# quickwit-oss/tantivy

Measured on AMD Instinct MI355X. Metric: queries_per_sec_2term_AND_bm25_top10, higher is better.
Workload: dtype u32+f32; 1 GPU; and2: 10000 queries/batch, k=10, one 10M-doc Zipf segment per GPU (256 terms, df_r=0.5N/r, WithFreqs); term ranks ~ Zipf(1); distinct_queries=3877, mode=block-max pruned (block_wand_intersection semantics), exchange=single rank: no exchange, segments_per_gpu=1, index_bytes=40381332

## Files before the change

include/tantivy_amd.h:

```cpp
#ifndef TANTIVY_AMD_H
#define TANTIVY_AMD_H

#include <stddef.h>
#include <stdint.h>

#ifdef __cplusplus
extern "C" {
#endif

#define TQ_TERMINATED 0x7FFFFFFFu
#define TQ_MAX_TERMS 16u
#define TQ_MAX_K 1024u

enum tq_status {
  TQ_OK = 0,
  TQ_ERR_INVALID = 1,
  TQ_ERR_HIP = 2,
  TQ_ERR_FORMAT = 3,
  TQ_ERR_UNSUPPORTED = 4,
  TQ_ERR_NO_DEVICE = 5
};

enum tq_record_option { TQ_BASIC = 0, TQ_WITH_FREQS = 1, TQ_WITH_FREQS_AND_POSITIONS = 2 };

// ... 152 lines not shown
typedef struct tq_submit_stats {
  uint64_t batches;
  uint64_t queries;
  uint64_t max_batch;
} tq_submit_stats;
int tq_get_submit_stats(tq_segment *seg, tq_submit_stats *out, int reset);

int tq_merge_topk(const float *scores, const uint32_t *docs, const uint32_t *counts,
                  uint32_t n_segments, uint32_t n_queries, uint32_t stride, uint32_t offset,
                  uint32_t limit, float *out_scores, uint32_t *out_segment_ords,
                  uint32_t *out_docs, uint32_t *out_counts);
int tq_merge_topk_device(tq_ctx *ctx, int device, const float *d_scores, const uint32_t *d_docs,
                         const uint32_t *d_counts, const uint32_t *segment_ords,
                         uint32_t n_segments, uint32_t n_queries, uint32_t stride,
                         uint32_t offset, uint32_t limit, float *d_out_scores,
                         uint32_t *d_out_segment_ords, uint32_t *d_out_docs,
                         uint32_t *d_out_counts, void *hip_stream);
int tq_copy_to_host_async(tq_ctx *ctx, int device, void *dst_pinned_host, const void *src_device, size_t bytes,
                          void *hip_stream);

#define TQ_COMM_ID_BYTES 128
typedef struct tq_comm tq_comm;
int tq_comm_unique_id(uint8_t *id_out );
int tq_comm_init(tq_ctx *ctx, int device, const uint8_t *id, int rank, int world, tq_comm **out);
void tq_comm_free(tq_comm *comm);
int tq_comm_info(const tq_comm *comm, int *rank, int *world, const char **library);
int tq_allgather_topk(tq_comm *comm, const float *d_scores, const uint32_t *d_docs,
                      const uint32_t *d_counts, uint32_t n_rows, uint32_t stride,
                      float *d_all_scores, uint32_t *d_all_docs, uint32_t *d_all_counts,
                      void *hip_stream);

int tq_decode_postings(tq_segment *seg, tq_term_handle term, uint32_t *docs, uint32_t *tfs);
int tq_decode_position_deltas(tq_segment *seg, tq_term_handle term, uint32_t *out, uint64_t cap,
                              uint64_t *n_out);

enum {
  TQ_TABLE_REC = 0,
  TQ_TABLE_COARSE = 1,
  TQ_TABLE_TAIL_DOCS = 2,
  TQ_TABLE_TAIL_TFS = 3,
  TQ_TABLE_POS_BLK = 4,
  TQ_TABLE_POS_TAIL = 5,
  TQ_TABLE_DENSE = 6,
  TQ_TABLE_BITS = 7,
  TQ_TABLE_POS_DIR = 8,
  TQ_TABLE_TF8 = 9,
  TQ_TABLE_RMAX = 10,
  TQ_TABLE_RDIR = 11,
  TQ_TABLE_LNORM = 12,
  TQ_TABLE_FLAT = 13,
  TQ_TABLE_PROBE_DENSE = 14,
  TQ_TABLE_PROBE_TF8 = 15,
  TQ_TABLE_PROBE_POS_DIR = 16,
  TQ_TABLE_DOCMAT = 32,
  TQ_TABLE_DOCCLS = 33,
  TQ_TABLE_LOCAL_CACHE = 34,
  TQ_TABLE_MIN_FIELDNORM_ID = 35
};
typedef struct tq_term_table_info_t {
  uint32_t n_blocks, n_full, n_tail, coarse_shift;
  uint64_t payload_base;
  uint32_t has_freq;
  uint32_t rdir_shift;
  uint32_t rmax_list;
  uint32_t n_pos_blocks, n_pos_tail;
  uint32_t field;
  uint64_t n_positions;
  uint32_t doc_freq;
  uint32_t probe_slot;
} tq_term_table_info_t;
int tq_term_table_read(tq_segment *seg, tq_term_handle term, uint32_t which, void *out, uint64_t cap_bytes,
                       uint64_t *n_bytes);
int tq_term_table_info(tq_segment *seg, tq_term_handle term, tq_term_table_info_t *info);

typedef struct tq_encoder tq_encoder;
int tq_encoder_create(tq_ctx *ctx, int device, tq_encoder **out);
void tq_encoder_free(tq_encoder *enc);
int tq_encode_postings(tq_encoder *enc, uint32_t n_terms, const uint64_t *term_starts,
                       const uint32_t *docs, const uint32_t *tfs, const uint8_t *fieldnorm_ids,
                       uint32_t num_docs, float avg_fieldnorm, uint8_t record_option, uint8_t *out,
                       uint64_t out_cap, uint64_t *out_term_starts, uint64_t *out_len);
int tq_encode_positions(tq_encoder *enc, uint32_t n_terms, const uint64_t *term_starts,
                        const uint32_t *position_deltas, uint8_t *out, uint64_t out_cap,
                        uint64_t *out_term_starts, uint64_t *out_len);
int tq_encode_postings_device(tq_encoder *enc, uint32_t n_terms, const uint64_t *term_starts,
                              const uint64_t *d_term_starts, const uint32_t *d_docs,
                              const uint32_t *d_tfs, const uint8_t *d_fieldnorm_ids,
                              uint32_t num_docs, float avg_fieldnorm, uint8_t record_option,
                              uint8_t *d_out, uint64_t out_cap, uint64_t *d_out_term_starts,
                              uint64_t *out_len, void *hip_stream);
int tq_encode_positions_device(tq_encoder *enc, uint32_t n_terms, const uint64_t *term_starts,
                               const uint64_t *d_term_starts, const uint32_t *d_position_deltas,
                               uint8_t *d_out, uint64_t out_cap, uint64_t *d_out_term_starts,
                               uint64_t *out_len, void *hip_stream);
int tq_encoder_last_kernel_ms(tq_encoder *enc, float *ms);

int tq_segment_set_alive_bitset(tq_segment *seg, const uint8_t *bytes, size_t len);
int tq_count_batch(tq_segment *seg, const tq_query *queries, uint32_t n_queries,
                   uint32_t *out_counts);
int tq_last_batch_match_counts(tq_segment *seg, uint32_t *out, uint32_t n_queries);
int tq_last_batch_slop_overflows(tq_segment *seg, uint32_t *out, uint32_t n_queries);

int tq_docset_batch(tq_segment *seg, const tq_query *queries, uint32_t n_queries,
                    uint32_t *out_docs, uint64_t out_cap, uint64_t *out_starts);
int tq_docset_batch_device(tq_segment *seg, const tq_query *queries, uint32_t n_queries,
                           uint32_t *d_out_docs, uint64_t out_cap, uint64_t *d_out_starts, void *hip_stream);
// ... 105 lines not shown
                           tq_agg_bucket_stats_t *out_entry_stats, uint32_t out_stride);
int tq_agg_terms_sub_batch_device(tq_segment *seg, const tq_query *queries, uint32_t n_queries, const tq_agg_terms_sub_request *req,
                                  tq_agg_terms_t *d_out_terms, uint64_t *d_out_keys, uint32_t *d_out_counts,
                                  tq_agg_bucket_stats_t *d_out_entry_stats, uint32_t out_stride, void *hip_stream);
void tq_agg_terms_sub_lds_capacities(uint32_t out[2]);
int tq_agg_terms_metric_image(const tq_agg_bucket_stats_t *rec, uint32_t value_type, uint32_t metric, uint64_t out[2]);

typedef struct tq_batch_stats {
  uint64_t algorithmic_bytes;
  uint64_t matches;
  float kernel_ms;
  float total_ms;
  uint32_t tiles;
  uint32_t chunks;
  uint32_t batches_averaged;
  float host_plan_ms;
  uint32_t kernel_mask;
  uint64_t unique_bytes;
} tq_batch_stats;
#define TQ_KERNEL_AND_DENSE 0x001u
#define TQ_KERNEL_AND 0x002u
#define TQ_KERNEL_UNION 0x004u
#define TQ_KERNEL_OR_WINDOWS 0x008u
#define TQ_KERNEL_PHRASE 0x010u
#define TQ_KERNEL_PHRASE_SWEEP 0x020u
#define TQ_KERNEL_BOOL 0x040u
#define TQ_KERNEL_USHARE 0x080u
#define TQ_KERNEL_XUNION 0x100u
#define TQ_KERNEL_ASHARE 0x200u
#define TQ_KERNEL_BSHARE 0x400u
#define TQ_KERNEL_COUNT_BITMAPS 0x800u
#define TQ_KERNEL_TREE 0x1000u
#define TQ_KERNEL_DOCSET 0x2000u
#define TQ_KERNEL_DOCSET_SCORE 0x4000u
#define TQ_KERNEL_ALL 0x8000u
#define TQ_KERNEL_DOCSET_TREE 0x10000u
#define TQ_KERNEL_DOCSET_TREE_SCORE 0x20000u
#define TQ_KERNEL_PHRASE_SLOP 0x40000u
#define TQ_KERNEL_SORT 0x80000u
#define TQ_KERNEL_AGG 0x100000u
#define TQ_KERNEL_AGG_SUB 0x200000u
#define TQ_KERNEL_AGG_TERMS 0x400000u
#define TQ_KERNEL_AGG_TERMS_SUB 0x800000u
int tq_last_batch_stats(tq_segment *seg, tq_batch_stats *out);
int tq_last_batch_query_kernels(tq_segment *seg, uint32_t *out, uint32_t n_queries);
typedef struct tq_segment_stats {
  uint64_t index_bytes, positions_bytes, fieldnorm_bytes, alive_bytes;
  uint64_t term_table_bytes, bitmap_bytes , docmat_bytes, posdir_bytes;
  uint64_t scratch_bytes;
  uint64_t dense_budget_bytes;
  uint32_t n_terms, n_dense_lists, n_docmat_columns;
  uint32_t probe_evictions;
  uint64_t device_scratch_bytes;
} tq_segment_stats;
int tq_segment_get_stats(tq_segment *seg, tq_segment_stats *out);
int tq_set_option(tq_segment *seg, const char *name, int64_t value);

#ifdef __cplusplus
}
#endif
#endif
```

tantivy_amd/binding.py:

```python
import ctypes as C
import os

import numpy as np

_HERE = os.path.dirname(os.path.abspath(__file__))
LIB_PATH = os.path.join(_HERE, "lib", "libtantivy_amd.so")
if os.environ.get("TQ_LIB_PATH"):
    LIB_PATH = os.environ["TQ_LIB_PATH"]

TERMINATED = 0x7FFFFFFF
TERM_ABSENT = 0xFFFFFFFF
TERM_ALL = 0xFFFFFFFE
STAR = TERM_ALL
ALL_EMPTY, ALL_PLAIN, ALL_BASED = 0, 1, 2
MODE_AND, MODE_OR, MODE_PHRASE, MODE_BOOL, MODE_TERM = 0, 1, 2, 3, 4
SHOULD, MUST, MUST_NOT = 0, 1, 2
BASIC, WITH_FREQS, WITH_FREQS_AND_POSITIONS = 0, 1, 2


class TantivyAmdError(RuntimeError):
    def __init__(self, code, msg):
        super().__init__("tantivy_amd error %d: %s" % (code, msg))
        self.code = code

# ... 20 lines not shown
    _fields_ = [("algorithmic_bytes", C.c_uint64), ("matches", C.c_uint64),
                ("kernel_ms", C.c_float), ("total_ms", C.c_float), ("tiles", C.c_uint32),
                ("chunks", C.c_uint32), ("batches_averaged", C.c_uint32),
                ("host_plan_ms", C.c_float), ("kernel_mask", C.c_uint32), ("unique_bytes", C.c_uint64)]


KERNEL_AND_DENSE, KERNEL_AND, KERNEL_UNION, KERNEL_OR_WINDOWS, KERNEL_PHRASE = 0x1, 0x2, 0x4, 0x8, 0x10
KERNEL_PHRASE_SWEEP, KERNEL_BOOL, KERNEL_USHARE, KERNEL_XUNION, KERNEL_ASHARE = 0x20, 0x40, 0x80, 0x100, 0x200
KERNEL_BSHARE = 0x400
KERNEL_COUNT_BITMAPS = 0x800
KERNEL_TREE = 0x1000
KERNEL_DOCSET = 0x2000
KERNEL_DOCSET_SCORE = 0x4000
KERNEL_ALL = 0x8000
KERNEL_DOCSET_TREE = 0x10000
KERNEL_DOCSET_TREE_SCORE = 0x20000
KERNEL_PHRASE_SLOP = 0x40000
KERNEL_SORT = 0x80000
KERNEL_AGG = 0x100000
KERNEL_AGG_SUB = 0x200000
KERNEL_AGG_TERMS = 0x400000
KERNEL_AGG_TERMS_SUB = 0x800000
VALUE_U64, VALUE_I64, VALUE_F64 = 0, 1, 2
AGG_MAX_BUCKETS = 65536
SORT_DESC, SORT_ASC = 0, 1
NULLS_LAST, NULLS_FIRST = 0, 1
MAX_K = 1024
MAX_SLOP, SLOP_CARRY_CAP = 255, 32
NESTED_PHRASE = 0x10
KERNEL_NAMES = {0x1: "and_dense", 0x2: "and", 0x4: "union", 0x8: "or_windows", 0x10: "phrase", 0x20: "phrase_sweep",
                0x40: "bool", 0x80: "ushare", 0x100: "xunion", 0x200: "ashare", 0x400: "bshare", 0x800: "count_bitmaps",
                0x1000: "tree", 0x2000: "docset", 0x4000: "docset_score", 0x8000: "all", 0x10000: "docset_tree",
                0x20000: "docset_tree_score", 0x40000: "phrase_slop", 0x80000: "sort", 0x100000: "agg", 0x200000: "agg_sub",
                0x400000: "agg_terms", 0x800000: "agg_terms_sub"}


def kernel_names(mask):
    return [n for b, n in sorted(KERNEL_NAMES.items()) if mask & b]


class TqAllForm(C.Structure):
    _fields_ = [("kind", C.c_uint32), ("base", C.c_float), ("min_should", C.c_uint32), ("keep_mask", C.c_uint32)]


class TqSubmitStats(C.Structure):
    _fields_ = [("batches", C.c_uint64), ("queries", C.c_uint64), ("max_batch", C.c_uint64)]


class TqSegmentStats(C.Structure):
    _fields_ = [(n, C.c_uint64) for n in (
        "index_bytes", "positions_bytes", "fieldnorm_bytes", "alive_bytes", "term_table_bytes",
        "bitmap_bytes", "docmat_bytes", "posdir_bytes", "scratch_bytes", "dense_budget_bytes")] + [
        (n, C.c_uint32) for n in ("n_terms", "n_dense_lists", "n_docmat_columns", "probe_evictions")] + [
        ("device_scratch_bytes", C.c_uint64)]


class TqTermInfo(C.Structure):
    _fields_ = [("postings_off", C.c_uint64), ("positions_off", C.c_uint64), ("postings_len", C.c_uint32),
                ("positions_len", C.c_uint32), ("doc_freq", C.c_uint32), ("pad_", C.c_uint32)]


class TqFieldFiles(C.Structure):
    _fields_ = [("idx", C.c_void_p), ("idx_len", C.c_size_t), ("pos", C.c_void_p), ("pos_len", C.c_size_t),
                ("fieldnorm", C.c_void_p), ("fn_len", C.c_size_t)]


class TqFieldsStats(C.Structure):
    _fields_ = [("n_fields", C.c_uint32), ("n_field_terms", C.c_uint32), ("extra_fieldnorm_bytes", C.c_uint64)]


MAX_FIELDS = 8


class TqhTermInfo(C.Structure):
    _fields_ = [("term_id", C.c_uint32), ("doc_freq", C.c_uint32), ("postings_start", C.c_uint64),
                ("postings_end", C.c_uint64), ("positions_start", C.c_uint64),
                ("positions_end", C.c_uint64)]


class TqhQuery(C.Structure):
    _fields_ = [("mode", C.c_uint8), ("n_terms", C.c_uint32), ("terms", C.POINTER(C.c_uint32)),
                ("phrase_offsets", C.POINTER(C.c_uint32)), ("occurs", C.POINTER(C.c_uint8)),
                ("clause_of", C.POINTER(C.c_uint8)), ("min_should_match", C.c_uint32), ("slop", C.c_uint32),
                ("boosts", C.POINTER(C.c_float)), ("nested_occurs", C.POINTER(C.c_uint8)),
                ("clause_min_should", C.POINTER(C.c_uint8)), ("atom_of", C.POINTER(C.c_uint8)),
                ("set_terms", C.POINTER(C.c_uint32)), ("set_starts", C.POINTER(C.c_uint32))]


TERM_SET_BASE = 0xFFFFFF00


class RawHandle(int):
    """A tq_term_handle as the C ABI returned it (DeviceIndex.term_set_prepare): DeviceIndex.term_handle passes it
    through untouched where a plain int is a term id of the dictionary."""


_lib = None

EXPORTS = [
    "tq_init", "tq_shutdown", "tq_last_error", "tq_segment_upload", "tq_segment_upload_device",
    "tq_segment_free",
    "tq_term_prepare", "tq_term_prepare_batch", "tq_search_batch", "tq_search_batch_device", "tq_search_batch_opts",
    "tq_search_batch_device_opts", "tq_search_batch_device_rows", "tq_merge_topk",
    "tq_merge_topk_device", "tq_copy_to_host_async", "tq_decode_postings", "tq_decode_position_deltas",
    "tq_last_batch_stats", "tq_segment_get_stats", "tq_segment_reserve_columns", "tq_set_option", "tq_segment_set_alive_bitset", "tq_count_batch",
    "tq_last_batch_match_counts", "tq_last_batch_slop_overflows", "tq_last_batch_query_kernels", "tq_encoder_create", "tq_encoder_free", "tq_encode_postings",
    "tq_encode_positions", "tq_encode_postings_device", "tq_encode_positions_device",
    "tq_encoder_last_kernel_ms", "tq_comm_unique_id", "tq_comm_init", "tq_comm_free",
    "tq_comm_info", "tq_allgather_topk",
    "tqh_last_error", "tqh_searcher_new", "tqh_searcher_free", "tqh_searcher_add_segment",
    "tqh_prepare_batch", "tqh_prepare_batch_next", "tqh_commit_next", "tqh_search_prepared", "tqh_collect_segment_prepared",
    "tqh_collect_segment_prepared_device", "tqh_search_prepared_device", "tqh_exchange_ms", "tqh_searcher_add_remote_stats",
    "tqh_bm25_for_terms", "tqh_segment_raw", "tqh_term_handle", "tqh_term_dictionary_values",
    "tqh_term_info_store_open", "tqh_term_info_store_free", "tqh_term_info_store_num_terms",
    "tqh_term_info_store_get", "tqh_term_info_store_write", "tqh_searcher_add_segment_with_store",
    "tqh_count_prepared", "tqh_searcher_add_segment_device_with_store",
    "tq_docset_batch", "tq_docset_batch_device", "tqh_docset_prepared",
    "tq_docset_scored_batch", "tq_docset_scored_batch_device", "tqh_docset_scored_prepared",
    "tq_all_query_form",
    "tq_term_set_prepare", "tq_term_set_info", "tq_term_set_release",
    "tq_segment_upload_fields", "tq_segment_get_fields_stats", "tq_term_prepare_field", "tq_term_prepare_batch_fields",
    "tq_term_field", "tqh_searcher_add_segment_fields", "tqh_searcher_add_remote_stats_fields",
    "tq_term_table_read", "tq_term_table_info",
    "tq_column_parse", "tq_column_upload", "tq_column_info", "tq_column_release", "tq_column_decode", "tq_range_prepare",
    "tq_search_sorted_batch", "tq_search_sorted_batch_device",
    "tq_agg_histogram_plan", "tq_agg_batch", "tq_agg_batch_device",
    "tq_agg_sub_batch", "tq_agg_sub_batch_device", "tq_agg_sub_lds_capacities",
    "tq_agg_terms_plan", "tq_agg_terms_batch", "tq_agg_terms_batch_device", "tq_agg_terms_lds_capacities",
    "tq_agg_terms_max_size",
    "tq_agg_terms_sub_batch", "tq_agg_terms_sub_batch_device", "tq_agg_terms_sub_lds_capacities", "tq_agg_terms_metric_image",
]

TERM_TABLES = {
    "rec": (0, np.uint32), "coarse": (1, np.uint32), "tail_docs": (2, np.uint32), "tail_tfs": (3, np.uint32),
    "pos_blk": (4, np.uint64), "pos_tail": (5, np.uint32), "dense": (6, np.uint32), "bits": (7, np.uint32),
    "pos_dir": (8, np.uint32), "tf8": (9, np.uint8), "rmax": (10, np.uint8), "rdir": (11, np.uint32),
    "lnorm": (12, np.uint8), "flat": (13, np.uint8), "probe_dense": (14, np.uint32), "probe_tf8": (15, np.uint8),
    "probe_pos_dir": (16, np.uint32),
    "docmat": (32, np.uint64), "doccls": (33, np.uint64), "local_cache": (34, np.float32), "min_fieldnorm_id": (35, np.uint32),
}


class TqTermTableInfo(C.Structure):
    _fields_ = [("n_blocks", C.c_uint32), ("n_full", C.c_uint32), ("n_tail", C.c_uint32), ("coarse_shift", C.c_uint32),
                ("payload_base", C.c_uint64), ("has_freq", C.c_uint32), ("rdir_shift", C.c_uint32),
                ("rmax_list", C.c_uint32), ("n_pos_blocks", C.c_uint32), ("n_pos_tail", C.c_uint32), ("field", C.c_uint32),
                ("n_positions", C.c_uint64), ("doc_freq", C.c_uint32), ("probe_slot", C.c_uint32)]


class TqColumnInfo(C.Structure):
    _fields_ = [("min_value", C.c_uint64), ("max_value", C.c_uint64), ("gcd", C.c_uint64), ("resident_bytes", C.c_uint64),
                ("num_rows", C.c_uint32), ("num_bits", C.c_uint32), ("codec", C.c_uint32), ("cardinality", C.c_uint32)]


MAX_COLUMNS = 16
CARD_FULL, CARD_OPTIONAL, CARD_MULTIVALUED = 0, 1, 2
CODEC_BITPACKED, CODEC_LINEAR, CODEC_BLOCKWISE_LINEAR = 0, 1, 2
BOUND_KINDS = {"in": 1, "ex": 2}


class TqAggRequest(C.Structure):
    _fields_ = [("column", C.c_uint32), ("value_type", C.c_uint8), ("histogram", C.c_uint8), ("has_hard_bounds", C.c_uint8),
                ("reserved", C.c_uint8), ("interval", C.c_double), ("offset", C.c_double), ("hard_min", C.c_double),
                ("hard_max", C.c_double)]


class TqAggHistPlan(C.Structure):
    _fields_ = [("base_pos", C.c_int64), ("n_buckets", C.c_uint32), ("reserved", C.c_uint32), ("bounds_min", C.c_double),
                ("bounds_max", C.c_double)]


AGG_STATS_DTYPE = np.dtype([(n, np.uint64) for n in ("matches", "count", "min_value", "max_value", "sum_lo", "sum_hi",
                                                     "in_bounds", "out_of_range")])


class TqAggMetricRequest(C.Structure):
    _fields_ = [("column", C.c_uint32), ("value_type", C.c_uint8), ("reserved", C.c_uint8 * 3)]


AGG_BUCKET_STATS_DTYPE = np.dtype([(n, np.uint64) for n in ("count", "min_value", "max_value", "sum_lo", "sum_hi")])


def _agg_request(column, value_type, histogram):
    req = TqAggRequest(column=int(column), value_type=int(value_type))
    if histogram is not None:
        req.histogram = 1
        req.interval = float(histogram["interval"])
        req.offset = float(histogram.get("offset", 0.0))
        hb = histogram.get("hard_bounds")
        if hb is not None:
            req.has_hard_bounds, req.hard_min, req.hard_max = 1, float(hb[0]), float(hb[1])
# ... 1040 lines not shown
        _check(lib().tq_term_table_info(self.segment_raw(segment_ord), int(handle), C.byref(info)))
        return {n: int(getattr(info, n)) for n, _ in TqTermTableInfo._fields_}

    def decode_position_deltas(self, term_id, cap, segment_ord=0):
        h = self.term_handle(term_id, segment_ord)
        out = np.zeros(max(1, cap), np.uint32)
        n = C.c_uint64()
        _check(lib().tq_decode_position_deltas(self.segment_raw(segment_ord), h, _u32(out), cap,
                                               C.byref(n)))
        return out[: min(cap, n.value)], n.value

    def set_alive_bitset(self, alive_bytes, segment_ord=0):
        if alive_bytes is None:
            _check(lib().tq_segment_set_alive_bitset(self.segment_raw(segment_ord), None, 0))
            return
        a = np.ascontiguousarray(np.frombuffer(bytes(alive_bytes), dtype=np.uint8))
        _check(lib().tq_segment_set_alive_bitset(self.segment_raw(segment_ord), a.ctypes.data,
                                                 a.size))

    def last_batch_match_counts(self, n, segment_ord=0):
        out = np.zeros(max(1, n), np.uint32)
        _check(lib().tq_last_batch_match_counts(self.segment_raw(segment_ord), _u32(out), n))
        return out[:n]

    def last_batch_slop_overflows(self, n, segment_ord=0):
        out = np.zeros(max(1, n), np.uint32)
        _check(lib().tq_last_batch_slop_overflows(self.segment_raw(segment_ord), _u32(out), n))
        return out[:n]

    def last_batch_query_kernels(self, n, segment_ord=0):
        out = np.zeros(max(1, n), np.uint32)
        _check(lib().tq_last_batch_query_kernels(self.segment_raw(segment_ord), _u32(out), n))
        return out[:n]

    def set_option(self, name, value, segment_ord=None):
        ords = range(self.n_segments) if segment_ord is None else [segment_ord]
        for o in ords:
            _check(lib().tq_set_option(self.segment_raw(o), name.encode(), int(value)))

    def last_batch_stats(self, segment_ord=0):
        st = TqBatchStats()
        _check(lib().tq_last_batch_stats(self.segment_raw(segment_ord), C.byref(st)))
        return {"algorithmic_bytes": st.algorithmic_bytes, "matches": st.matches,
                "kernel_ms": st.kernel_ms, "total_ms": st.total_ms, "tiles": st.tiles,
                "chunks": st.chunks, "batches_averaged": st.batches_averaged,
                "host_plan_ms": st.host_plan_ms, "kernel_mask": int(st.kernel_mask),
                "kernels": kernel_names(int(st.kernel_mask)), "unique_bytes": int(st.unique_bytes)}

    def segment_stats(self, segment_ord=0):
        st = TqSegmentStats()
        _check(lib().tq_segment_get_stats(self.segment_raw(segment_ord), C.byref(st)))
        out = {n: int(getattr(st, n)) for n, _ in TqSegmentStats._fields_}
        out["derived_bytes"] = (out["term_table_bytes"] + out["bitmap_bytes"] + out["docmat_bytes"]
                                + out["posdir_bytes"])
        out["tantivy_bytes"] = (out["index_bytes"] + out["positions_bytes"] + out["fieldnorm_bytes"]
                                + out["alive_bytes"])
        return out

    def _raw_flat_queries(self, queries, segment_ord):
        n = len(queries)
        qs = (TqQuery * max(1, n))()
        keep = []
        for i, q in enumerate(queries):
            extra = q[-1] if isinstance(q[-1], dict) else None
            if extra is not None:
                q = q[:-1]
            mode, terms = q[0], q[1]
            hs = (C.c_uint32 * max(1, len(terms)))(*[self.term_handle(t, segment_ord) for t in terms])
            keep.append(hs)
            qs[i].n_terms = len(terms)
            qs[i].terms = C.cast(hs, C.POINTER(C.c_uint32))
            qs[i].mode = mode
            qs[i].k = 1
            if mode == MODE_BOOL:
                oc = (C.c_uint8 * len(terms))(*[int(o) for o in q[2]])
                keep.append(oc)
                qs[i].occurs = C.cast(oc, C.POINTER(C.c_uint8))
                if len(q) > 3 and q[3] is not None:
                    co = (C.c_uint8 * len(terms))(*[int(o) for o in q[3]])
                    keep.append(co)
                    qs[i].clause_of = C.cast(co, C.POINTER(C.c_uint8))
                if len(q) > 4:
                    qs[i].min_should_match = int(q[4])
                if extra and extra.get("nested_occurs") is not None:
                    na = (C.c_uint8 * len(terms))(*[int(o) for o in extra["nested_occurs"]])
                    keep.append(na)
                    qs[i].nested_occurs = C.cast(na, C.POINTER(C.c_uint8))
                if extra and extra.get("atom_of") is not None:
                    aa = (C.c_uint8 * len(terms))(*[int(o) for o in extra["atom_of"]])
                    keep.append(aa)
                    qs[i].atom_of = C.cast(aa, C.POINTER(C.c_uint8))
                if extra and extra.get("phrase_offsets") is not None:
                    pa = (C.c_uint32 * len(terms))(*[int(o) for o in extra["phrase_offsets"]])
                    keep.append(pa)
                    qs[i].phrase_offsets = C.cast(pa, C.POINTER(C.c_uint32))
                if extra and extra.get("clause_min_should") is not None:
                    ma = (C.c_uint8 * 16)(*[int(extra["clause_min_should"].get(c, 0)) for c in range(16)])
                    keep.append(ma)
                    qs[i].clause_min_should = C.cast(ma, C.POINTER(C.c_uint8))
            elif mode == MODE_PHRASE:
                oa = (C.c_uint32 * len(terms))(*(q[2] if len(q) > 2 and q[2] is not None else range(len(terms))))
                keep.append(oa)
                qs[i].phrase_offsets = C.cast(oa, C.POINTER(C.c_uint32))
                if len(q) > 3:
                    qs[i].slop = int(q[3])
        return qs, keep

# ... 390 lines not shown
```

tantivy_amd/csrc/tq_api.cpp:

```cpp
#include "tq_internal.hpp"
#include "../host/bm25.hpp"

namespace tqi {

thread_local std::string g_last_error;

int fail(int code, const char *fmt, ...) {
  char buf[512];
  va_list ap;
  va_start(ap, fmt);
  vsnprintf(buf, sizeof buf, fmt, ap);
  va_end(ap);
  g_last_error = buf;
  return code;
}
}

int tq_internal_fail(int code, const char *where, const char *what) {
  return fail(code, "%s: %s", where, what);
}
bool tq_internal_ctx_has_device(const tq_ctx *ctx, int device) {
  return std::find(ctx->devices.begin(), ctx->devices.end(), device) != ctx->devices.end();
}

// ... 465 lines not shown
      }
      s->batches_reported = s->batches_timed;
      if (n) {
        s->stats.kernel_ms = (float)(k_sum / n);
        s->stats.total_ms = (float)(t_sum / n);
      }
      s->stats.batches_averaged = n;
    }
    s->stats.host_plan_ms = s->host_ms_n ? (float)(s->host_ms_sum / s->host_ms_n) : 0.0f;
    s->host_ms_sum = 0;
    s->host_ms_n = 0;
    s->stats_pending = false;
  }
  *out = s->stats;
  return TQ_OK;
}

int tq_segment_reserve_columns(tq_segment *s, const uint64_t *postings_offs, uint32_t n) {
  if (!s || (!postings_offs && n)) return fail(TQ_ERR_INVALID, "tq_segment_reserve_columns: null argument");
  TQ_SEGMENT_LOCK(s);
  if (!s->terms.empty())
    return fail(TQ_ERR_INVALID, "tq_segment_reserve_columns: call it before the first tq_term_prepare");
  s->reserved_cols.clear();
  for (uint32_t i = 0; i < n && i < TQD_MAT_SLOTS; ++i) s->reserved_cols[postings_offs[i]] = true;
  s->cols_reserved = true;
  return TQ_OK;
}

int tq_segment_get_stats(tq_segment *s, tq_segment_stats *out) {
  if (!s || !out) return fail(TQ_ERR_INVALID, "tq_segment_get_stats: null argument");
  TQ_SEGMENT_LOCK(s);
  tq_segment_stats r{};
  r.index_bytes = s->idx_len;
  r.positions_bytes = s->pos_len;
  r.fieldnorm_bytes = s->d_fn ? s->max_doc : 0;
  r.alive_bytes = s->bytes_alive;
  r.term_table_bytes = s->bytes_term_tables + s->d_terms_cap * sizeof(TqdTerm);
  r.bitmap_bytes = s->bytes_bitmaps;
  r.docmat_bytes = s->bytes_docmat;
  r.posdir_bytes = s->bytes_posdir;
  r.scratch_bytes = s->d_stage.cap + s->d_stage_alt.cap + s->d_misc.cap + s->d_thr.cap + s->d_qmatches.cap + s->d_share_words.cap +
                    s->d_ashare_words.cap + s->d_bshare_words.cap + s->d_count_queries.cap + s->d_count_out.cap +
                    s->d_count_bits.cap + s->d_count_wgs.cap + s->d_set_work.cap + s->docset_scratch_bytes();
  {
    std::lock_guard<std::mutex> lk(s->dscratch->m);
    r.device_scratch_bytes = s->dscratch->partials.cap + s->dscratch->share_stage.cap + s->dscratch->ashare_stage.cap +
                             s->dscratch->bshare_stage.cap;
  }
  r.n_terms = (uint32_t)s->terms.size();
  r.n_dense_lists = s->n_dense_lists;
  r.n_docmat_columns = s->n_mat_slots;
  r.probe_evictions = (uint32_t)std::min<uint64_t>(s->probe_evictions, 0xFFFFFFFFull);
  r.dense_budget_bytes = s->dense_budget();
  *out = r;
  return TQ_OK;
}

int tq_set_option(tq_segment *s, const char *name, int64_t value) {
  if (!s || !name) return fail(TQ_ERR_INVALID, "tq_set_option: null argument");
  TQ_SEGMENT_LOCK(s);
  if (!strcmp(name, "exhaustive"))
    __atomic_store_n(&s->opt.exhaustive, value != 0 ? 1 : 0, __ATOMIC_RELAXED);
  else if (!strcmp(name, "timing"))
    s->opt.timing = value != 0;
  else if (!strcmp(name, "use_dpp"))
    s->opt.use_dpp = value != 0;
  else if (!strcmp(name, "use_dense"))
    s->opt.use_dense = value != 0;
  else if (!strcmp(name, "or_windows"))
    s->opt.or_windows = value < 0 ? -1 : (value != 0);
  else if (!strcmp(name, "dense_ratio") && value >= 1)
    s->opt.dense_ratio = (int)value;
  else if (!strcmp(name, "rdir_budget_x") && value >= 0 && value <= 0x7FFFFFFF)
    s->opt.rdir_budget_x = (int)value;
  else if (!strcmp(name, "probe_budget_x") && value >= 0 && value <= 0x7FFFFFFF)
    s->opt.probe_budget_x = (int)value, s->probe_full = false;
  else if (!strcmp(name, "dense_budget_x") && value >= 0)
    s->opt.dense_budget_x = (int)value;
  else if (!strcmp(name, "bound_slack_ppm") && value >= 0 && value <= 1000000000)
    __atomic_store_n(&s->opt.bound_slack_ppm, (int)value, __ATOMIC_RELAXED);
  else if (!strcmp(name, "dense"))
    s->opt.dense = value != 0;
  else if (!strcmp(name, "docmat"))
    s->opt.docmat = value != 0;
  else if (!strcmp(name, "docsig"))
    s->opt.docsig = value != 0;
  else if (!strcmp(name, "device_prepare"))
    s->opt.device_prepare = value != 0;
  else if (!strcmp(name, "xunion_ratio") && value >= 0 && value <= 0x7FFFFFFF)
    s->opt.xunion_ratio = (int)value;
  else if (!strcmp(name, "count_bitmap_ratio") && value >= 0 && value <= 0x7FFFFFFF)
    s->opt.count_bitmap_ratio = (int)value;
  else if (!strcmp(name, "docset_temp_lists") && value >= 0 && value <= 0x7FFFFFFF)
    s->opt.docset_temp_lists = (int)value;
  else if (!strcmp(name, "docset_trees") && (value == 0 || value == 1))
    s->opt.docset_trees = (int)value;
  else if (!strcmp(name, "docset_score_trees") && (value == 0 || value == 1))
    s->opt.docset_score_trees = (int)value;
  else if (!strcmp(name, "sort_slices") && value >= 0 && value <= 256)
    s->opt.sort_slices = (int)value;
  else if (!strcmp(name, "agg_slices") && value >= 0 && value <= 256)
    s->opt.agg_slices = (int)value;
  else if (!strcmp(name, "agg_lds_buckets") && value >= 0 && value <= (int64_t)tqk_agg_lds_buckets())
    s->opt.agg_lds_buckets = (int)value;
  else if (!strcmp(name, "ashare_inline_warm") && value >= 0 && value <= 2)
    s->opt.ashare_inline_warm = (int)value;
  else if (!strcmp(name, "ashare_min_batch") && value >= 0 && value <= 0x7FFFFFFF)
    s->opt.ashare_min_batch = (int)value;
  else if (!strcmp(name, "xunion_min_queries") && value >= 1 && value <= 0x7FFFFFFF)
    s->opt.xunion_min_queries = (int)value;
  else if (!strcmp(name, "record_query_kernels"))
    s->opt.record_query_kernels = value != 0;
  else if (!strcmp(name, "debug") && value >= -1 && value <= 0x7FFFFFFF)
    s->opt.debug = (int)value;
  else if (!strcmp(name, "submit_window_us") && value >= 0 && value <= 1000000)
    s->opt.submit_window_us = (int)value;
  else
    return fail(TQ_ERR_INVALID, "unknown option '%s'", name);
  return TQ_OK;
}

int tq_decode_postings(tq_segment *s, tq_term_handle term, uint32_t *docs, uint32_t *tfs) {
  if (!s || !docs || !tfs) return fail(TQ_ERR_INVALID, "tq_decode_postings: null argument");
  TQ_SEGMENT_LOCK(s);
  if (term >= s->terms.size()) return fail(TQ_ERR_INVALID, "unknown term handle %u", term);
  if (s->terms[term].set_kind != TermHost::kNoSet) return fail(TQ_ERR_INVALID, "tq_decode_postings: handle %u is a term set: it has no postings", term);
  HIP_TRY(hipSetDevice(s->device));
// ... 26 lines not shown
  if (n == 0 || !out) return TQ_OK;
  HIP_TRY(hipSetDevice(s->device));
  int rc = sync_terms(s, s->stream);
  if (rc != TQ_OK) return rc;
  rc = s->d_misc.ensure(n * sizeof(uint32_t));
  if (rc != TQ_OK) return rc;
  hipError_t e = tqk_launch_decode_positions(s->dseg, s->d_terms, term, (uint32_t *)s->d_misc.p, n,
                                             s->stream);
  if (e != hipSuccess) return fail(TQ_ERR_HIP, "decode launch: %s", hipGetErrorString(e));
  HIP_TRY(hipMemcpyAsync(out, s->d_misc.p, n * sizeof(uint32_t), hipMemcpyDeviceToHost, s->stream));
  HIP_TRY(hipStreamSynchronize(s->stream));
  return TQ_OK;
}

namespace {
struct TableSpan {
  const void *p = nullptr;
  size_t bytes = 0;
  bool host = false;
};
bool table_span(tq_segment *s, uint32_t term, uint32_t which, TableSpan &sp) {
  if (which >= TQ_TABLE_DOCMAT) {
    const size_t per_doc = (size_t)s->max_doc * sizeof(uint64_t);
    switch (which) {
      case TQ_TABLE_DOCMAT: sp = {s->d_docmat, s->d_docmat ? per_doc : 0, false}; return true;
      case TQ_TABLE_DOCCLS: sp = {s->d_doccls, s->d_doccls ? per_doc : 0, false}; return true;
      case TQ_TABLE_LOCAL_CACHE: sp = {s->d_local_cache, s->d_local_cache ? 256 * sizeof(float) : 0, false}; return true;
      case TQ_TABLE_MIN_FIELDNORM_ID: sp = {&s->dseg.min_fieldnorm_id, sizeof(uint32_t), true}; return true;
      default: return false;
    }
  }
  const TermHost &t = s->terms[term];
  const TqdTerm &d = s->h_dterms[term];
  const size_t n_words = bitmap_words(s);
  const size_t n_dir = ((size_t)t.doc_freq + 3) / 4 + 1;
  const bool list = t.set_kind == TermHost::kNoSet;
  uint32_t n_buckets = 0;
  if (list && t.n_blocks) (void)coarse_shift(s->max_doc, t.n_blocks, &n_buckets);
  auto span = [&](const void *p, size_t bytes) { sp = {p, p ? bytes : 0, false}; };
  switch (which) {
    case TQ_TABLE_REC: span(list ? d.rec : nullptr, 16 * ((size_t)t.n_blocks + 1)); return true;
    case TQ_TABLE_COARSE: span(list ? d.coarse : nullptr, 4 * ((size_t)n_buckets + 1)); return true;
    case TQ_TABLE_TAIL_DOCS: span(list && t.n_tail ? d.tail_docs : nullptr, 4 * (size_t)t.n_tail); return true;
    case TQ_TABLE_TAIL_TFS: span(list && t.n_tail ? d.tail_tfs : nullptr, 4 * (size_t)t.n_tail); return true;
    case TQ_TABLE_POS_BLK: span(list && d.n_pos_blocks ? d.pos_blk : nullptr, 8 * (size_t)d.n_pos_blocks); return true;
    case TQ_TABLE_POS_TAIL: span(list && d.n_pos_tail ? d.pos_tail : nullptr, 4 * (size_t)d.n_pos_tail); return true;
    case TQ_TABLE_DENSE: span(t.dense_blob, n_words * sizeof(uint2)); return true;
    case TQ_TABLE_BITS: span(list ? d.bits : nullptr, ((n_words + 255) & ~(size_t)255) * sizeof(uint32_t)); return true;
    case TQ_TABLE_POS_DIR: span(list ? t.posdir_blob : nullptr, n_dir * sizeof(uint32_t)); return true;
    case TQ_TABLE_TF8: span(list ? t.tf8_blob : nullptr, t.doc_freq); return true;
    case TQ_TABLE_RMAX: span(list ? t.rmax_blob : nullptr, tqd_rm_level_off(s->max_doc, TQD_RM_LEVELS)); return true;
    case TQ_TABLE_RDIR: span(list ? t.rdir_blob : nullptr, t.rdir_shift ? rdir_bytes(s, t.doc_freq, t.rdir_shift) : 0); return true;
    case TQ_TABLE_LNORM: span(list ? t.lnorm_blob : nullptr, (size_t)t.n_blocks * 128u); return true;
    case TQ_TABLE_FLAT:
      span(list ? t.flat_blob : nullptr, (((size_t)t.doc_freq * sizeof(uint32_t) + 15) & ~(size_t)15) + t.doc_freq);
      return true;
    case TQ_TABLE_PROBE_DENSE: span(t.probe_dense_blob, n_words * sizeof(uint2)); return true;
    case TQ_TABLE_PROBE_TF8: span(t.probe_tf8_blob, t.doc_freq); return true;
    case TQ_TABLE_PROBE_POS_DIR: span(t.probe_posdir_blob, n_dir * sizeof(uint32_t)); return true;
    default: return false;
  }
}
int table_handle_ok(tq_segment *s, tq_term_handle term, const char *who) {
  if (term >= s->terms.size()) return fail(TQ_ERR_INVALID, "%s: unknown term handle %u", who, term);
  if (s->terms[term].set_kind == TermHost::kSetReleased) return fail(TQ_ERR_INVALID, "%s: handle %u is a released term set", who, term);
  return TQ_OK;
}
int table_quiesce(tq_segment *s) {
  HIP_TRY(hipSetDevice(s->device));
  const int rc = wait_segment_idle(s);
  if (rc != TQ_OK) return rc;
  HIP_TRY(hipStreamSynchronize(s->stream));
  prep_apply_lmax(s, true);
  return TQ_OK;
}
}

int tq_term_table_read(tq_segment *s, tq_term_handle term, uint32_t which, void *out, uint64_t cap_bytes, uint64_t *n_bytes) {
  if (!s || !n_bytes) return fail(TQ_ERR_INVALID, "tq_term_table_read: null argument");
  *n_bytes = 0;
  TQ_SEGMENT_LOCK(s);
  if (which < TQ_TABLE_DOCMAT) {
    const int hrc = table_handle_ok(s, term, "tq_term_table_read");
    if (hrc != TQ_OK) return hrc;
  }
  int rc = table_quiesce(s);
  if (rc != TQ_OK) return rc;
  TableSpan sp;
  if (!table_span(s, term, which, sp)) return fail(TQ_ERR_INVALID, "tq_term_table_read: unknown table %u", which);
  *n_bytes = sp.bytes;
  if (!sp.bytes || !out || !cap_bytes) return TQ_OK;
  if (cap_bytes < sp.bytes)
    return fail(TQ_ERR_INVALID, "tq_term_table_read: table %u holds %zu bytes, room for %llu", which, sp.bytes, (unsigned long long)cap_bytes);
  if (sp.host) {
    memcpy(out, sp.p, sp.bytes);
    return TQ_OK;
  }
  HIP_TRY(hipMemcpyAsync(out, sp.p, sp.bytes, hipMemcpyDeviceToHost, s->stream));
  HIP_TRY(hipStreamSynchronize(s->stream));
  return TQ_OK;
}

int tq_term_table_info(tq_segment *s, tq_term_handle term, tq_term_table_info_t *info) {
  if (!s || !info) return fail(TQ_ERR_INVALID, "tq_term_table_info: null argument");
  TQ_SEGMENT_LOCK(s);
  int rc = table_handle_ok(s, term, "tq_term_table_info");
// ... 113 lines not shown
```

tantivy_amd/csrc/tq_ashare.hip:

```cpp
#include "tq_common.hpp"

#ifndef TQ_BS_SGPR
#define TQ_BS_SGPR 96
#endif
#ifndef TQ_BS_WAVES
#define TQ_BS_WAVES 5
#endif
#ifndef TQ_AS_WAVES
#define TQ_AS_WAVES 5
#endif
#ifndef TQ_AS_TIMERS
#define TQ_AS_TIMERS 0
#endif
#ifndef TQ_AS_PREFETCH
#define TQ_AS_PREFETCH 1
#endif

namespace {

constexpr uint32_t AS_GROUP = TQD_AS_GROUP;
constexpr uint32_t AS_COUNTER_BITS = 0x7FE0u | 0xF00000u | 0x40000000u;

template <bool BOOLQ>
struct AShareLds {
  float cache[256];
  uint32_t q_doc[127], q_tf[127], q_tag[127];
  TqdALeadLds lead[AS_GROUP];
  uint32_t lthr[AS_GROUP];
  uint32_t lk[AS_GROUP];
  uint32_t cnt[AS_GROUP];
  uint32_t flen[AS_GROUP];
  float bw[BOOLQ ? AS_GROUP * TQD_AS_MAX_TERMS : 1];
  uint32_t pay[(TQ_AS_PREFETCH && !BOOLQ) ? 260 : 1];
};

template <int R>
__device__ __forceinline__ uint64_t as_kth_largest_key(const uint64_t (&v)[R], uint32_t k) {
  uint64_t ans = 0;
  for (int bit = 63; bit >= 0; --bit) {
    const uint64_t trial = ans | (1ull << bit);
    uint32_t c = 0;
#pragma unroll
    for (int r = 0; r < R; ++r) c += (uint32_t)__popcll(__ballot(v[r] >= trial));
    if (c >= k) ans = trial;
  }
  return ans;
}

__device__ __forceinline__ uint32_t as_exact_tf(const uint8_t *idx, const TqdTerm *terms, uint32_t handle,
                                                uint32_t pi) {
  const TqdTermHead *h = terms + handle;
  TermRef tr{};
  tr.rec = h->rec;
  tr.tail_tfs = h->tail_tfs;
  tr.payload_base = h->payload_base;
  tr.has_freq = h->has_freq & 1u;
  const uint4 r = tr.rec[pi >> 7];
  return block_tf_at(idx, tr, make_uint2(r.y, r.z), pi & 127u);
}

template <int KPL, bool BOOLQ, bool RD = false>
__global__ __launch_bounds__(64) __attribute__((amdgpu_num_sgpr(TQ_BS_SGPR), amdgpu_waves_per_eu(BOOLQ ? TQ_BS_WAVES : TQ_AS_WAVES, 8))) void
ashare_kernel(TqkAShareParams p) {
  constexpr bool USE_DPP = true;
  constexpr bool PF = TQ_AS_PREFETCH && !BOOLQ;
  constexpr int R = KPL + 1;
  constexpr uint32_t CAPL = (uint32_t)R * 64u;
  __shared__ AShareLds<BOOLQ> L;
  const int lane = (int)__lane_id();
  const TqdSegment seg = p.seg;
  const uint8_t *idx = seg.idx;
  uint64_t *const my_stage = p.stage + (size_t)blockIdx.x * (size_t)(AS_GROUP * CAPL);
  const uint8_t *const tbase = p.table_base;
  const uint32_t bmode = BOOLQ ? 0u : p.bound_mode;
  uint32_t cache_loaded = 0xFFFFFFFFu;
  uint32_t qn = 0;
  uint32_t n_scored = 0;
  uint32_t n_leads = 0;
  const uint32_t tphase = TQ_AS_TIMERS ? (p.debug >> 16) & 15u : 0u;
  uint64_t tacc = 0, tlast = 0;
  auto tb = [&](uint32_t ph) __attribute__((always_inline)) {
    if (TQ_AS_TIMERS && tphase == ph) tlast = __builtin_readcyclecounter();
  };
  auto te = [&](uint32_t ph) __attribute__((always_inline)) {
    if (TQ_AS_TIMERS && tphase == ph) tacc += __builtin_readcyclecounter() - tlast;
  };
// ... 231 lines not shown
    wave_mem_fence();
    const uint32_t cn = (uint32_t)lane < AS_GROUP ? L.cnt[lane] & 0xFFFFu : 0u;
    uint64_t full = __ballot(cn > CAPL - 64u);
    while (full) {
      const uint32_t gs = (uint32_t)__builtin_ctzll(full);
      full &= full - 1ull;
      const uint32_t ns = (uint32_t)__builtin_amdgcn_readlane((int)cn, (int)gs);
      const uint32_t ks = uni(L.lk[gs]) & 0xFFu;
      if (p.debug & 4096u) ++n_scored;
      const uint64_t kth = compact_slot(gs, ns, ks);
      const uint32_t t = (uint32_t)(kth >> 32);
      if ((uint32_t)lane == gs) {
        L.cnt[gs] = (L.cnt[gs] & 0xFFFF0000u) | ks;
        if (t > L.lthr[gs]) L.lthr[gs] = t;
        atomicMax(p.thr_val + L.lead[gs].query, t);
      }
    }
    wave_mem_fence();
    te(7u);
    tb(6u);
  };

  const uint32_t n_launch = p.n_tasks - p.task_begin;
  const uint32_t nq = p.n_queues ? p.n_queues : 1u;
  const uint32_t xcc = (uint32_t)__builtin_amdgcn_s_getreg((3 << 11) | 20) & 7u;
  const uint32_t home = xcc % nq;
  uint32_t q_tried = 0;
  for (;;) {
    tb(2u);
    uint32_t task = 0xFFFFFFFFu;
    while (q_tried < nq) {
      uint32_t qx = home + q_tried;
      if (qx >= nq) qx -= nq;
      const uint32_t q0 = (uint32_t)((uint64_t)n_launch * qx / nq), q1 = (uint32_t)((uint64_t)n_launch * (qx + 1u) / nq);
      uint32_t t = 0;
      if (lane == 0) t = atomicAdd(p.task_counter + qx, 1u);
      t = uni(t) + q0;
      if (t < q1) {
        task = t + p.task_begin;
        break;
      }
      ++q_tried;
    }
    if (task == 0xFFFFFFFFu) break;
    const uint4 trec = sload(p.tasks + task);
    const uint32_t j0 = trec.y, nb_task = trec.z & 0xFFFFu, ci = trec.z >> 24, lead0 = trec.w;
    n_leads = (trec.z >> 16) & 0xFFu;
    const TermRef lead = load_term(p.terms, trec.x);
    uint32_t lnorm = 0;
    if constexpr (!BOOLQ) lnorm = sload(&p.leads[lead0].any2_lo);
    auto norm_pair = [&](uint32_t j) __attribute__((always_inline)) -> uint32_t {
      return reinterpret_cast<const uint16_t *>(tbase + ((uint64_t)lnorm << 3))[(size_t)j * 64u + (uint32_t)lane];
    };
    if (ci != cache_loaded) {
      const float *cg = p.caches + (size_t)ci * 256u;
      wave_mem_fence();
      for (int i = lane; i < 256; i += WAVE) L.cache[i] = cg[i];
      wave_mem_fence();
      cache_loaded = ci;
    }
    wave_mem_fence();
    float my_w = 0.0f, my_rest = 0.0f;
    uint32_t my_mlo = 0, my_mhi = 0;
    uint32_t my_xlo = 0, my_xhi = 0, my_a1lo = 0, my_a1hi = 0, my_a2lo = 0, my_a2hi = 0;
    uint32_t my_blo = 0, my_bhi = 0;
    bool twin = false;
    const bool is_lead = (uint32_t)lane < n_leads;
    if (is_lead) {
      const TqdALead mine = p.leads[lead0 + lane];
      L.lead[lane] = TqdALeadLds{mine.query, mine.info, mine.w, mine.rest, mine.dense_off, mine.tf8_off};
      my_w = mine.w;
      my_rest = mine.rest;
      my_mlo = mine.mask_lo;
      my_mhi = mine.mask_hi;
      if constexpr (BOOLQ) {
        my_xlo = mine.excl_lo;
        my_xhi = mine.excl_hi;
        my_a1lo = mine.any1_lo;
        my_a1hi = mine.any1_hi;
        my_a2lo = mine.any2_lo;
        my_a2hi = mine.any2_hi;
        my_blo = mine.dense_off;
        my_bhi = mine.tf8_off;
        const TqdQuery *Q = p.queries + mine.query;
        const uint32_t li = (mine.info >> 16) & 15u, nt = mine.info & 31u;
#pragma unroll
        for (uint32_t m = 0; m < TQD_AS_MAX_TERMS; ++m) L.bw[(uint32_t)lane * TQD_AS_MAX_TERMS + m] = (m > li && m < nt) ? Q->weight[m] : 0.0f;
      }
      if constexpr (!BOOLQ) {
        my_xlo = (bmode && (mine.info & 31u) == 2u) ? mine.excl_lo : 0u;
        const bool rdir = bmode && (mine.info & TQD_AL_RDIR) != 0u;
        my_xhi = rdir ? mine.dense_off | ((mine.info >> 16) & 31u) : 0u;
        if (my_xlo || rdir) {
          const float r1 = mine.rest * p.bound_slack * (1.00002f / 255.0f) * (float)(mine.any1_hi & 0xFFu);
          my_rest = r1 < mine.rest ? r1 : mine.rest;
        }
      }
      twin = lane != 0 && (mine.info & 0x200u) != 0u;
      L.lk[lane] = mine.k | (mine.thr_row << 8);
      L.lthr[lane] = __hip_atomic_load(p.thr_val + mine.query, __ATOMIC_RELAXED, __HIP_MEMORY_SCOPE_AGENT);
    }
    if ((uint32_t)lane < AS_GROUP) L.cnt[lane] = 0u;
    const bool is_head = is_lead && !twin;
    const uint32_t heads = (uint32_t)__ballot(is_head);
    if (is_head) {
      const uint32_t above = (uint32_t)lane >= 31u ? 0u : heads & ~((2u << lane) - 1u);
// ... 60 lines not shown
          blk_last = rec_mine.x;
          const uint32_t wide = blk_last >= blk_first ? (blk_last - blk_first) >> TQD_RM_SHIFT : 0xFFFFFFFFu;
          const uint32_t lvl = wide ? (33u - (uint32_t)__builtin_clz(wide)) >> 1 : 0u;
          if (lvl < TQD_RM_LEVELS) rm_pack = tqd_rm_level_off(seg.max_doc, lvl) | ((TQD_RM_SHIFT + 2u * lvl) << 24);
        }
      }
      uint32_t pass_mask = 0;
      float need_blk = 3.0e38f;
      for (uint32_t lm = live_heads; lm; lm &= lm - 1u) {
        const uint32_t g = (uint32_t)__builtin_ctz(lm);
        const float w = __uint_as_float((uint32_t)__builtin_amdgcn_readlane((int)__float_as_uint(my_w), (int)g));
        float rest = __uint_as_float((uint32_t)__builtin_amdgcn_readlane((int)__float_as_uint(my_rest), (int)g));
        const uint32_t thr = (uint32_t)__builtin_amdgcn_readlane((int)fam_thr, (int)g);
        if constexpr (!BOOLQ) {
          const uint32_t rmo = (uint32_t)__builtin_amdgcn_readlane((int)my_xlo, (int)g);
          if ((bmode & 1u) && rmo) {
            const uint8_t *rt = tbase + ((uint64_t)rmo << 3) + (rm_pack & 0xFFFFFFu);
            const uint32_t sh = rm_pack >> 24;
            const uint32_t qa = sh ? (uint32_t)rt[blk_first >> sh] : 255u, qb = sh ? (uint32_t)rt[blk_last >> sh] : 255u;
            if (p.debug & 0x800000u) n_scored += 2u * (uint32_t)__popcll(__ballot(sh != 0u));
            const float w1 = uni_f(L.lead[g].rest);
            const float r1 = w1 * p.bound_slack * (1.00002f / 255.0f) * (float)(qa > qb ? qa : qb);
            rest = r1 < rest ? r1 : rest;
          }
        }
        bool empty = false;
        if constexpr (!BOOLQ) {
          const uint32_t rdo = (uint32_t)__builtin_amdgcn_readlane((int)my_xhi, (int)g);
          if ((bmode & 1u) && rdo) {
            const uint32_t S = rdo & 31u;
            const uint32_t *dr = reinterpret_cast<const uint32_t *>(tbase + ((uint64_t)(rdo & ~31u) << 3));
            if (blk_last >= blk_first) empty = dr[blk_first >> S] == dr[(blk_last >> S) + 1u];
          }
        }
        const float ub = w * tfn_max * p.bound_slack;
        if (in_tile && !empty && sortable((ub + rest) * 1.000004f + (w + rest) * 4.0e-6f) >= thr) {
          pass_mask |= 1u << g;
          if constexpr (!BOOLQ) {
            const float thr_f = __uint_as_float((uint32_t)__builtin_amdgcn_readlane((int)__float_as_uint(fam_thr_f), (int)g));
            const float num = thr_f - rest * 1.00001f;
            const float nd = (thr_f > 0.0f && num > 0.0f) ? num * __builtin_amdgcn_rcpf(w) * 0.99999f : -1.0f;
            need_blk = nd < need_blk ? nd : need_blk;
          }
        }
      }
      uint64_t todo = __ballot(pass_mask != 0u);
      uint32_t since_refresh = 0;
      te(3u);
      uint32_t npair_next = 0;
      auto prefetch = [&](uint64_t rest) __attribute__((always_inline)) {
        if (!PF || !rest) return;
        const uint32_t nb2 = (uint32_t)__builtin_ctzll(rest);
        if (lnorm) npair_next = norm_pair(i_base + nb2);
        const uint32_t meta = (uint32_t)__builtin_amdgcn_readlane((int)rec_mine.y, (int)nb2);
        const uint32_t off = (uint32_t)__builtin_amdgcn_readlane((int)rec_mine.z, (int)nb2);
        if (meta == META_TAIL) return;
        const uint32_t nbytes = 16u * ((meta & 31u) + (lead.has_freq ? (meta >> 8) & 0xFFu : 0u));
        const uint32_t o = 16u * (uint32_t)lane;
        if (o < nbytes)
          __builtin_amdgcn_global_load_lds((const __attribute__((address_space(1))) void *)(idx + lead.payload_base + off + o),
                                           (__attribute__((address_space(3))) void *)L.pay, 16, 0, 0);
      };
      if constexpr (PF) {
        wave_mem_fence();
        prefetch(todo);
      }
      while (todo) {
        const uint32_t b = (uint32_t)__builtin_ctzll(todo);
        todo &= todo - 1ull;
        if (++since_refresh == 8u) {
          since_refresh = 0;
          tb(9u);
          refresh_thr();
          update_families();
          te(9u);
          if (!live) break;
        }
        tb(4u);
        uint32_t lm = (uint32_t)__builtin_amdgcn_readlane((int)pass_mask, (int)b) & live_heads;
        const uint32_t prev_l = (uint32_t)__builtin_amdgcn_readlane((int)prev_mine, (int)b);
        const uint2 mo_l = make_uint2((uint32_t)__builtin_amdgcn_readlane((int)rec_mine.y, (int)b),
                                      (uint32_t)__builtin_amdgcn_readlane((int)rec_mine.z, (int)b));
        if (!lm) {
          if constexpr (PF) {
            asm volatile("s_waitcnt vmcnt(0)" ::: "memory");
            wave_mem_fence();
            prefetch(todo);
          }
          te(4u);
          continue;
        }
        if (p.debug & 256u) ++n_scored;
        if (p.debug & 0x100000u)
          n_scored += 16u + (mo_l.x == META_TAIL ? 8u * lead.n_tail : 16u * ((mo_l.x & 31u) + (lead.has_freq ? (mo_l.x >> 8) & 0xFFu : 0u)));
        uint32_t c0, c1, t0, t1;
        uint32_t npair = 0;
        if constexpr (PF) {
        npair = npair_next;
        if (mo_l.x == META_TAIL) {
          asm volatile("s_waitcnt vmcnt(0)" ::: "memory");
          decode_docs<USE_DPP>(idx, lead, mo_l, prev_l, lane, c0, c1);
          decode_tfs(idx, lead, mo_l, lane, t0, t1);
        } else {
          const uint32_t doc_bits = mo_l.x & 31u;
          const uint32_t strict = (mo_l.x >> 6) & 1u;
          const uint32_t tf_bits = lead.has_freq ? (mo_l.x >> 8) & 0xFFu : 0u;
          asm volatile("s_waitcnt vmcnt(0)" ::: "memory");
          wave_mem_fence();
          if (lead.has_freq) {
            unpack2_lds(L.pay + 4u * doc_bits, tf_bits, lane, t0, t1);
            t0 += strict;
            t1 += strict;
          } else {
            t0 = 1u;
            t1 = 1u;
          }
          uint32_t x0, x1;
          unpack2_lds(L.pay, doc_bits, lane, x0, x1);
          finish_docs<USE_DPP>(x0, x1, strict, prev_l, lane, c0, c1);
        }
        wave_mem_fence();
        prefetch(todo);
        } else {
        if (lnorm) npair = norm_pair(i_base + b);
        decode_docs<USE_DPP>(idx, lead, mo_l, prev_l, lane, c0, c1);
        decode_tfs(idx, lead, mo_l, lane, t0, t1);
        }
        if (TQ_AS_TIMERS && tphase == 4u && c0 == 0xFFFFFFFEu) ++n_scored;
        te(4u);
        tb(5u);
        const bool v0 = c0 != TQD_TERMINATED, v1 = c1 != TQD_TERMINATED;
        float block_need = 3.0e38f;
        for (uint32_t x = lm; x; x &= x - 1u) {
          const float nd = __uint_as_float((uint32_t)__builtin_amdgcn_readlane((int)__float_as_uint(fam_need), (int)__builtin_ctz(x)));
          block_need = nd < block_need ? nd : block_need;
        }
        if constexpr (!BOOLQ) {
          if (bmode & 2u) {
            const float nb = __uint_as_float((uint32_t)__builtin_amdgcn_readlane((int)__float_as_uint(need_blk), (int)b));
            block_need = nb > block_need ? nb : block_need;
          }
        }
        if (!lnorm) {
          npair = (v0 ? fieldnorm_id(seg, c0) : 0u) | ((v1 ? fieldnorm_id(seg, c1) : 0u) << 8);
          if (p.debug & 0x40000000u) n_scored += (uint32_t)(__popcll(__ballot(v0)) + __popcll(__ballot(v1)));
        }
        const uint32_t nid0 = npair & 0xFFu, nid1 = npair >> 8;
        const float f0 = (float)t0, f1 = (float)t1;
        const float tfn0 = f0 * __builtin_amdgcn_rcpf(f0 + L.cache[nid0]);
        const float tfn1 = f1 * __builtin_amdgcn_rcpf(f1 + L.cache[nid1]);
        const bool g0 = v0 && tfn0 >= block_need, g1 = v1 && tfn1 >= block_need;
        const uint64_t mw0 = g0 ? seg.docmat[c0] : 0ull;
        const uint64_t mw1 = g1 ? seg.docmat[c1] : 0ull;
        const uint64_t valid0 = __ballot(g0), valid1 = __ballot(g1);
        if (p.debug & 0x200000u) n_scored += (uint32_t)(__popcll(__ballot(v0)) + __popcll(__ballot(v1)));
        if (p.debug & 0x400000u) n_scored += (uint32_t)(__popcll(valid0) + __popcll(valid1));
        if (TQ_AS_TIMERS && tphase == 5u && (uint32_t)mw0 == 0xFFFFFFFEu) ++n_scored;
        te(5u);
        tb(6u);
        uint32_t pm_lo = 0, pm_hi = 0;
        uint64_t mem0 = valid0, mem1 = valid1;
        uint32_t pb0 = 0xFFu, pb1 = 0xFFu;
        if (p.debug & 2048u) lm = 0;
        for (; lm; lm &= lm - 1u) {
          const uint32_t g = (uint32_t)__builtin_ctz(lm);
          if (p.debug & 32u) ++n_scored;
          const uint32_t mlo = (uint32_t)__builtin_amdgcn_readlane((int)my_mlo, (int)g);
          const uint32_t mhi = (uint32_t)__builtin_amdgcn_readlane((int)my_mhi, (int)g);
          const float need = __uint_as_float((uint32_t)__builtin_amdgcn_readlane((int)__float_as_uint(fam_need), (int)g));
          if constexpr (BOOLQ) {
            const uint32_t xlo = (uint32_t)__builtin_amdgcn_readlane((int)my_xlo, (int)g);
            const uint32_t xhi = (uint32_t)__builtin_amdgcn_readlane((int)my_xhi, (int)g);
            const uint32_t a1lo = (uint32_t)__builtin_amdgcn_readlane((int)my_a1lo, (int)g);
            const uint32_t a1hi = (uint32_t)__builtin_amdgcn_readlane((int)my_a1hi, (int)g);
            const uint32_t a2lo = (uint32_t)__builtin_amdgcn_readlane((int)my_a2lo, (int)g);
            const uint32_t a2hi = (uint32_t)__builtin_amdgcn_readlane((int)my_a2hi, (int)g);
            const uint32_t l0 = (uint32_t)mw0, h0 = (uint32_t)(mw0 >> 32), l1 = (uint32_t)mw1, h1 = (uint32_t)(mw1 >> 32);
            bool b0 = !((l0 & xlo) | (h0 & xhi));
            bool b1 = !((l1 & xlo) | (h1 & xhi));
            if (a1lo | a1hi) {
              b0 = b0 && ((l0 & a1lo) | (h0 & a1hi));
              b1 = b1 && ((l1 & a1lo) | (h1 & a1hi));
            }
            if (a2lo | a2hi) {
              b0 = b0 && ((l0 & a2lo) | (h0 & a2hi));
              b1 = b1 && ((l1 & a2lo) | (h1 & a2hi));
            }
            b0 = b0 && tfn0 >= need;
            b1 = b1 && tfn1 >= need;
            if (!((__ballot(b0) & valid0) | (__ballot(b1) & valid1))) continue;
            const uint32_t blo = (uint32_t)__builtin_amdgcn_readlane((int)my_blo, (int)g);
            const uint32_t bhi = (uint32_t)__builtin_amdgcn_readlane((int)my_bhi, (int)g);
            pb0 = pb1 = (uni(L.lead[g].info) >> 20) & 0xFFu;
            if (blo | bhi) {
              const float wl = __uint_as_float((uint32_t)__builtin_amdgcn_readlane((int)__float_as_uint(my_w), (int)g));
              const float thr_f = __uint_as_float((uint32_t)__builtin_amdgcn_readlane((int)__float_as_uint(fam_thr_f), (int)g));
              const float4 wa = *reinterpret_cast<const float4 *>(&L.bw[g * TQD_AS_MAX_TERMS]);
              const float4 wb = *reinterpret_cast<const float4 *>(&L.bw[g * TQD_AS_MAX_TERMS + 4u]);
              const float wv[8] = {wa.x, wa.y, wa.z, wa.w, wb.x, wb.y, wb.z, wb.w};
              float ps0 = __uint_as_float(mlo), ps1 = ps0;
#pragma unroll
              for (uint32_t m = 0; m < TQD_AS_MAX_TERMS; ++m) {
                const uint32_t bp = ((m < 4u ? blo : bhi) >> (8u * (m & 3u))) & 0xFFu;
                if (!bp) continue;
                const uint32_t sh = bp & 31u;
                const uint32_t p0 = ((bp & 32u ? h0 : l0) >> sh) & 1u, p1 = ((bp & 32u ? h1 : l1) >> sh) & 1u;
                ps0 += p0 ? wv[m] : 0.0f;
                ps1 += p1 ? wv[m] : 0.0f;
                pb0 &= ~((p0 ^ 1u) << m);
// ... 174 lines not shown
```

tantivy_amd/csrc/tq_internal.hpp:

```cpp
#pragma once
#include <hip/hip_runtime.h>

#include <algorithm>
#include <array>
#include <atomic>
#include <chrono>
#include <condition_variable>
#include <deque>
#include <map>
#include <mutex>
#include <new>
#include <cstdlib>
#include <cmath>
#include <cstdarg>
#include <cstdio>
#include <cstring>
#include <string>
#include <unordered_map>
#include <unordered_set>
#include <thread>
#include <vector>

#include "../../include/tantivy_amd.h"
#include "tq_device.h"
// ... 28 lines not shown
    cap = 0;
    void *np = nullptr;
    HIP_TRY(hipMalloc(&np, ncap));
    p = np;
    cap = ncap;
    return TQ_OK;
  }
  void release() {
    if (p) (void)hipFree(p);
    p = nullptr;
    cap = 0;
  }
};
struct PinnedBuf {
  void *p = nullptr;
  size_t cap = 0;
  int ensure(size_t n) {
    if (n <= cap) return TQ_OK;
    const size_t ncap = std::max(n, cap * 2);
    if (p) (void)hipHostFree(p);
    p = nullptr;
    cap = 0;
    void *np = nullptr;
    HIP_TRY(hipHostMalloc(&np, ncap, hipHostMallocDefault));
    p = np;
    cap = ncap;
    return TQ_OK;
  }
  void release() {
    if (p) (void)hipHostFree(p);
    p = nullptr;
    cap = 0;
  }
};

struct TermHost {
  void *blob = nullptr;
  const TqdTerm *d_self = nullptr;
  void *dense_blob = nullptr;
  void *posdir_blob = nullptr;
  void *tf8_blob = nullptr;
  void *pos_blob = nullptr;
  void *probe_dense_blob = nullptr, *probe_tf8_blob = nullptr;
  void *probe_posdir_blob = nullptr;
  int32_t probe_slot = -1;
  void *rdir_blob = nullptr;
  void *rdir_ent = nullptr;
  uint32_t rdir_shift = 0;
  uint8_t *probe_own_dir = nullptr;
  void *rmax_blob = nullptr;
  uint32_t rmax_list = 255;
  void *flat_blob = nullptr;
  void *lnorm_blob = nullptr;
  uint32_t doc_freq = 0, n_blocks = 0, n_full = 0, n_tail = 0;
  uint32_t last_doc = 0;
  bool wants_col = true;
  uint64_t postings_len = 0, positions_len = 0;
  uint64_t n_positions = 0;
  enum : uint8_t { kNoSet = 0, kSet = 1, kSetReleased = 2 };
  uint8_t set_kind = kNoSet;
  uint8_t field = 0;
};

inline uint32_t rd32(const uint8_t *p) {
  return (uint32_t)p[0] | ((uint32_t)p[1] << 8) | ((uint32_t)p[2] << 16) | ((uint32_t)p[3] << 24);
}
inline bool read_vint(const uint8_t *d, size_t len, size_t &at, uint64_t &out) {
  uint64_t r = 0;
  unsigned shift = 0;
  while (at < len) {
    uint8_t b = d[at++];
    r |= (uint64_t)(b & 127u) << shift;
    if (b & 128u) {
      out = r;
      return true;
    }
    shift += 7;
    if (shift > 63) return false;
  }
  return false;
}
inline bool read_vint32_block(const uint8_t *d, size_t len, size_t &at, uint32_t &out) {
  uint32_t r = 0, shift = 0;
  while (at < len) {
    uint8_t b = d[at++];
    r += (uint32_t)(b & 127u) << shift;
    if (b & 128u) {
      out = r;
      return true;
    }
    shift += 7;
  }
  return false;
}

struct Options {
  int exhaustive = 0;
  int timing = 0;
  int use_dpp = 1;
  int dense = 1;
  int dense_ratio = TQD_DENSE_RATIO;
  int dense_budget_x = 8;
  int use_dense = 1;
  int docmat = 1;
  int docsig = 1;
  int device_prepare = 0;
  int or_windows = -1;
  int bound_slack_ppm = 0;
  int xunion_ratio = 64;
  int xunion_min_queries = 64;
  int rdir_budget_x = 4;
  int probe_budget_x = 16;
  int count_bitmap_ratio = 128;
  int docset_temp_lists = 0;
  int docset_trees = 0;
  int docset_score_trees = 0;
  int sort_slices = 0;
  int agg_slices = 0;
  int agg_lds_buckets = -1;
  int ashare_inline_warm = 1;
  int ashare_min_batch = 16;
  int submit_window_us = 100;
  int record_query_kernels = 0;
  int debug = -1;
};


inline uint32_t tune_u32(const char *name, uint32_t dflt) {
  const char *v = getenv(name);
  return v && *v ? (uint32_t)strtoul(v, nullptr, 10) : dflt;
}

}
using namespace tqi;

struct DeviceScratch {
  std::mutex m;
  DevBuf partials, share_stage, ashare_stage, bshare_stage;
  hipEvent_t ev_last = nullptr;
  hipStream_t last_stream = nullptr;
  bool in_flight = false;
};
struct tq_ctx {
  std::vector<int> devices;
  std::mutex m;
  std::map<int, DeviceScratch *> scratch;
  DeviceScratch *scratch_for(int device) {
    std::lock_guard<std::mutex> lk(m);
    DeviceScratch *&p = scratch[device];
    if (!p) p = new DeviceScratch();
    return p;
  }
  ~tq_ctx() {
    for (auto &kv : scratch) {
      (void)hipSetDevice(kv.first);
      if (kv.second->ev_last) (void)hipEventDestroy(kv.second->ev_last);
      kv.second->partials.release();
      kv.second->share_stage.release();
      kv.second->ashare_stage.release();
      kv.second->bshare_stage.release();
      delete kv.second;
    }
  }
// ... 34 lines not shown
  bool d_terms_dirty = false;
  size_t d_terms_dirty_from = ~(size_t)0;
  size_t d_terms_synced = 0;
  size_t dense_bytes_total = 0;
  uint8_t *dense_arena = nullptr;
  size_t dense_arena_cap = 0, dense_arena_used = 0;
  std::vector<void *> dense_extra;
  bool dense_arena_vmm = false;
  void *dense_arena_va = nullptr;
  size_t dense_arena_mapped = 0, dense_arena_first = 0;
  std::vector<std::pair<hipMemGenericAllocationHandle_t, size_t>> dense_arena_chunks;
  size_t bytes_term_tables = 0, bytes_bitmaps = 0, bytes_docmat = 0, bytes_posdir = 0, bytes_alive = 0;
  uint32_t n_dense_lists = 0;
  uint32_t n_set_slots = 0;
  std::vector<uint32_t> set_free_slots;
  std::vector<void *> set_free_tables;
  DevBuf d_set_work;
  struct ColumnHost {
    bool live = false;
    tq_column_info_t info{};
    TqkColumn dev{};
    void *d_payload = nullptr;
    void *d_blocks = nullptr;
    void *d_present = nullptr;
    uint64_t payload_len = 0;
  };
  ColumnHost columns[TQ_MAX_COLUMNS];
  uint32_t alive_docs = 0;
  std::unordered_map<uint64_t, uint32_t> term_by_off;
  std::unordered_map<uint64_t, bool> reserved_cols;
  bool cols_reserved = false;
  DevBuf d_stage, d_misc, d_thr, d_qmatches;
  DevBuf d_share_words;
  DevBuf d_count_queries, d_count_out, d_count_bits, d_count_wgs;
  DevBuf d_docset_queries, d_docset_counts, d_docset_offs, d_docset_partials, d_docset_starts, d_docset_docs;
  DevBuf d_docset_squeries, d_docset_caches, d_docset_scores;
  DevBuf d_docset_trees;
  DevBuf d_sort_ks, d_sort_partials, d_sort_slice_counts, d_sort_rows;
  PinnedBuf h_sort_ks;
  DevBuf d_agg_rows;
  DevBuf d_agg_term_rows;
  PinnedBuf h_docset;
  size_t docset_scratch_bytes() const {
    return d_docset_queries.cap + d_docset_counts.cap + d_docset_offs.cap + d_docset_partials.cap + d_docset_starts.cap +
           d_docset_docs.cap + d_docset_squeries.cap + d_docset_caches.cap + d_docset_scores.cap +
           d_docset_trees.cap + d_sort_ks.cap + d_sort_partials.cap + d_sort_slice_counts.cap + d_sort_rows.cap + d_agg_rows.cap + d_agg_term_rows.cap;
  }
  DevBuf d_ashare_words, d_bshare_words;
  DeviceScratch *dscratch = nullptr;
  size_t share_span_terms = 0;
  uint64_t share_table_lo = 0;
  bool share_span_ok = true;
  bool lnorm_off = false;
  uint32_t last_batch_queries = 0;
  DevBuf d_slop_over;
  bool last_batch_slop = false;
  uint32_t slop_over_words = 0;
  std::vector<uint32_t> slop_over_host;
  std::vector<uint32_t> last_query_kernel;
  PinnedBuf h_stage, h_out;
  static constexpr int kTimingRing = 16;
  hipEvent_t ev_stage_done = nullptr, ev_fork = nullptr, ev_join = nullptr;
  hipEvent_t ev_batch_done = nullptr;
  hipStream_t last_stream = nullptr;
  bool batch_in_flight = false;
  hipStream_t side_stream = nullptr;
  hipStream_t copy_stream = nullptr;
  DevBuf d_stage_alt;
  hipEvent_t ev_copy_done[2] = {nullptr, nullptr}, ev_buf_free[2] = {nullptr, nullptr};
  bool buf_used[2] = {false, false};
  uint64_t batches_enqueued = 0;
  hipEvent_t ev_t0[kTimingRing] = {}, ev_t1[kTimingRing] = {}, ev_k0[kTimingRing] = {},
             ev_k1[kTimingRing] = {};
  uint64_t batches_timed = 0, batches_reported = 0;
  bool stage_in_flight = false;
  double host_ms_sum = 0;
  uint32_t host_ms_n = 0;
  unsigned long long *d_match_counter = nullptr;
  Options opt;
  size_t dense_budget() const { return (size_t)opt.dense_budget_x * (idx_len + pos_len + max_doc); }
  size_t probe_budget() const { return (size_t)opt.probe_budget_x * (idx_len + pos_len + max_doc); }
  size_t rdir_budget() const { return (size_t)opt.rdir_budget_x * (idx_len + pos_len + max_doc); }
  size_t rdir_bytes_total = 0;
  PinnedBuf h_prep_stage[2];
  hipEvent_t ev_prep[2] = {nullptr, nullptr}, ev_prep_order = nullptr;
  bool prep_used[2] = {false, false};
  uint32_t prep_calls = 0;
  int prep_pending = -1;
  std::vector<uint32_t> prep_lmax_handles[2];
  const uint32_t *prep_lmax_host[2] = {nullptr, nullptr};
  size_t probe_bytes_total = 0;
  bool probe_full = false;
  struct ProbeSlot {
    uint8_t *base = nullptr;
    uint32_t owner = 0xFFFFFFFFu;
    uint64_t last_batch = 0;
  };
  std::vector<ProbeSlot> probe_slots;
  size_t probe_slot_bytes = 0, probe_bm_bytes = 0, probe_tf_cap = 0, probe_dir_cap = 0, probe_rm_bytes = 0;
  uint64_t probe_batch = 1;
  uint64_t probe_evictions = 0;
  uint64_t probe_replaced_batch = 0;
  uint32_t probe_replaced_n = 0;
  uint64_t probe_no_room_batch = 0;
  bool probe_waited = false;
  bool device_prepare() const { return h_idx.empty() || opt.device_prepare != 0; }
// ... 369 lines not shown
inline bool dense_fits(const tq_segment *s) { return s->dense_bytes_total + dense_table_bytes(s) <= s->dense_budget(); }
struct WalkSource {
  const uint8_t *idx;
  size_t idx_len;
  const uint8_t *pos;
  size_t pos_len;
  uint8_t record_option;
  uint32_t max_doc;
};
inline WalkSource walk_source(const tq_segment *s) {
  return {s->h_idx.data(), s->h_idx.size(), s->h_pos.data(), s->h_pos.size(), s->record_option, s->max_doc};
}
inline size_t align16(size_t x) { return (x + 15) & ~(size_t)15; }
struct TermBlobLayout {
  size_t o_rec = 0, o_coarse = 0, o_tdocs = 0, o_ttfs = 0, o_pboff = 0, o_ptail = 0, o_self = 0, total = 0;
};
TermBlobLayout term_blob_layout(uint32_t n_blocks, uint32_t n_buckets, uint32_t n_tail, uint32_t n_pos_blocks, uint32_t n_pos_tail);
uint32_t coarse_shift(uint32_t max_doc, uint32_t n_blocks, uint32_t *n_buckets);
struct WalkedTerm {
  std::vector<uint8_t> hb;
  TermBlobLayout lay;
  TqdTerm dt{};
  TermHost th;
  uint64_t postings_off = 0;
};
int host_walk_term(const WalkSource &src, uint64_t postings_off, uint32_t postings_len, uint64_t positions_off,
                   uint32_t positions_len, uint32_t doc_freq, WalkedTerm &w);
void place_walked_term(WalkedTerm &w, uint8_t *blob);
const char *tqp_message(uint32_t st);
int term_alloc(tq_segment *s, size_t bytes, uint8_t **out);
void term_release(tq_segment *s, uint8_t *blob, size_t bytes);
int dense_alloc(tq_segment *s, size_t bytes, void **out);
void dense_release(tq_segment *s, void *ptr);
void dense_arena_free(tq_segment *s);
int rdir_alloc(tq_segment *s, size_t bytes, void **out);
struct DecodedList {
  uint32_t *dd = nullptr, *dt = nullptr, *scan_scratch = nullptr, *rm_acc = nullptr;
};
int decode_list(tq_segment *s, const TermHost &t, size_t scan_words, bool want_rm, DecodedList &dl);
hipError_t enqueue_bitmap(tq_segment *s, const DecodedList &dl, uint32_t doc_freq, void *blob);
hipError_t enqueue_rmax(tq_segment *s, const DecodedList &dl, uint32_t doc_freq, uint8_t *out);
hipError_t finish_tables(tq_segment *s, const DecodedList &dl, uint32_t *bad, uint32_t *lmax);
inline uint32_t rmax_list_of(uint32_t lmax) { return lmax ? std::min<uint32_t>(lmax, 255u) : 255u; }
inline uint32_t sig_bit(uint32_t handle) { return (handle * 0x9E3779B1u) >> (32 - 4); }
uint32_t rdir_plan(tq_segment *s, uint32_t doc_freq);
size_t rdir_dir_words(const tq_segment *s, uint32_t S);
size_t rdir_bytes(const tq_segment *s, uint32_t doc_freq, uint32_t S);
int attach_rdir(tq_segment *s, uint32_t handle, uint32_t S, void **tab);
int ensure_docmat(tq_segment *s);
int add_to_doc_signatures(tq_segment *s, uint32_t handle);
int build_dense_device(tq_segment *s, uint32_t handle);
int build_flat(tq_segment *s, uint32_t handle, hipStream_t st, bool *ok);
void build_lnorm(tq_segment *s, uint32_t handle, hipStream_t st);
void prep_apply_lmax(tq_segment *s, bool wait);
int build_probe_tables(tq_segment *s, uint32_t handle, bool *ok, bool must = false);
int build_probe_posdir(tq_segment *s, uint32_t handle, bool *ok);
void probe_begin_batch(tq_segment *s);
void probe_touch(tq_segment *s, uint32_t handle);
inline bool query_has_all(const tq_query &q) {
  if (!q.terms || q.n_terms > TQ_MAX_TERMS) return false;
  for (uint32_t i = 0; i < q.n_terms; ++i)
    if (q.terms[i] == TQ_TERM_ALL) return true;
  return false;
}
struct AllForm {
  uint32_t kind = TQ_ALL_EMPTY;
  float base = 0.0f;
  uint32_t min_should = 0, keep_mask = 0;
  bool boost_mixed = false;
};
int all_query_form(const tq_query &q, AllForm &f, const char **why);
struct AllView {
  tq_query q;
  tq_term_handle terms[TQ_MAX_TERMS];
  float weights[TQ_MAX_TERMS];
  uint8_t occurs[TQ_MAX_TERMS], clause_of[TQ_MAX_TERMS];
  uint32_t pos[TQ_MAX_TERMS];
};
void all_strip_view(const tq_query &q, const AllForm &f, AllView &v);
inline bool is_term_set(const tq_segment *s, uint32_t h) { return h < s->terms.size() && s->terms[h].set_kind == TermHost::kSet; }
int set_table_acquire(tq_segment *s, void **tab);
void set_table_release(tq_segment *s, void *tab);
uint32_t set_slot_commit(tq_segment *s, void *tab, uint32_t n_docs);
void free_columns(tq_segment *s);
inline const void *expression_bitmap(const tq_segment *s, const TermHost &th) {
  return th.dense_blob && (s->opt.use_dense || th.set_kind == TermHost::kSet) ? th.dense_blob : nullptr;
}
static_assert(TQK_MAX_FIELDS == TQ_MAX_FIELDS, "the multi-field launch parameters hold one fieldnorm pointer per field");
inline uint32_t term_field_of(const tq_segment *s, uint32_t h) { return h < s->terms.size() ? s->terms[h].field : 0u; }
inline bool query_names_field(const tq_segment *s, const tq_query &q) {
  if (!q.terms || q.n_terms > TQ_MAX_TERMS) return false;
  for (uint32_t i = 0; i < q.n_terms; ++i)
    if (term_field_of(s, q.terms[i])) return true;
  return false;
}
struct FieldScope {
  tq_segment *s;
  uint8_t was;
  FieldScope(tq_segment *seg, uint8_t field) : s(seg), was(seg->prep_field) { s->prep_field = field; }
  ~FieldScope() { s->prep_field = was; }
  FieldScope(const FieldScope &) = delete;
  FieldScope &operator=(const FieldScope &) = delete;
};
int check_field_query(const tq_segment *s, const tq_query &q, uint32_t qi, const char *fn);
inline bool query_names_set(const tq_segment *s, const tq_query &q) {
  if (!q.terms || q.n_terms > TQ_MAX_TERMS) return false;
// ... 163 lines not shown
```

tantivy_amd/csrc/tq_launch.h:

```cpp
#pragma once
#include <hip/hip_runtime.h>
#include <stdint.h>

#include "tq_device.h"

struct TqkSinks {
  uint64_t *partials;
  unsigned long long *match_counter;
  uint32_t *query_matches;
  const uint32_t *out_index;
};

struct TqkScanParams {
  TqdSegment seg;
  const TqdTerm *terms;
  const TqdQuery *queries;
  const uint32_t *tile_starts;
  const uint4 *chunk_recs;
  const float *caches;
  const TqkSinks *sinks;
  uint32_t *thr_slots;
  uint32_t n_queries;
  uint32_t total_tiles;
  uint32_t n_chunks;
// ... 465 lines not shown
  uint32_t access;
  uint32_t clause_end;
  uint32_t n_must_lists;
  uint32_t all_base_bits;
  uint32_t handle[TQD_MAX_TERMS];
  float weight[TQD_MAX_TERMS];
  uint32_t shift[TQD_MAX_TERMS];
  const void *tab[TQD_MAX_TERMS];
  const void *aux[TQD_MAX_TERMS];
};
struct TqkScoreParams {
  TqdSegment seg;
  const TqdTerm *terms;
  const TqkScoreQuery *queries;
  const float *caches;
  const uint32_t *tile_counts;
  const uint64_t *tile_offs;
  const uint32_t *out_docs;
  float *out_scores;
  uint64_t out_cap;
  uint32_t n_queries, n_tiles;
  uint32_t any_blocks;
};
hipError_t tqk_launch_docset_score(const TqkScoreParams &p, hipStream_t st);
struct TqkScoreFieldsParams {
  TqkScoreParams base;
  const uint8_t *fn[TQK_MAX_FIELDS];
};
hipError_t tqk_launch_docset_score_fields(const TqkScoreFieldsParams &p, hipStream_t st);
struct TqkDocsetTreeScoreParams {
  TqdSegment seg;
  const TqdTerm *terms;
  const TqdTreeQuery *queries;
  const uint32_t *query_of;
  const float *caches;
  const uint8_t *table_base;
  const uint32_t *tile_counts;
  const uint64_t *tile_offs;
  const uint32_t *out_docs;
  float *out_scores;
  uint64_t out_cap;
  uint32_t n_queries, n_tiles;
  uint32_t any_phrase;
};
hipError_t tqk_launch_docset_tree_score(const TqkDocsetTreeScoreParams &p, hipStream_t st);
hipError_t tqk_launch_ashare(const TqkAShareParams &p, int kpl, hipStream_t st);
uint32_t tqk_ashare_waves_per_cu();
uint32_t tqk_bshare_waves_per_cu();
hipError_t tqk_launch_xunion(const TqkDenseParams &p, int kpl, hipStream_t st);
hipError_t tqk_launch_flat_list(const TqdSegment &seg, const TqdTerm *terms, uint32_t handle,
                                uint32_t n_blocks, uint32_t *docs, uint8_t *tf8, hipStream_t st);
hipError_t tqk_launch_lead_norms(const TqdSegment &seg, const TqdTerm *terms, uint32_t handle, uint32_t n_blocks,
                                 uint8_t *out, hipStream_t st);
hipError_t tqk_launch_decode_list(const TqdSegment &seg, const TqdTerm *terms, uint32_t handle,
                                  uint32_t n_blocks, uint32_t *docs, uint32_t *tfs, bool use_dpp,
                                  hipStream_t st);
hipError_t tqk_launch_decode_positions(const TqdSegment &seg, const TqdTerm *terms,
                                       uint32_t handle, uint32_t *out, uint64_t n, hipStream_t st);
hipError_t tqk_launch_merge_segments(const TqkSegMergeParams &p, hipStream_t st);
hipError_t tqk_launch_docmat_init(uint64_t *mat, const uint8_t *fieldnorm, uint32_t const_id,
                                  uint32_t max_doc, hipStream_t st);
hipError_t tqk_launch_docmat_set(uint64_t *mat, const uint32_t *docs, uint32_t n, uint32_t slot,
                                 uint32_t max_doc, hipStream_t st);
hipError_t tqk_launch_tf8_pack(const uint32_t *tfs, uint32_t n, uint8_t *out, hipStream_t st);


struct tq_ctx;
int tq_internal_fail(int code, const char *where, const char *what);
bool tq_internal_ctx_has_device(const tq_ctx *ctx, int device);
```

tantivy_amd/csrc/tq_misc.hip:

```cpp
#include "tq_common.hpp"

namespace {

template <int KPL, bool PRE>
__global__ __launch_bounds__(64) void merge_kernel(TqkMergeParams p) {
  const int lane = (int)__lane_id();
  const uint32_t q = PRE ? blockIdx.x % p.n_queries : blockIdx.x;
  if (q >= p.n_queries) return;
  const TqdQuery *Q = uni_ptr(p.queries + q);
  const uint32_t k = uni(Q->k);
  uint32_t part_start = uni(Q->part_start), n_parts = uni(Q->n_parts);
  const uint32_t per = tqk_merge_slice_lists(n_parts, p.pre_slices);
  uint32_t stride = 1u;
  if constexpr (PRE) {
    if (per == 1u) return;
    const uint32_t sl = blockIdx.x / p.n_queries;
    if (sl * per >= n_parts) return;
    part_start += sl * per;
    n_parts = n_parts - sl * per < per ? n_parts - sl * per : per;
    if (n_parts == 1u) return;
  } else {
    stride = per;
    n_parts = (n_parts + per - 1u) / per;
  }
// ... 180 lines not shown
          }
        }
      }
    }
  }
  if (!ent || !cache) return;
  for (int o = 32; o; o >>= 1) {
    const uint32_t other = (uint32_t)__shfl_xor((int)lmax, o, WAVE);
    lmax = other > lmax ? other : lmax;
  }
  if (lane == 0 && lmax) atomicMax(lmax_out + blockIdx.x, lmax);
}
__global__ void rdir_fill_kernel(const uint32_t *docs, const uint32_t *tfs, uint32_t n, uint32_t max_doc, uint32_t *dir,
                                 uint32_t S) {
  const uint32_t i = blockIdx.x * blockDim.x + threadIdx.x;
  if (i >= n) return;
  uint32_t *ent = dir + (((max_doc >> S) + 2u + 3u) & ~3u);
  const uint32_t doc = docs[i];
  if (doc >= max_doc) return;
  ent[i] = rdir_entry(doc, tfs[i], S);
  const uint32_t r_to = doc >> S;
  for (uint32_t r = i ? (docs[i - 1u] >> S) + 1u : 0u; r <= r_to; ++r) dir[r] = i;
  if (i + 1u == n)
    for (uint32_t r = r_to + 1u; r <= (max_doc >> S) + 1u; ++r) dir[r] = n;
}

__global__ void doccls_set_kernel(uint64_t *cls, const uint32_t *docs, const uint32_t *tfs, uint32_t n, uint32_t slot,
                                  uint32_t max_doc) {
  const uint32_t i = blockIdx.x * blockDim.x + threadIdx.x;
  if (i < n && docs[i] < max_doc) {
    const uint32_t tf = tfs[i];
    const uint64_t c = tf >= 3u ? 3ull : (tf ? (uint64_t)tf : 3ull);
    atomicOr((unsigned long long *)(cls + docs[i]), (unsigned long long)(c << (2u * slot)));
  }
}

__global__ void tf8_pack_kernel(const uint32_t *tfs, uint32_t n, uint8_t *out) {
  const uint32_t i = blockIdx.x * blockDim.x + threadIdx.x;
  if (i < n) out[i] = (uint8_t)(tfs[i] < 255u ? tfs[i] : 255u);
}

__global__ __launch_bounds__(256) void lead_norms_kernel(TqdSegment seg, const TqdTerm *terms, uint32_t handle, uint8_t *out) {
  const int lane = (int)__lane_id();
  const uint32_t wave = uni(threadIdx.x >> 6);
  const TermRef t = load_term(terms, handle);
  const uint32_t j = blockIdx.x * 4u + wave;
  if (j >= t.n_blocks) return;
  uint32_t d0, d1;
  decode_docs<true>(uni_ptr(seg.idx), t, uni_mo(t, j), block_prev_last(t, j), lane, d0, d1);
  const uint32_t n0 = d0 < seg.max_doc ? (uint32_t)seg.fieldnorm[d0] : 0u, n1 = d1 < seg.max_doc ? (uint32_t)seg.fieldnorm[d1] : 0u;
  reinterpret_cast<uint16_t *>(out)[j * 64u + (uint32_t)lane] = (uint16_t)(n0 | (n1 << 8));
}

}

hipError_t tqk_launch_tf8_pack(const uint32_t *tfs, uint32_t n, uint8_t *out, hipStream_t st) {
  if (n == 0) return hipSuccess;
  hipLaunchKernelGGL(tf8_pack_kernel, dim3((n + 255) / 256), dim3(256), 0, st, tfs, n, out);
  return hipGetLastError();
}
hipError_t tqk_launch_lead_norms(const TqdSegment &seg, const TqdTerm *terms, uint32_t handle, uint32_t n_blocks,
                                 uint8_t *out, hipStream_t st) {
  if (n_blocks == 0 || !seg.fieldnorm) return hipSuccess;
  hipLaunchKernelGGL(lead_norms_kernel, dim3((n_blocks + 3) / 4), dim3(256), 0, st, seg, terms, handle, out);
  return hipGetLastError();
}
hipError_t tqk_launch_docmat_init(uint64_t *mat, const uint8_t *fieldnorm, uint32_t const_id,
                                  uint32_t max_doc, hipStream_t st) {
  if (max_doc == 0) return hipSuccess;
  hipLaunchKernelGGL(docmat_init_kernel, dim3((max_doc + 255) / 256), dim3(256), 0, st, mat,
                     fieldnorm, const_id, max_doc);
  return hipGetLastError();
}
hipError_t tqk_launch_docmat_set(uint64_t *mat, const uint32_t *docs, uint32_t n, uint32_t slot,
                                 uint32_t max_doc, hipStream_t st) {
  if (n == 0) return hipSuccess;
  hipLaunchKernelGGL(docmat_set_kernel, dim3((n + 255) / 256), dim3(256), 0, st, mat, docs, n, slot,
                     max_doc);
  return hipGetLastError();
}
hipError_t tqk_launch_docsig_batch(const TqdSegment &seg, const TqdTerm *const *selfs, const uint32_t *bits, uint32_t n,
                                   uint64_t *mat, uint32_t *const *tabs, const uint32_t *shifts, const uint32_t *dfs,
                                   const float *cache, uint32_t *lmax_out, bool use_dpp, hipStream_t st) {
  if (n == 0) return hipSuccess;
  if (use_dpp)
    hipLaunchKernelGGL((docsig_batch_kernel<true>), dim3(n), dim3(256), 0, st, seg, selfs, bits, mat, tabs, shifts, dfs, cache, lmax_out);
  else
    hipLaunchKernelGGL((docsig_batch_kernel<false>), dim3(n), dim3(256), 0, st, seg, selfs, bits, mat, tabs, shifts, dfs, cache, lmax_out);
  return hipGetLastError();
}
hipError_t tqk_launch_rdir_fill(const uint32_t *docs, const uint32_t *tfs, uint32_t n, uint32_t max_doc, uint32_t *dir,
                                uint32_t S, hipStream_t st) {
  if (n == 0) return hipSuccess;
  hipLaunchKernelGGL(rdir_fill_kernel, dim3((n + 255) / 256), dim3(256), 0, st, docs, tfs, n, max_doc, dir, S);
  return hipGetLastError();
}
hipError_t tqk_launch_doccls_set(uint64_t *cls, const uint32_t *docs, const uint32_t *tfs, uint32_t n, uint32_t slot,
                                 uint32_t max_doc, hipStream_t st) {
  if (n == 0) return hipSuccess;
  hipLaunchKernelGGL(doccls_set_kernel, dim3((n + 255) / 256), dim3(256), 0, st, cls, docs, tfs, n, slot, max_doc);
  return hipGetLastError();
}
hipError_t tqk_launch_zero(const TqkZeroParams &p, hipStream_t st) {
  if (p.n == 0) return hipSuccess;
  uint32_t max_words = 0;
  for (uint32_t i = 0; i < p.n; ++i) max_words = max_words > p.words[i] ? max_words : p.words[i];
  if (max_words == 0) return hipSuccess;
  const uint32_t bx = (max_words / 4u + 2047u) / 2048u;
  hipLaunchKernelGGL(zero_regions_kernel, dim3(bx ? (bx > 256u ? 256u : bx) : 1u, p.n), dim3(256), 0, st, p);
  return hipGetLastError();
}
template <bool PRE>
static void launch_merge_t(const TqkMergeParams &p, int kpl, dim3 grid, dim3 block, hipStream_t st) {
  switch (kpl) {
    case 1: merge_kernel<1, PRE><<<grid, block, 0, st>>>(p); break;
    case 2: merge_kernel<2, PRE><<<grid, block, 0, st>>>(p); break;
    case 4: merge_kernel<4, PRE><<<grid, block, 0, st>>>(p); break;
// ... 39 lines not shown
```

tantivy_amd/csrc/tq_plan_share.cpp:

```cpp
#include "tq_internal.hpp"

namespace tqi {

int build_share_plan(tq_segment *s, Group &g, PlanScratch &ps) {
  static const uint32_t kTaskCost = std::max<uint32_t>(64u, tune_u32("TQ_US_TASK_COST", 2048));
  static const uint32_t kTaskBlocksMax = std::max<uint32_t>(1u, tune_u32("TQ_US_TASK_BLOCKS", 64));
  static const uint32_t kGroupMax = std::min<uint32_t>(TQD_US_GROUP, std::max<uint32_t>(1u, tune_u32("TQ_US_GROUP", TQD_US_GROUP)));
  const size_t nq = g.queries.size();
  g.kpl = kpl_for(g.max_k);
  static const bool ptrace = getenv("TQ_PLAN_TRACE") != nullptr;
  auto pt_last = std::chrono::steady_clock::now();
  auto pt = [&](const char *what) {
    if (!ptrace) return;
    const auto now = std::chrono::steady_clock::now();
    fprintf(stderr, "[tq share plan] %-12s %7.2f ms\n", what, std::chrono::duration<double, std::milli>(now - pt_last).count());
    pt_last = now;
  };
  std::vector<ShareKey> &keys = ps.share_keys;
  {
    std::vector<uint32_t> &rank = ps.term_rank, &distinct = ps.term_distinct;
    if (rank.size() < s->terms.size()) rank.resize(s->terms.size(), 0u);
    distinct.clear();
    size_t n_pairs = 0;
    for (size_t q = 0; q < nq; ++q) {
// ... 297 lines not shown
      if (owner[q] != q) continue;
      const TqdQuery &dq = g.queries[q];
      const uint64_t sig = sigs[q];
      auto bit_of = [&](uint32_t handle) -> uint32_t {
        const uint32_t col = column_of(handle);
        const uint32_t sig1 = !col ? (s->h_dterms[handle].has_freq >> 16) & 0xFFu : 0u;
        return col ? col : (sig1 ? TQD_SIG_SHIFT + (sig1 - 1u) : 0u);
      };
      if (!boolean) {
        TqdALead ld{};
        ld.query = (uint32_t)q;
        ld.w = dq.weight[0];
        float rest = 0.0f;
        uint64_t mask = 0;
        for (uint32_t m = 1; m < dq.n_terms; ++m) {
          rest += dq.weight[m];
          const uint32_t bitpos = bit_of(dq.term[m]);
          if (bitpos) mask |= 1ull << bitpos;
        }
        ld.rest = rest;
        ld.mask_lo = (uint32_t)mask;
        ld.mask_hi = (uint32_t)(mask >> 32);
        ld.info = dq.n_terms | (column_of(dq.term[1]) ? 0x100u : 0u);
        {
          static const bool kUseCls = tune_u32("TQ_AS_CLS", 1) != 0;
          const uint32_t hf = s->h_dterms[dq.term[1]].has_freq;
          if (kUseCls && s->d_doccls && ((hf >> 24) & 1u)) ld.info |= ((hf >> 8) & 0x3Fu) << 10;
        }
        {
          const TermHost &t1 = s->terms[dq.term[1]];
          const bool own = t1.dense_blob && t1.tf8_blob;
          static const bool kUseRdir = tune_u32("TQ_AS_RDIR", 1) != 0;
          if (!own && dq.n_terms == 2u && t1.rdir_blob && s->rdir_span_ok && (kUseRdir || !(t1.probe_dense_blob && t1.probe_tf8_blob))) {
            ld.info |= TQD_AL_RDIR | (t1.rdir_shift << 16);
            ld.dense_off = off_of(t1.rdir_blob);
            ld.tf8_off = off_of(t1.rdir_ent);
          } else {
            ld.dense_off = off_of(own ? t1.dense_blob : t1.probe_dense_blob);
            ld.tf8_off = off_of(own ? t1.tf8_blob : t1.probe_tf8_blob);
          }
        }
        {
          const TermHost &t1 = s->terms[dq.term[1]];
          const float w1 = dq.weight[1];
          float others = 0.0f;
          for (uint32_t m = 2; m < dq.n_terms; ++m) others += dq.weight[m];
          const bool rdir = (ld.info & TQD_AL_RDIR) != 0u;
          ld.excl_lo = kUseRanges && !rdir && t1.rmax_blob ? off_of(t1.rmax_blob) : 0u;
          memcpy(&ld.excl_hi, &w1, sizeof(float));
          memcpy(&ld.any1_lo, &others, sizeof(float));
          ld.any1_hi = (ld.excl_lo || (kUseRanges && rdir)) ? t1.rmax_list : 255u;
        }
        ld.any2_lo = off_of(s->terms[dq.term[0]].lnorm_blob);
        ld.k = dq.k;
        ld.thr_row = dq.thr_index;
        unsorted[lead0[q]] = ld;
        keys[lead0[q]] = ALeadKey{((uint64_t)dq.term[0] << 8) | (uint64_t)(dq.cache_idx & 0xFFu), mask, sig, lead0[q], 0u};
        continue;
      }
      const uint32_t n_lead = std::max<uint32_t>(1u, dq.n_lead);
      for (uint32_t m = 0; m < dq.n_terms; ++m)
      {
        const TermHost &th = s->terms[dq.term[m]];
        const bool own = th.dense_blob && th.tf8_blob;
        if (!own && !(th.probe_dense_blob && th.probe_tf8_blob) && th.rdir_blob && s->rdir_span_ok)
        {
          A.alists[q * TQD_AS_MAX_TERMS + m] = make_uint2(off_of(th.rdir_blob) | th.rdir_shift, off_of(th.rdir_ent));
          any_rdir.store(true, std::memory_order_relaxed);
        } else
          A.alists[q * TQD_AS_MAX_TERMS + m] = make_uint2(off_of(own ? th.dense_blob : th.probe_dense_blob), off_of(own ? th.tf8_blob : th.probe_tf8_blob));
      }
      for (uint32_t li = 0; li < n_lead; ++li) {
        TqdALead ld{};
        ld.query = (uint32_t)q;
        ld.w = dq.weight[li];
        float rest = 0.0f;
        for (uint32_t m = dq.n_terms; m-- > li + 1u;) rest += dq.weight[m];
        uint64_t excl = 0, any[TQ_MAX_TERMS + 1] = {0};
        uint32_t n_any = 0;
        if (li < dq.n_opt_lead) {
          uint64_t m1 = 0;
          for (uint32_t m = dq.n_opt_lead; m < dq.n_lead; ++m) {
            const uint32_t b = bit_of(dq.term[m]);
            m1 = b && m1 != ~0ull ? m1 | (1ull << b) : ~0ull;
          }
          if (m1 != ~0ull && m1) any[n_any++] = m1;
        }
        uint64_t cm = 0;
        for (uint32_t m = 0; m < dq.n_terms; ++m) {
          if (m == li) continue;
          const uint32_t role = (dq.roles >> (2u * m)) & 3u;
          const uint32_t col = column_of(dq.term[m]);
          if (role == TQD_ROLE_MUST_NOT) {
            if (col) excl |= 1ull << col;
          } else if (m < dq.n_lead) {
            if (m < li && col) excl |= 1ull << col;
          } else if (role == TQD_ROLE_MUST) {
            const uint32_t b = bit_of(dq.term[m]);
            cm = b && cm != ~0ull ? cm | (1ull << b) : ~0ull;
            if ((dq.clause_end >> m) & 1u) {
              if (cm != ~0ull && cm) any[n_any++] = cm;
              cm = 0;
            }
          }
        }
        uint64_t bytes = 0;
// ... 295 lines not shown
```

tantivy_amd/csrc/tq_search.cpp:

```cpp
#include "tq_internal.hpp"

namespace tqi {
namespace {

using Clock = std::chrono::steady_clock;

struct Knobs {
  bool use_bshare = tune_u32("TQ_BSHARE", 1) != 0, bs_rdir = tune_u32("TQ_BS_RDIR", 1) != 0;
  bool use_ashare = tune_u32("TQ_ASHARE", 1) != 0;
  uint32_t ashare_min = std::max<uint32_t>(1u, tune_u32("TQ_AS_MIN_LEADS", 1));
  bool use_ushare = tune_u32("TQ_USHARE", 1) != 0;
  uint32_t debug = tune_u32("TQ_DEBUG", 0);
};
const Knobs &knobs() {
  static const Knobs k;
  return k;
}

struct Batch {
  tq_segment *s;
  const tq_query *queries;
  uint32_t n_queries, out_stride;
  float *out_scores;
  uint32_t *out_docs, *out_counts;
  void *hip_stream;
  CallOpts co;
  uint32_t *out_segment_ords;
  uint32_t segment_ord;
  bool replan = false;
  hipStream_t st = nullptr;
  bool exhaustive = false, or_windows = false;
  Clock::time_point t0, t_route, t_routed, t_laid, t_waited, t_filled;
  size_t terms_from = 0, terms_to = 0;
  std::vector<const float *> caches;
  uint32_t n_union_queries = 0, n_bool_queries = 0, n_sparse2 = 0;
  uint32_t n_all_queries = 0;
  const uint8_t *set_q = nullptr;
  const uint32_t *slop_q = nullptr;
  bool and_probe = false, ashare_on = false, ashare_and = false;
  uint32_t and_tile_cap = TQD_AND_TILE, dense_min_queries = 1;
  uint64_t unique_bytes = 0, dense_ratio = 0;
  PlanScratch *ps = nullptr;
  Group *groups = nullptr;
  RouteTotals t;
  int cus = 256;
  size_t part_off_bytes[kNGroups] = {}, partial_bytes = 0;
  struct Copy { size_t off; const void *src; size_t bytes; };
  std::vector<Copy> copies;
  size_t stage = 0, o_caches = 0, o_terms = 0;
  int bx = 0;
  const uint8_t *ds = nullptr;
  DeviceScratch *sc = nullptr;
  int slot = 0;
  uint32_t grid[kNGroups] = {};
};

}

void update_table_span(tq_segment *s) {
  if (s->share_span_terms == s->terms.size()) return;
  uint64_t lo = ~0ull, hi = 0;
  for (const TermHost &th : s->terms)
    for (const void *ptr : {th.dense_blob, th.tf8_blob, th.probe_dense_blob, th.probe_tf8_blob, th.rmax_blob, th.posdir_blob, th.probe_posdir_blob, th.lnorm_blob})
      if (ptr) {
        lo = std::min<uint64_t>(lo, (uint64_t)ptr);
        hi = std::max<uint64_t>(hi, (uint64_t)ptr);
      }
  if (lo == ~0ull) lo = hi = 8;
  {
    uint64_t lo2 = lo, hi2 = hi;
    for (const auto &ch : s->rdir_chunks) {
      lo2 = std::min<uint64_t>(lo2, (uint64_t)ch.first);
      hi2 = std::max<uint64_t>(hi2, (uint64_t)ch.first + ch.second);
    }
    s->rdir_span_ok = !s->rdir_chunks.empty() && hi2 - (lo2 - 8) < (8ull << 32);
    if (s->rdir_span_ok) {
      lo = lo2;
      hi = hi2;
    }
  }
  s->share_table_lo = (lo - 8) & ~255ull;
  s->share_span_ok = hi - s->share_table_lo < (8ull << 32);
  s->share_span_terms = s->terms.size();
}

namespace {

int sync_term_records(Batch &b) {
  HIP_TRY(hipSetDevice(b.s->device));
  b.st = b.hip_stream ? (hipStream_t)b.hip_stream : b.s->stream;
  prep_apply_lmax(b.s, false);
  if (b.s->prep_pending >= 0) {
    if (b.st != b.s->stream) HIP_TRY(hipStreamWaitEvent(b.st, b.s->ev_prep[b.s->prep_pending], 0));
    b.s->prep_pending = -1;
  }
  if (b.s->d_terms_dirty) {
    const size_t n_terms_now = b.s->h_dterms.size();
    if (b.s->d_terms && n_terms_now <= b.s->d_terms_cap && b.s->d_terms_dirty_from >= b.s->d_terms_synced) {
      b.terms_from = std::min(b.s->d_terms_dirty_from, n_terms_now);
      b.terms_to = n_terms_now;
    } else {
      const int rc = sync_terms(b.s, b.st);
      if (rc != TQ_OK) return rc;
    }
  }
  update_table_span(b.s);
  return TQ_OK;
}

void look_at_queries(Batch &b) {
  if (!b.s->plan) b.s->plan = new PlanScratch();
  b.ps = b.s->plan;
  b.ps->q_cache.resize(b.n_queries);
  const size_t n_terms_known = b.s->terms.size();
  const float *last_tc = nullptr;
  uint32_t last_idx = 0;
// ... 148 lines not shown
  b.ashare_on = knobs().use_ashare && !b.exhaustive && b.s->d_docmat && b.s->opt.use_dense && b.s->share_span_ok;
  b.ashare_and = b.ashare_on && !b.co.no_ashare;
  uint64_t and_lead_blocks = 0;
  if (ps.term_stamp.size() < 2 * b.s->terms.size()) ps.term_stamp.resize(2 * b.s->terms.size(), 0u);
  if (++ps.batch_stamp == 0u) {
    std::fill(ps.term_stamp.begin(), ps.term_stamp.end(), 0u);
    ps.batch_stamp = 1u;
  }
  ps.and_lead_count.assign(b.ashare_on ? b.s->terms.size() : 0, 0u);
  ps.q_leader.resize(b.ashare_on ? b.n_queries : 0);
  for (uint32_t qi = 0; qi < b.n_queries; ++qi) {
    const tq_query &q = b.queries[qi];
    if (!q.terms || q.n_terms > TQ_MAX_TERMS) continue;
    uint32_t lead_blocks = 0xFFFFFFFFu;
    for (uint32_t i = 0; i < q.n_terms; ++i) {
      const uint32_t h = q.terms[i];
      if (h >= b.s->terms.size()) continue;
      lead_blocks = std::min(lead_blocks, b.s->terms[h].n_blocks);
      if (ps.term_stamp[2 * h] != ps.batch_stamp) {
        ps.term_stamp[2 * h] = ps.batch_stamp;
        b.unique_bytes += b.s->terms[h].postings_len;
      }
      if (q.mode == TQ_MODE_PHRASE && ps.term_stamp[2 * h + 1] != ps.batch_stamp) {
        ps.term_stamp[2 * h + 1] = ps.batch_stamp;
        b.unique_bytes += b.s->terms[h].positions_len;
      }
    }
    if (q.mode == TQ_MODE_AND && q.n_terms >= 2 && lead_blocks != 0xFFFFFFFFu) and_lead_blocks += lead_blocks;
    if (b.ashare_on) {
      const uint32_t lh = ashare_leader(b, q, ps.q_cache[qi]);
      ps.q_leader[qi] = lh;
      if (lh != 0xFFFFFFFFu) ++ps.and_lead_count[lh];
    }
  }
  if (b.ashare_on) {
    static const uint32_t kMinBatchEnv = tune_u32("TQ_AS_MIN_BATCH", 0xFFFFFFFFu);
    const uint32_t min_batch = kMinBatchEnv != 0xFFFFFFFFu ? kMinBatchEnv : (uint32_t)b.s->opt.ashare_min_batch;
    uint32_t n_el = 0;
    for (uint32_t qi = 0; qi < b.n_queries && n_el < min_batch; ++qi) {
      const uint32_t lh = ps.q_leader[qi];
      if (lh != 0xFFFFFFFFu && ps.and_lead_count[lh] >= knobs().ashare_min) ++n_el;
    }
    b.ashare_and = n_el >= min_batch;
  }
  static const uint32_t kSmallBatchTiles = std::max<uint32_t>(1u, tune_u32("TQ_AND_SMALL_TILES", 2048));
  static const uint32_t kMinTileBlocks = std::min<uint32_t>(TQD_AND_TILE, std::max<uint32_t>(1u, tune_u32("TQ_AND_MIN_TILE", 4)));
  static const uint64_t kSmallBatchBlocks = tune_u32("TQ_AND_SMALL_BLOCKS", 8192);
  b.and_tile_cap = and_lead_blocks < kSmallBatchBlocks
                       ? (uint32_t)std::min<uint64_t>(TQD_AND_TILE, std::max<uint64_t>(kMinTileBlocks, and_lead_blocks / kSmallBatchTiles))
                       : TQD_AND_TILE;
}

void build_leader_norms(Batch &b) {
  if (!b.ashare_and || !b.s->dseg.fieldnorm) return;
  const PlanScratch &ps = *b.ps;
  for (size_t h = 0; h < ps.and_lead_count.size(); ++h)
    if (ps.and_lead_count[h] >= knobs().ashare_min && !b.s->terms[h].lnorm_blob) build_lnorm(b.s, (uint32_t)h, b.st);
  update_table_span(b.s);
}

struct Route {
  TqdQuery dq{};
  int group = kGUnion;
  uint32_t n_tiles = 0, tile_cost = 1;
  uint64_t qbytes = 0;
};

int check_query(const Batch &b, uint32_t qi) {
  const tq_query &q = b.queries[qi];
  if (q.n_terms == 0 || q.n_terms > TQ_MAX_TERMS)
    return fail(TQ_ERR_INVALID, "query %u: n_terms %u not in 1..%u", qi, q.n_terms, TQ_MAX_TERMS);
  if (q.k == 0 || q.k > TQ_MAX_K || q.k > b.out_stride)
    return fail(TQ_ERR_INVALID, "query %u: k %u not in 1..min(%u, out_stride %u)", qi, q.k,
                TQ_MAX_K, b.out_stride);
  if (!q.terms || !q.weights || !q.tf_cache)
    return fail(TQ_ERR_INVALID, "query %u: null terms/weights/tf_cache", qi);
  if (q.mode > TQ_MODE_BOOL) return fail(TQ_ERR_INVALID, "query %u: bad mode", qi);
  if (q.mode == TQ_MODE_BOOL && !q.occurs)
    return fail(TQ_ERR_INVALID, "query %u: TQ_MODE_BOOL needs occurs", qi);
  if (q.mode == TQ_MODE_PHRASE && (q.n_terms < 2 || !q.phrase_offsets))
    return fail(TQ_ERR_INVALID, "query %u: a phrase needs >= 2 terms and offsets", qi);
  if (q.mode == TQ_MODE_PHRASE && q.n_terms > 8)
    return fail(TQ_ERR_UNSUPPORTED, "query %u: device phrases take at most 8 terms", qi);
  for (uint32_t i = 0; i < (q.mode == TQ_MODE_PHRASE ? 1u : q.n_terms); ++i)
    if (!std::isfinite(q.weights[i]))
      return fail(TQ_ERR_INVALID, "query %u: weight %u is not finite", qi, i);
  for (uint32_t i = 0; i < q.n_terms; ++i)
    if (q.terms[i] != TQ_TERM_ABSENT && q.terms[i] != TQ_TERM_ALL && q.terms[i] >= b.s->terms.size())
      return fail(TQ_ERR_INVALID, "query %u: unknown term handle %u", qi, q.terms[i]);
  return TQ_OK;
}

int sort_by_doc_freq(const Batch &b, uint32_t qi, Route &r) {
  const tq_query &q = b.queries[qi];
  const bool phrase = q.mode == TQ_MODE_PHRASE;
  uint32_t order[TQ_MAX_TERMS];
  for (uint32_t i = 0; i < q.n_terms; ++i) order[i] = i;
  small_stable_sort(order, order + q.n_terms, [&](uint32_t x, uint32_t y) {
    return b.s->terms[q.terms[x]].doc_freq < b.s->terms[q.terms[y]].doc_freq;
  });
  uint32_t max_off = 0;
  if (phrase)
    for (uint32_t i = 0; i < q.n_terms; ++i) max_off = std::max(max_off, q.phrase_offsets[i]);
  for (uint32_t i = 0; i < q.n_terms; ++i) {
    const uint32_t src = order[i];
    r.dq.term[i] = q.terms[src];
    r.dq.weight[i] = phrase ? q.weights[0] : q.weights[src];
    r.qbytes += b.s->terms[q.terms[src]].postings_len;
    if (phrase) {
      r.dq.phrase_off[i] = max_off - q.phrase_offsets[src];
      if (b.s->terms[q.terms[src]].positions_len == 0)
// ... 569 lines not shown
  uint8_t *hs = (uint8_t *)b.s->h_stage.p;
  for (const Batch::Copy &c : b.copies) {
    const uint32_t parts = c.bytes >= (1u << 20) ? std::min<uint32_t>(plan_threads(), 4u) : 1u;
    parallel_slabs(parts, [&](uint32_t pi) {
      const size_t x = (c.bytes * pi / parts) & ~(size_t)63, y = pi + 1 == parts ? c.bytes : (c.bytes * (pi + 1) / parts) & ~(size_t)63;
      memcpy(hs + c.off + x, (const uint8_t *)c.src + x, y - x);
    });
  }
  {
    const Group &g = b.groups[kGAShare];
    TqdAQuery *aq = (TqdAQuery *)(hs + g.o_queries);
    TqdQuery *xq = (TqdQuery *)(hs + g.o_xqueries);
    uint32_t n_ext = 0;
    for (size_t q = 0; q < g.queries.size(); ++q) {
      const TqdQuery &dq = g.queries[q];
      TqdAQuery r{};
      r.part_start = dq.part_start;
      r.chunk_first = dq.chunk_first;
      r.k = dq.k;
      r.term1 = dq.term[1];
      r.n_terms = dq.n_terms;
      r.ext = 0xFFFFFFFFu;
      if (dq.n_terms > 2u) {
        if (n_ext == b.t.n_ashare_ext) return fail(TQ_ERR_INVALID, "shared intersections: more queries of three and more lists than were routed");
        r.ext = n_ext;
        xq[n_ext++] = dq;
      }
      aq[q] = r;
    }
  }
  for (int gi = 0; gi < kNGroups; ++gi) {
    const Group &g = b.groups[gi];
    if (g.queries.empty()) continue;
    TqkSinks sk{};
    sk.partials = (uint64_t *)((uint8_t *)b.sc->partials.p + b.part_off_bytes[gi]);
    sk.match_counter = b.s->d_match_counter;
    sk.query_matches = (uint32_t *)b.s->d_qmatches.p;
    sk.out_index = (const uint32_t *)(b.ds + g.o_outidx);
    memcpy(hs + g.o_sinks, &sk, sizeof sk);
  }
  b.t_filled = Clock::now();
  return TQ_OK;
}

int order_batch(Batch &b) {
  b.slot = (int)(b.s->batches_timed % tq_segment::kTimingRing);
  const int rc = order_after_last_batch(b.s, b.st);
  if (rc != TQ_OK) return rc;
  if (b.sc->in_flight && b.sc->last_stream != b.st) HIP_TRY(hipStreamWaitEvent(b.st, b.sc->ev_last, 0));
  if (b.s->opt.timing) HIP_TRY(hipEventRecord(b.s->ev_t0[b.slot], b.st));
  return TQ_OK;
}

int enqueue_copy(Batch &b) {
  if (b.s->buf_used[b.bx]) HIP_TRY(hipStreamWaitEvent(b.s->copy_stream, b.s->ev_buf_free[b.bx], 0));
  HIP_TRY(hipMemcpyAsync((void *)b.ds, b.s->h_stage.p, b.stage, hipMemcpyHostToDevice, b.s->copy_stream));
  HIP_TRY(hipEventRecord(b.s->ev_stage_done, b.s->copy_stream));
  HIP_TRY(hipEventRecord(b.s->ev_copy_done[b.bx], b.s->copy_stream));
  HIP_TRY(hipStreamWaitEvent(b.st, b.s->ev_copy_done[b.bx], 0));
  b.s->stage_in_flight = true;
  if (b.terms_to > b.terms_from) {
    HIP_TRY(hipMemcpyAsync(b.s->d_terms + b.terms_from, b.ds + b.o_terms, (b.terms_to - b.terms_from) * sizeof(TqdTerm),
                           hipMemcpyDeviceToDevice, b.st));
    b.s->d_terms_dirty = false;
    b.s->d_terms_dirty_from = ~(size_t)0;
    b.s->d_terms_synced = b.terms_to;
  }
  return TQ_OK;
}

DevBuf &list_words(tq_segment *s, int gi) {
  return gi == kGAShare ? s->d_ashare_words : gi == kGBShare ? s->d_bshare_words : s->d_share_words;
}
DevBuf &list_stage(DeviceScratch &sc, int gi) {
  return gi == kGAShare ? sc.ashare_stage : gi == kGBShare ? sc.bshare_stage : sc.share_stage;
}

int zero_batch_buffers(Batch &b) {
  TqkZeroParams zp{};
  auto zero_later = [&](void *ptr, size_t bytes) -> int {
    if (!bytes) return TQ_OK;
    if (zp.n == (uint32_t)TQK_ZERO_MAX || (bytes & 3u) || ((uintptr_t)ptr & 3u) || bytes > 0xFFFFFFFFull * 4u) {
      HIP_TRY(hipMemsetAsync(ptr, 0, bytes, b.st));
      return TQ_OK;
    }
    zp.ptr[zp.n] = (uint32_t *)ptr;
    zp.words[zp.n++] = (uint32_t)(bytes >> 2);
    return TQ_OK;
  };
  int rc = zero_later(b.s->d_match_counter, sizeof(unsigned long long));
  if (rc == TQ_OK) rc = zero_later(b.s->d_qmatches.p, (size_t)b.n_queries * sizeof(uint32_t));
  if (rc != TQ_OK) return rc;
  b.s->last_batch_queries = b.n_queries;
  b.s->last_batch_slop = !b.groups[kGSlop].queries.empty();
  b.s->slop_over_words = b.n_queries;
  if (b.s->last_batch_slop) {
    rc = b.s->d_slop_over.ensure((size_t)b.n_queries * sizeof(uint32_t));
    if (rc == TQ_OK) rc = zero_later(b.s->d_slop_over.p, (size_t)b.n_queries * sizeof(uint32_t));
    if (rc != TQ_OK) return rc;
  }
  if (b.t.n_thr_rows) {
    const size_t thr_bytes = (size_t)b.t.n_thr_rows * TQD_THR_SLOTS * sizeof(uint32_t);
    rc = b.s->d_thr.ensure(thr_bytes);
    if (rc == TQ_OK) rc = zero_later(b.s->d_thr.p, thr_bytes);
    if (rc != TQ_OK) return rc;
  }
// ... 409 lines not shown
    if (all_based) {
      for (uint32_t i = 0; i < q.n_terms; ++i) {
        const bool must_not = q.mode == TQ_MODE_BOOL && q.occurs && q.occurs[i] == TQ_MUST_NOT;
        if (is_term_set(s, q.terms[i]) && !must_not)
          return fail(TQ_ERR_UNSUPPORTED, "tq_search_batch: query %u: a term set as a Should clause beside a match-all clause stays on the CPU (its counts and doc sets are taken)", qi);
        if (names_field && term_field_of(s, q.terms[i]) && !must_not)
          return fail(TQ_ERR_UNSUPPORTED, "tq_search_batch: query %u: a Should term of field %u (the scoring terms of a query whose match-all clauses make every doc a candidate are its Should terms) stays on the CPU (its counts and doc sets are taken)", qi, term_field_of(s, q.terms[i]));
      }
      continue;
    }
    if (!(names_set && query_names_set(s, q)) && !(names_field && query_names_field(s, q))) continue;
    if (st.set_q.empty()) st.set_q.assign(n_queries, 0);
    st.set_q[qi] = 1;
    ++st.n_set;
    if (q.mode == TQ_MODE_BOOL) continue;
    if (st.eff.empty()) st.eff.assign(queries, queries + n_queries);
    st.set_occurs.emplace_back();
    st.set_occurs.back().fill(q.mode == TQ_MODE_AND ? (uint8_t)TQ_MUST : (uint8_t)TQ_SHOULD);
    tq_query &v = st.eff[qi];
    v.mode = TQ_MODE_BOOL;
    v.occurs = st.set_occurs.back().data();
    v.clause_of = v.nested_occurs = v.clause_min_should = v.atom_of = nullptr;
    v.min_should_match = 0;
  }
  return TQ_OK;
}

size_t host_rows_layout(uint32_t n_queries, uint32_t out_stride, size_t &o_docs, size_t &o_counts) {
  const size_t n = (size_t)n_queries * out_stride;
  o_docs = (n * sizeof(float) + 255) & ~(size_t)255;
  o_counts = (o_docs + n * sizeof(uint32_t) + 255) & ~(size_t)255;
  return o_counts + (size_t)n_queries * sizeof(uint32_t);
}

}

int search_batch_impl(tq_segment *s, const tq_query *queries, uint32_t n_queries,
                      uint32_t out_stride, float *d_out_scores, uint32_t *d_out_docs,
                      uint32_t *d_out_counts, void *hip_stream, const CallOpts &co, uint32_t *d_out_segment_ords,
                      uint32_t segment_ord) {
  if (!s || (!queries && n_queries) || !d_out_scores || !d_out_docs || !d_out_counts)
    return fail(TQ_ERR_INVALID, "tq_search_batch: null argument");
  if (n_queries == 0) return TQ_OK;
  AllStrip strip;
  int rc = strip_all_clauses(s, queries, n_queries, strip);
  if (rc != TQ_OK) return rc;
  if (!strip.eff.empty()) queries = strip.eff.data();
  Batch b{s, queries, n_queries, out_stride, d_out_scores, d_out_docs, d_out_counts, hip_stream, co, d_out_segment_ords, segment_ord};
  b.n_all_queries = strip.n_all_based;
  b.set_q = strip.n_set ? strip.set_q.data() : nullptr;
  b.slop_q = strip.slop_q.empty() ? nullptr : strip.slop_q.data();
  rc = plan_batch(b);
  while (rc != TQ_OK && b.replan) {
    b = Batch{s, queries, n_queries, out_stride, d_out_scores, d_out_docs, d_out_counts, hip_stream, b.co, d_out_segment_ords, segment_ord};
    b.n_all_queries = strip.n_all_based;
    b.set_q = strip.n_set ? strip.set_q.data() : nullptr;
    b.slop_q = strip.slop_q.empty() ? nullptr : strip.slop_q.data();
    rc = plan_batch(b);
  }
  if (rc != TQ_OK) return rc;
  b.sc = s->dscratch;
  std::unique_lock<std::mutex> scratch_lock(b.sc->m);
  if ((rc = lay_out_stage(b)) != TQ_OK || (rc = fill_stage(b)) != TQ_OK || (rc = order_batch(b)) != TQ_OK) return rc;
  DrainOnError drain_on_error{s, b.st};
  if ((rc = enqueue_copy(b)) != TQ_OK || (rc = zero_batch_buffers(b)) != TQ_OK || (rc = launch_groups(b)) != TQ_OK ||
      (rc = launch_merges(b)) != TQ_OK || (rc = finish_batch(b)) != TQ_OK)
    return rc;
  drain_on_error.armed = false;
  s->host_ms_sum += std::chrono::duration<double, std::milli>((Clock::now() - b.t0) - (b.t_waited - b.t_laid)).count();
  ++s->host_ms_n;
  return TQ_OK;
}

int resolve_opts(const tq_segment *s, const tq_search_opts *o, CallOpts &co) {
  co.exhaustive = __atomic_load_n(&s->opt.exhaustive, __ATOMIC_RELAXED) != 0;
  uint32_t ppm = (uint32_t)__atomic_load_n(&s->opt.bound_slack_ppm, __ATOMIC_RELAXED);
  if (o) {
    if (o->exhaustive == 0 || o->exhaustive == 1)
      co.exhaustive = o->exhaustive != 0;
    else if (o->exhaustive != -1)
      return fail(TQ_ERR_INVALID, "tq_search_opts.exhaustive must be -1, 0 or 1");
    if (o->bound_slack_ppm != TQ_OPT_DEFAULT) ppm = o->bound_slack_ppm;
    if (ppm > 1000000000u) return fail(TQ_ERR_INVALID, "bound_slack_ppm above 1e9");
  }
  co.bound_slack = 1.0f + (float)ppm * 1e-6f;
  return TQ_OK;
}

int search_batch_host(tq_segment *s, const tq_query *queries, uint32_t n_queries,
                      uint32_t out_stride, float *out_scores, uint32_t *out_docs,
                      uint32_t *out_counts, const CallOpts &co) {
  if (!s || !out_scores || !out_docs || !out_counts)
    return fail(TQ_ERR_INVALID, "tq_search_batch: null argument");
  if (n_queries == 0) return TQ_OK;
  HIP_TRY(hipSetDevice(s->device));
  const size_t n = (size_t)n_queries * out_stride;
  size_t o_docs, o_counts;
  const size_t o_over = (host_rows_layout(n_queries, out_stride, o_docs, o_counts) + 255) & ~(size_t)255;
  int rc = s->h_out.ensure(o_over + (size_t)n_queries * sizeof(uint32_t));
  if (rc != TQ_OK) return rc;
  uint8_t *h = (uint8_t *)s->h_out.p;
  CallOpts co_over = co;
  co_over.h_slop_over = (uint32_t *)(h + o_over);
  rc = search_batch_impl(s, queries, n_queries, out_stride, (float *)h, (uint32_t *)(h + o_docs),
                         (uint32_t *)(h + o_counts), nullptr, co_over);
  if (rc != TQ_OK) return rc;
  HIP_TRY(hipStreamSynchronize(s->stream));
  memcpy(out_scores, h, n * sizeof(float));
  memcpy(out_docs, h + o_docs, n * sizeof(uint32_t));
  memcpy(out_counts, h + o_counts, (size_t)n_queries * sizeof(uint32_t));
  if (co.defer_slop_verdict) {
    if (s->last_batch_slop) s->slop_over_host.assign((const uint32_t *)(h + o_over), (const uint32_t *)(h + o_over) + n_queries);
    return TQ_OK;
  }
  return s->last_batch_slop ? slop_overflow_verdict("tq_search_batch", (const uint32_t *)(h + o_over), n_queries) : TQ_OK;
}
// ... 104 lines not shown
```

tantivy_amd/csrc/tq_term_tables.cpp:

```cpp
#include "tq_internal.hpp"

namespace tqi {

size_t rdir_dir_words(const tq_segment *s, uint32_t S) { return (((size_t)(s->max_doc >> S) + 2u) + 3u) & ~(size_t)3u; }
size_t rdir_bytes(const tq_segment *s, uint32_t doc_freq, uint32_t S) {
  return (rdir_dir_words(s, S) + (size_t)doc_freq) * sizeof(uint32_t);
}
uint32_t rdir_plan(tq_segment *s, uint32_t doc_freq) {
  static const uint32_t kRatio = tune_u32("TQ_RDIR_RATIO", 0);
  static const uint32_t kMinDf = std::max<uint32_t>(1u, tune_u32("TQ_RDIR_MIN_DF", 256));
  if (!s->opt.dense || s->opt.rdir_budget_x <= 0 || s->max_doc < 4096u || doc_freq < kMinDf) return 0u;
  if (kRatio && (uint64_t)doc_freq * kRatio >= s->max_doc) return 0u;
  static const uint32_t kPerRange = std::max<uint32_t>(1u, tune_u32("TQ_RDIR_PER_RANGE", 1));
  uint32_t S = 2;
  while (S < 16u && (s->max_doc >> S) + 1u > doc_freq / kPerRange) ++S;
  if (s->rdir_bytes_total + rdir_bytes(s, doc_freq, S) > s->rdir_budget()) return 0u;
  return S;
}
int attach_rdir(tq_segment *s, uint32_t handle, uint32_t S, void **tab) {
  TermHost &t = s->terms[handle];
  const int rc = rdir_alloc(s, rdir_bytes(s, t.doc_freq, S), tab);
  if (rc != TQ_OK) return rc;
  t.rdir_blob = *tab;
  t.rdir_ent = (uint32_t *)*tab + rdir_dir_words(s, S);
// ... 103 lines not shown
}

int build_flat(tq_segment *s, uint32_t handle, hipStream_t st, bool *ok) {
  TermHost &t = s->terms[handle];
  *ok = t.flat_blob != nullptr;
  if (*ok || t.doc_freq == 0) return TQ_OK;
  const size_t doc_bytes = ((size_t)t.doc_freq * sizeof(uint32_t) + 15) & ~(size_t)15;
  const size_t bytes = doc_bytes + (((size_t)t.doc_freq + 15) & ~(size_t)15);
  if (s->dense_bytes_total + bytes > s->dense_budget()) return TQ_OK;
  void *blob = nullptr;
  {
    const int arc = dense_alloc(s, bytes + PAD, &blob);
    if (arc != TQ_OK) return arc;
  }
  const hipError_t e = tqk_launch_flat_list(s->dseg, t.d_self, 0u, t.n_blocks, (uint32_t *)blob,
                                            (uint8_t *)blob + doc_bytes, st);
  if (e != hipSuccess) {
    dense_release(s, blob);
    return fail(TQ_ERR_HIP, "flat list: %s", hipGetErrorString(e));
  }
  t.flat_blob = blob;
  s->dense_bytes_total += bytes;
  s->bytes_bitmaps += bytes;
  *ok = true;
  return TQ_OK;
}

void build_lnorm(tq_segment *s, uint32_t handle, hipStream_t st) {
  TermHost &t = s->terms[handle];
  if (t.lnorm_blob || s->lnorm_off || !t.n_blocks || !t.d_self || !s->dseg.fieldnorm || t.field) return;
  const size_t bytes = (size_t)t.n_blocks * 128u;
  if (s->dense_bytes_total + bytes > s->dense_budget()) return;
  void *blob = nullptr;
  if (dense_alloc(s, bytes + PAD, &blob) != TQ_OK) {
    (void)hipGetLastError();
    return;
  }
  if ((uint64_t)blob < s->share_table_lo + 8u || (uint64_t)blob + bytes - s->share_table_lo >= (8ull << 32)) {
    dense_release(s, blob);
    s->lnorm_off = true;
    return;
  }
  if (tqk_launch_lead_norms(s->dseg, t.d_self, 0u, t.n_blocks, (uint8_t *)blob, st) != hipSuccess) {
    (void)hipGetLastError();
    dense_release(s, blob);
    return;
  }
  t.lnorm_blob = blob;
  s->dense_bytes_total += bytes;
  s->bytes_bitmaps += bytes;
  s->share_span_terms = ~(size_t)0;
}

int ensure_docmat(tq_segment *s) {
  if (s->d_docmat) return TQ_OK;
  const size_t mat_bytes = (size_t)s->max_doc * sizeof(uint64_t);
  if (s->dense_bytes_total + mat_bytes > s->dense_budget()) return TQ_OK;
  HIP_TRY(hipMalloc((void **)&s->d_docmat, mat_bytes + PAD));
  HIP_TRY(hipMemsetAsync((uint8_t *)s->d_docmat + mat_bytes, 0, PAD, s->stream));
  const hipError_t e = tqk_launch_docmat_init(s->d_docmat, s->d_fn, s->dseg.const_fieldnorm_id, s->max_doc, s->stream);
  if (e != hipSuccess) return fail(TQ_ERR_HIP, "docmat init: %s", hipGetErrorString(e));
  s->dense_bytes_total += mat_bytes;
  s->bytes_docmat = mat_bytes;
  s->dseg.docmat = s->d_docmat;
  return TQ_OK;
}

int add_to_doc_signatures(tq_segment *s, uint32_t handle) {
  TermHost &t = s->terms[handle];
  if (t.doc_freq == 0) return TQ_OK;
  const bool has_col = ((s->h_dterms[handle].has_freq >> 8) & 0xFFu) != 0u;
  bool want_sig = s->opt.docsig && s->opt.docmat && s->opt.dense && s->max_doc >= 4096u && !has_col;
  const uint32_t rd_shift = !(t.dense_blob && t.tf8_blob) && !t.rdir_blob ? rdir_plan(s, t.doc_freq) : 0u;
  if (want_sig) {
    const int rc = ensure_docmat(s);
    if (rc != TQ_OK) return rc;
    want_sig = s->d_docmat != nullptr;
  }
  if (!want_sig && !rd_shift) return TQ_OK;
  DecodedList dl;
  int rc = decode_list(s, t, 0, false, dl);
  if (rc != TQ_OK) return rc;
  hipError_t e = hipSuccess;
  if (want_sig) {
    const uint32_t bit = sig_bit(handle);
    e = tqk_launch_docmat_set(s->d_docmat, dl.dd, t.doc_freq, (TQD_SIG_SHIFT - 8u) + bit, s->max_doc, s->stream);
    if (e != hipSuccess) return fail(TQ_ERR_HIP, "docmat signature: %s", hipGetErrorString(e));
    s->h_dterms[handle].has_freq |= (bit + 1u) << 16;
    mark_term_dirty(s, handle);
  }
  if (rd_shift) {
    void *tab = nullptr;
    rc = attach_rdir(s, handle, rd_shift, &tab);
    if (rc != TQ_OK) return rc;
    e = tqk_launch_rdir_fill(dl.dd, dl.dt, t.doc_freq, s->max_doc, (uint32_t *)tab, rd_shift, s->stream);
    if (e != hipSuccess) {
      t.rdir_blob = t.rdir_ent = nullptr, t.rdir_shift = 0;
      return fail(TQ_ERR_HIP, "range directory: %s", hipGetErrorString(e));
    }
    if (s->d_local_cache && !t.field) {
      uint32_t *acc = dl.dt + t.doc_freq + 8u, lmax = 0;
      e = hipMemsetAsync(acc, 0, sizeof(uint32_t), s->stream);
      if (e == hipSuccess) e = tqp_launch_list_max(dl.dd, dl.dt, t.doc_freq, s->d_fn, s->dseg.const_fieldnorm_id, s->d_local_cache, acc, s->stream);
      if (e == hipSuccess) e = hipMemcpyAsync(&lmax, acc, 4, hipMemcpyDeviceToHost, s->stream);
      if (e == hipSuccess) e = hipStreamSynchronize(s->stream);
      if (e != hipSuccess) return fail(TQ_ERR_HIP, "list maximum: %s", hipGetErrorString(e));
      if (lmax) t.rmax_list = std::min<uint32_t>(lmax, 255u);
    }
  }
  return TQ_OK;
}

int build_dense_device(tq_segment *s, uint32_t handle) {
  TermHost &t = s->terms[handle];
  const size_t n_words = bitmap_words(s);
  DecodedList dl;
  int rc = decode_list(s, t, tqp_scan_scratch_words((uint32_t)std::max<size_t>(n_words, (size_t)t.doc_freq / 4 + 2)), true, dl);
  if (rc != TQ_OK) return rc;
  uint32_t *const dd = dl.dd, *const dt = dl.dt;
  rc = build_tf8(s, handle, dt);
  if (rc != TQ_OK) return rc;
  if (t.tf8_blob) {
    rc = build_rmax(s, handle, dl);
    if (rc != TQ_OK) return rc;
  }
  void *blob = nullptr;
  {
    const int arc = dense_alloc(s, n_words * sizeof(uint2), &blob);
    if (arc != TQ_OK) return arc;
  }
  s->bytes_bitmaps += n_words * sizeof(uint2);
  ++s->n_dense_lists;
  uint32_t h_bad = 0;
  hipError_t e = enqueue_bitmap(s, dl, t.doc_freq, blob);
  if (e == hipSuccess) e = finish_tables(s, dl, &h_bad, nullptr);
  if (e != hipSuccess || h_bad) {
    dense_release(s, blob);
    return e != hipSuccess ? fail(TQ_ERR_HIP, "dense tables: %s", hipGetErrorString(e))
                           : fail(TQ_ERR_FORMAT, "posting list not strictly increasing below max_doc");
  }
  t.dense_blob = blob;
  s->h_dterms[handle].dense = (const uint2 *)blob;
  mark_term_dirty(s, handle);
  if (s->n_mat_slots < TQD_MAT_SLOTS && s->opt.docmat && t.wants_col) {
    {
      const int mrc = ensure_docmat(s);
      if (mrc != TQ_OK) return mrc;
    }
    if (s->d_docmat) {
      const uint32_t slot = s->n_mat_slots++;
      e = tqk_launch_docmat_set(s->d_docmat, dd, t.doc_freq, slot, s->max_doc, s->stream);
      if (e != hipSuccess) return fail(TQ_ERR_HIP, "docmat set: %s", hipGetErrorString(e));
      static const bool kDocCls = tune_u32("TQ_DOCCLS", 1) != 0;
      if (kDocCls && slot < TQD_CLS_SLOTS && t.tf8_blob) {
        const size_t cls_bytes = (size_t)s->max_doc * sizeof(uint64_t);
        if (!s->d_doccls && s->dense_bytes_total + cls_bytes <= s->dense_budget()) {
          HIP_TRY(hipMalloc((void **)&s->d_doccls, cls_bytes + PAD));
          HIP_TRY(hipMemsetAsync(s->d_doccls, 0, cls_bytes + PAD, s->stream));
          s->dense_bytes_total += cls_bytes;
          s->bytes_docmat += cls_bytes;
          s->dseg.doccls = s->d_doccls;
        }
        if (s->d_doccls) {
          e = tqk_launch_doccls_set(s->d_doccls, dd, dt, t.doc_freq, slot, s->max_doc, s->stream);
          if (e != hipSuccess) return fail(TQ_ERR_HIP, "doccls set: %s", hipGetErrorString(e));
          s->h_dterms[handle].has_freq |= 1u << 24;
        }
      }
      s->h_dterms[handle].has_freq |= (slot + 1u) << 8;
    }
  }
  if (t.positions_len > 0) {
    const size_t n_dir = ((size_t)t.doc_freq + 3) / 4 + 1;
    const size_t dir_bytes = (n_dir * sizeof(uint32_t) + PAD + 15) & ~(size_t)15;
    const size_t n_bits = (n_words + 255) & ~(size_t)255;
    void *db = nullptr;
    {
      const int arc = dense_alloc(s, dir_bytes + n_bits * sizeof(uint32_t) + PAD, &db);
      if (arc != TQ_OK) return arc;
    }
    e = tqp_launch_posdir(dt, t.doc_freq, (uint32_t *)db, (uint32_t)n_dir, dl.scan_scratch, s->stream);
    if (e == hipSuccess)
      e = tqp_launch_bits((const uint2 *)blob, (uint32_t)n_words, (uint32_t *)((uint8_t *)db + dir_bytes), (uint32_t)n_bits, s->stream);
    uint32_t total = 0;
    if (e == hipSuccess)
      e = hipMemcpyAsync(&total, (uint32_t *)db + (n_dir - 1), 4, hipMemcpyDeviceToHost, s->stream);
    if (e == hipSuccess) e = hipStreamSynchronize(s->stream);
    if (e != hipSuccess || total != (uint32_t)t.n_positions) {
      dense_release(s, db);
      return e != hipSuccess ? fail(TQ_ERR_HIP, "position directory: %s", hipGetErrorString(e))
                             : fail(TQ_ERR_FORMAT, "term freqs sum to %u positions, the stream holds %llu",
                                    total, (unsigned long long)t.n_positions);
    }
    t.posdir_blob = db;
    s->h_dterms[handle].pos_dir = (const uint32_t *)db;
    s->h_dterms[handle].bits = (const uint32_t *)((uint8_t *)db + dir_bytes);
    s->dense_bytes_total += n_dir * sizeof(uint32_t) + n_bits * sizeof(uint32_t);
    s->bytes_posdir += n_dir * sizeof(uint32_t) + n_bits * sizeof(uint32_t);
  }
  HIP_TRY(hipStreamSynchronize(s->stream));
  return TQ_OK;
}

// ... 2 lines not shown
```

tantivy_amd/csrc/tq_terms.cpp:

```cpp
#include "tq_internal.hpp"

namespace tqi {

uint32_t add_term(tq_segment *s, const TqdTerm &dt, const TermHost &th, uint64_t postings_off) {
  const uint32_t handle = (uint32_t)s->terms.size();
  s->terms.push_back(th);
  s->terms.back().wants_col = !s->cols_reserved || s->reserved_cols.count(postings_off) != 0;
  s->h_dterms.push_back(dt);
  if (s->prep_field) {
    s->terms.back().field = s->prep_field;
    s->terms.back().wants_col = !s->cols_reserved;
    s->h_dterms.back().has_freq |= (uint32_t)s->prep_field << 26;
    ++s->n_field_terms;
  }
  mark_term_dirty(s, handle);
  s->term_by_off.emplace(postings_off, handle);
  return handle;
}

int register_term(tq_segment *s, const TqdTerm &dt, const TermHost &th, uint64_t postings_off, tq_term_handle *out) {
  const uint32_t handle = add_term(s, dt, th, postings_off);
  *out = handle;
  if (dense_candidate(s, th.doc_freq) && dense_fits(s)) {
    s->dense_bytes_total += dense_table_bytes(s);
// ... 355 lines not shown
    const uint32_t handle = add_term(s, w.dt, w.th, w.postings_off);
    b.out[b.walked_of[k]] = handle;
    if (!w.th.doc_freq) continue;
    const bool sig = sigs && s->d_docmat;
    const uint32_t S = rdir_plan(s, w.th.doc_freq);
    void *tab = nullptr;
    if (S && attach_rdir(s, handle, S, &tab) != TQ_OK) {
      (void)hipGetLastError();
      tab = nullptr;
    }
    if (tab) b.any_tab = true;
    if (!sig && !tab) continue;
    const uint32_t bit = sig_bit(handle);
    h_selfs[b.n_sig++] = w.th.d_self;
    b.tabs.push_back((uint32_t *)tab);
    b.bits.push_back(sig ? bit : 0xFFFFFFFFu);
    b.shifts.push_back(tab ? S : 0u);
    b.dfs.push_back(w.th.doc_freq);
    s->prep_lmax_handles[b.bx].push_back(handle);
    if (sig) s->h_dterms[handle].has_freq |= (bit + 1u) << 16;
  }
  if (b.n_sig) {
    const size_t n_sig = b.n_sig;
    uint8_t *at = (uint8_t *)(h_selfs + n_sig);
    memcpy(at, b.tabs.data(), n_sig * sizeof(uint32_t *));
    at += n_sig * sizeof(uint32_t *);
    for (const std::vector<uint32_t> *arr : {&b.bits, &b.shifts, &b.dfs}) {
      memcpy(at, arr->data(), n_sig * sizeof(uint32_t));
      at += n_sig * sizeof(uint32_t);
    }
    memset(at, 0, n_sig * sizeof(uint32_t));
  }
  b.t4 = Clock::now();
  return TQ_OK;
}

int enqueue_upload(PrepareBatch &b) {
  tq_segment *s = b.s;
  const uint32_t bx = b.bx, n_sig = b.n_sig;
  hipStream_t cs = s->copy_stream ? s->copy_stream : s->stream;
  hipError_t e = hipSuccess;
  if (cs != s->stream) {
    if (!s->ev_prep_order) e = hipEventCreateWithFlags(&s->ev_prep_order, hipEventDisableTiming);
    if (e == hipSuccess) e = hipEventRecord(s->ev_prep_order, s->stream);
    if (e == hipSuccess) e = hipStreamWaitEvent(cs, s->ev_prep_order, 0);
  }
  if (e == hipSuccess) e = hipMemcpyAsync(b.region, b.hs, b.stage_bytes + b.ptr_bytes, hipMemcpyHostToDevice, cs);
  bool lmax_pending = false;
  if (e == hipSuccess && n_sig) {
    const TqdTerm **d_selfs = (const TqdTerm **)(b.region + b.stage_bytes);
    uint32_t *const *d_tabs = (uint32_t *const *)(d_selfs + n_sig);
    const uint32_t *d_bits = (const uint32_t *)(d_tabs + n_sig);
    uint32_t *d_lmax = (uint32_t *)(d_bits + 3 * n_sig);
    e = tqk_launch_docsig_batch(s->dseg, d_selfs, d_bits, n_sig, s->d_docmat, b.any_tab ? d_tabs : nullptr, d_bits + n_sig,
                                d_bits + 2 * n_sig, s->d_local_cache, d_lmax, s->opt.use_dpp != 0, cs);
    if (e == hipSuccess && b.any_tab && s->d_local_cache) {
      uint32_t *h_lmax = (uint32_t *)(b.hs + b.stage_bytes + b.ptr_bytes);
      e = hipMemcpyAsync(h_lmax, d_lmax, (size_t)n_sig * sizeof(uint32_t), hipMemcpyDeviceToHost, cs);
      s->prep_lmax_host[bx] = h_lmax;
      lmax_pending = true;
    }
  }
  if (!lmax_pending) s->prep_lmax_handles[bx].clear();
  if (e == hipSuccess) e = hipEventRecord(s->ev_prep[bx], cs);
  if (e == hipSuccess && cs != s->stream) e = hipStreamWaitEvent(s->stream, s->ev_prep[bx], 0);
  if (e != hipSuccess) return fail(TQ_ERR_HIP, "term upload: %s", hipGetErrorString(e));
  s->prep_used[bx] = true;
  s->prep_pending = (int)bx;
  return TQ_OK;
}

void resolve_repeats(PrepareBatch &b) {
  for (uint32_t i : b.fresh)
    if (b.out[i] == TQ_TERM_ABSENT) {
      auto it = b.s->term_by_off.find(b.infos[i].postings_off);
      if (it != b.s->term_by_off.end()) b.out[i] = it->second;
    }
}
}

int tqi::term_prepare_batch_shifted(tq_segment *s, const tq_term_info *infos, uint32_t n, tq_term_handle *out, uint8_t field) {
  PrepareBatch b{s, infos, n, out};
  {
    TQ_SEGMENT_LOCK(s);
    resolve_known(b);
  }
  if (b.fresh.empty()) return TQ_OK;
  static const bool trace = getenv("TQ_TRACE") != nullptr;
  b.trace = trace;
  b.t0 = b.t1 = b.t2 = b.t3 = b.t4 = Clock::now();
  if (!s->device_prepare()) prewalk(b);
  b.t1 = Clock::now();
  TQ_SEGMENT_LOCK(s);
  FieldScope field_scope(s, field);
  b.t2 = b.t3 = b.t4 = Clock::now();
  HIP_TRY(hipSetDevice(s->device));
  if (s->device_prepare()) {
    for (uint32_t i : b.fresh) {
      const int rc = prepare_one(b, i);
      if (rc != TQ_OK) return rc;
    }
    return TQ_OK;
  }
  int rc = classify_and_walk(b);
  if (rc == TQ_OK && !b.walked.empty()) {
    rc = stage_blobs(b);
// ... 14 lines not shown
```

tantivy_amd/host/searcher.cpp:

```cpp
#include "searcher.hpp"

#include "term_info_store.hpp"

#include <algorithm>
#include <cmath>
#include <cstring>

namespace tantivy_amd {

namespace {
[[noreturn]] void throw_tq(int code) {
  const std::string msg = tq_last_error();
  switch (code) {
    case TQ_ERR_INVALID: throw TantivyError(TantivyError::InvalidArgument, msg);
    case TQ_ERR_FORMAT: throw TantivyError(TantivyError::DataCorruption, msg);
    case TQ_ERR_UNSUPPORTED: throw TantivyError(TantivyError::Unsupported, msg);
    default: throw TantivyError(TantivyError::SystemError, msg);
  }
}
}

SegmentReader::SegmentReader(tq_ctx *ctx, int device, uint32_t segment_ord, uint32_t max_doc,
                             uint8_t record_option, const uint8_t *idx, size_t idx_len,
                             const uint8_t *pos, size_t pos_len, const uint8_t *fieldnorm,
// ... 487 lines not shown
              w.nested_occurs.push_back((uint8_t)TQ_MUST);
              w.atom_of.push_back(member);
            }
          }
        } else if (c.second.kind == Query::Term) {
          add(c.second.term, bc, Occur::Must);
        } else if (c.second.kind == Query::Phrase) {
          add_phrase(c.second, bc, Occur::Must);
        } else {
          for (auto &sub : c.second.clauses) {
            if (sub.second.kind == Query::Term)
              add(sub.second.term, bc * sub.second.boost, sub.first);
            else if (sub.second.kind == Query::Phrase)
              add_phrase(sub.second, bc * sub.second.boost, sub.first);
            else if (is_member_union(sub.second))
              for (auto &leaf : sub.second.clauses) add(leaf.second.term, bc * sub.second.boost * leaf.second.boost, sub.first, TQ_NESTED_ANY);
            else
              for (auto &leaf : sub.second.clauses) add(leaf.second.term, bc * sub.second.boost * leaf.second.boost, sub.first);
            ++member;
          }
          if (tree && c.second.minimum_number_should_match) {
            if (clause >= TQ_MAX_TERMS || c.second.minimum_number_should_match > 255)
              throw TantivyError(TantivyError::Unsupported, "nested minimum_number_should_match out of range");
            if (w.clause_min_should.empty()) w.clause_min_should.assign(TQ_MAX_TERMS, 0);
            w.clause_min_should[clause] = (uint8_t)c.second.minimum_number_should_match;
          }
        }
        ++clause;
      }
      if (w.terms.size() > TQ_MAX_TERMS)
        throw TantivyError(TantivyError::Unsupported, "more than 16 terms stay on the CPU");
      if (any_phrase) w.phrase_offsets.resize(w.terms.size(), 0u);
      w.min_should_match = (uint32_t)std::min<size_t>(msm, 0xFFFFu);
      return w;
    }
  }
  throw TantivyError(TantivyError::InvalidArgument, "unknown query kind");
}

namespace {
struct SegmentBatch {
  std::vector<tq_query> qs;
  std::vector<tq_term_handle> handles;
  SegmentBatch() = default;
  SegmentBatch(const std::shared_ptr<SegmentReader> &seg_p, const std::vector<Weight> &weights, uint32_t k) { fill(seg_p, weights, k); }
  void fill(const std::shared_ptr<SegmentReader> &seg_p, const std::vector<Weight> &weights, uint32_t k) {
    SegmentReader &seg = *seg_p;
    const size_t n = weights.size();
    qs.resize(n);
    size_t total_terms = 0;
    for (auto &w : weights) total_terms += w.terms.size();
    handles.clear();
    handles.reserve(total_terms);
    if (n > 1) {
      std::vector<uint32_t> fresh;
      for (auto &w : weights)
        for (uint32_t t : w.terms)
          if (t < kTermSetBase && !seg.handle_known(t)) fresh.push_back(t);
      if (!fresh.empty()) seg.prepare_terms(fresh.data(), fresh.size());
    }
    for (size_t i = 0; i < n; ++i) {
      const Weight &w = weights[i];
      const size_t at = handles.size();
      for (uint32_t t : w.terms) handles.push_back(resolve_handle(seg_p, w, t));
      tq_query &q = qs[i];
      q.n_terms = (uint32_t)w.terms.size();
      q.terms = handles.data() + at;
      q.weights = w.weights.data();
      q.tf_cache = w.bm25->tf_cache();
      q.mode = w.mode;
      q.phrase_offsets = w.phrase_offsets.empty() ? nullptr : w.phrase_offsets.data();
      q.k = k;
      q.occurs = w.occurs.empty() ? nullptr : w.occurs.data();
      q.clause_of = w.clause_of.empty() ? nullptr : w.clause_of.data();
      q.min_should_match = w.min_should_match;
      q.slop = w.slop;
      q.nested_occurs = w.nested_occurs.empty() ? nullptr : w.nested_occurs.data();
      q.clause_min_should = w.clause_min_should.empty() ? nullptr : w.clause_min_should.data();
      q.atom_of = w.atom_of.empty() ? nullptr : w.atom_of.data();
    }
  }
};
}

struct Searcher::DeviceBatch {
  std::mutex m;
  SegmentBatch b;
};

Searcher::Searcher(std::vector<std::shared_ptr<SegmentReader>> segments)
    : segments_(std::move(segments)), device_batch_(new DeviceBatch()) {
  for (auto &s : segments_) n_fields_ = std::max(n_fields_, s->num_fields());
}
Searcher::~Searcher() { delete[] fast_weights_.load(std::memory_order_relaxed); }

uint32_t Searcher::bound_slack_ppm(const SegmentReader &seg) const {
  const double global = (double)total_num_tokens() / (double)total_num_docs();
  const double local = seg.max_doc() ? (double)seg.total_num_tokens() / (double)seg.max_doc() : global;
  double ppm = 0.0;
  if (global > 0.0 && local > 0.0 && global != local) {
    const double d = std::abs(global - local) / std::min(global, local);
    ppm = std::ceil(((1.0 + d) * (1.0 + d) - 1.0) * 1e6) + 2.0;
  }
  return (uint32_t)std::min(ppm, 1e9);
}

void Searcher::collect_segment_batch(size_t segment_ord, const std::vector<Weight> &weights,
                                     uint32_t k, std::vector<float> &scores,
                                     std::vector<uint32_t> &docs, std::vector<uint32_t> &counts) {
  SegmentReader &seg = *segments_[segment_ord];
  const size_t n = weights.size();
  SegmentBatch b(segments_[segment_ord], weights, k);
  scores.assign(n * k, 0.0f);
  docs.assign(n * k, TERMINATED);
  counts.assign(n, 0);
  const tq_search_opts opts{-1, bound_slack_ppm(seg)};
  const int rc = tq_search_batch_opts(seg.raw(), b.qs.data(), (uint32_t)n, k, scores.data(),
                                      docs.data(), counts.data(), &opts);
  if (rc != TQ_OK) throw_tq(rc);
}

std::vector<uint64_t> Searcher::count_batch(const std::vector<Weight> &weights) {
  std::vector<uint64_t> total(weights.size(), 0);
  std::vector<uint32_t> per(weights.size());
  for (auto &seg : segments_) {
    SegmentBatch b(seg, weights, 1);
    const int rc = tq_count_batch(seg->raw(), b.qs.data(), (uint32_t)weights.size(), per.data());
    if (rc != TQ_OK) throw_tq(rc);
    for (size_t i = 0; i < per.size(); ++i) total[i] += per[i];
  }
  return total;
}

// ... 143 lines not shown
```

tantivy_amd/host/searcher.hpp:

```cpp
#pragma once
#include <atomic>
#include <memory>
#include <mutex>
#include <stdexcept>
#include <string>
#include <unordered_map>
#include <utility>
#include <vector>

#include "../../include/tantivy_amd.h"
#include "bm25.hpp"

namespace tantivy_amd {

struct TantivyError : std::runtime_error {
  enum Kind { InvalidArgument, SchemaError, SystemError, DataCorruption, Unsupported } kind;
  TantivyError(Kind k, const std::string &msg) : std::runtime_error(msg), kind(k) {}
};

struct TermInfo {
  uint32_t doc_freq = 0;
  uint64_t postings_start = 0, postings_end = 0;
  uint64_t positions_start = 0, positions_end = 0;
};

struct DocAddress {
  uint32_t segment_ord = 0;
  DocId doc_id = 0;
  bool operator==(const DocAddress &o) const {
    return segment_ord == o.segment_ord && doc_id == o.doc_id;
  }
};

class SegmentReader {
 public:
  SegmentReader(tq_ctx *ctx, int device, uint32_t segment_ord, uint32_t max_doc, uint8_t record_option,
                const tq_field_files *fields, uint32_t n_fields);
  SegmentReader(tq_ctx *ctx, int device, uint32_t segment_ord, uint32_t max_doc,
                uint8_t record_option, const uint8_t *idx, size_t idx_len, const uint8_t *pos,
                size_t pos_len, const uint8_t *fieldnorm, size_t fn_len);
  struct DeviceResident {};
  SegmentReader(DeviceResident, tq_ctx *ctx, int device, uint32_t segment_ord, uint32_t max_doc,
                uint8_t record_option, const uint8_t *d_idx, size_t idx_len, const uint8_t *d_pos,
                size_t pos_len, const uint8_t *d_fieldnorm, size_t fn_len, uint64_t total_num_tokens);
  ~SegmentReader();
  SegmentReader(const SegmentReader &) = delete;
  SegmentReader &operator=(const SegmentReader &) = delete;

  void add_term(uint32_t term_id, const TermInfo &info, uint32_t field = 0);
  uint32_t term_field(uint32_t term_id) const;
  uint32_t num_fields() const { return n_fields_; }
  void set_term_info_store(std::shared_ptr<const class TermInfoStore> store);
  const TermInfo *get_term_info(uint32_t term_id) const;
  tq_term_handle term_handle(uint32_t term_id);
  void prepare_terms(const uint32_t *term_ids, size_t n);
  bool handle_known(uint32_t term_id) const;
  uint32_t max_doc() const { return max_doc_; }
  uint32_t segment_ord() const { return segment_ord_; }
  uint64_t total_num_tokens(uint32_t field = 0) const { return field < n_fields_ ? total_num_tokens_[field] : 0; }
  uint8_t record_option() const { return record_option_; }
  tq_segment *raw() const { return seg_; }

 private:
  tq_segment *seg_ = nullptr;
  uint32_t segment_ord_, max_doc_;
  uint8_t record_option_;
  uint32_t n_fields_ = 1;
  uint64_t total_num_tokens_[TQ_MAX_FIELDS] = {};
  std::unordered_map<uint32_t, uint8_t> term_field_;
  mutable std::mutex m_;
  mutable std::unordered_map<uint32_t, TermInfo> terms_;
  std::unordered_map<uint32_t, tq_term_handle> handles_;
  static constexpr uint32_t kFastHandles = 1u << 20;
  static constexpr tq_term_handle kHandleUnknown = 0xFFFFFFFEu;
  std::atomic<std::atomic<tq_term_handle> *> fast_handles_{nullptr};
  std::shared_ptr<const class TermInfoStore> store_;
};

enum class Occur { Should, Must, MustNot };

struct Query {
  enum Kind { Term, Boolean, Phrase, All, TermSet } kind;
  uint32_t term = 0;
  std::vector<uint32_t> set_terms;
  std::vector<std::pair<Occur, Query>> clauses;
  size_t minimum_number_should_match = 0;
  Score boost = 1.0f;
  std::vector<std::pair<uint32_t, uint32_t>> phrase_terms;
  uint32_t slop = 0;

  static Query term_query(uint32_t term) {
    Query q;
    q.kind = Term;
    q.term = term;
    return q;
  }
  static Query all() {
    Query q;
    q.kind = All;
    return q;
  }
  static Query term_set(std::vector<uint32_t> term_ids) {
    Query q;
    q.kind = TermSet;
    q.set_terms = std::move(term_ids);
    return q;
  }
  static Query boolean(std::vector<std::pair<Occur, Query>> clauses) {
    Query q;
    q.kind = Boolean;
    q.clauses = std::move(clauses);
    return q;
  }
  Query &boosted(Score b) {
    boost *= b;
    return *this;
  }
  Query &set_minimum_number_should_match(size_t n) {
    minimum_number_should_match = n;
    return *this;
  }
  static Query phrase(const std::vector<uint32_t> &terms, uint32_t slop = 0) {
    Query q;
    q.kind = Phrase;
    for (uint32_t i = 0; i < terms.size(); ++i) q.phrase_terms.emplace_back(i, terms[i]);
    q.slop = slop;
    return q;
// ... 210 lines not shown
```

Baseline: 11.88 million queries/s.

## Precompute per-leader docmat words in block order and prefetch them into LDS

Adds a per-term table that stores, in posting-block order, the doc-matrix words for each lead term's documents. The AND/BM25 kernel then reads them with the prefetch into LDS (or a coalesced load) instead of doing random gathers into the docmat array per candidate. Epoch tracking invalidates and refills a table whenever the docmat changes. Eligible terms are limited by a doc_freq cut and a memory budget, and the change costs extra memory plus a fill kernel per new lead. It also adds a host fast path that resolves query term handles from the lock-free handle table before falling back to the slower resolution.

```diff
diff --git a/include/tantivy_amd.h b/include/tantivy_amd.h
--- a/include/tantivy_amd.h
+++ b/include/tantivy_amd.h
@@ -228,6 +228,7 @@
   TQ_TABLE_PROBE_DENSE = 14,
   TQ_TABLE_PROBE_TF8 = 15,
   TQ_TABLE_PROBE_POS_DIR = 16,
+  TQ_TABLE_LMAT = 17,
   TQ_TABLE_DOCMAT = 32,
   TQ_TABLE_DOCCLS = 33,
   TQ_TABLE_LOCAL_CACHE = 34,
@@ -439,6 +440,9 @@
   uint32_t n_terms, n_dense_lists, n_docmat_columns;
   uint32_t probe_evictions;
   uint64_t device_scratch_bytes;
+  uint64_t lead_mat_bytes;
+  uint32_t lead_mat_stale;
+  uint32_t pad_;
 } tq_segment_stats;
 int tq_segment_get_stats(tq_segment *seg, tq_segment_stats *out);
 int tq_set_option(tq_segment *seg, const char *name, int64_t value);
diff --git a/tantivy_amd/binding.py b/tantivy_amd/binding.py
--- a/tantivy_amd/binding.py
+++ b/tantivy_amd/binding.py
@@ -96,7 +96,8 @@
         "index_bytes", "positions_bytes", "fieldnorm_bytes", "alive_bytes", "term_table_bytes",
         "bitmap_bytes", "docmat_bytes", "posdir_bytes", "scratch_bytes", "dense_budget_bytes")] + [
         (n, C.c_uint32) for n in ("n_terms", "n_dense_lists", "n_docmat_columns", "probe_evictions")] + [
-        ("device_scratch_bytes", C.c_uint64)]
+        ("device_scratch_bytes", C.c_uint64), ("lead_mat_bytes", C.c_uint64), ("lead_mat_stale", C.c_uint32),
+        ("pad_", C.c_uint32)]
 
 
 class TqTermInfo(C.Structure):
@@ -180,7 +181,7 @@
     "pos_blk": (4, np.uint64), "pos_tail": (5, np.uint32), "dense": (6, np.uint32), "bits": (7, np.uint32),
     "pos_dir": (8, np.uint32), "tf8": (9, np.uint8), "rmax": (10, np.uint8), "rdir": (11, np.uint32),
     "lnorm": (12, np.uint8), "flat": (13, np.uint8), "probe_dense": (14, np.uint32), "probe_tf8": (15, np.uint8),
-    "probe_pos_dir": (16, np.uint32),
+    "probe_pos_dir": (16, np.uint32), "lmat": (17, np.uint64),
     "docmat": (32, np.uint64), "doccls": (33, np.uint64), "local_cache": (34, np.float32), "min_fieldnorm_id": (35, np.uint32),
 }
 
@@ -1327,7 +1328,7 @@
         _check(lib().tq_segment_get_stats(self.segment_raw(segment_ord), C.byref(st)))
         out = {n: int(getattr(st, n)) for n, _ in TqSegmentStats._fields_}
         out["derived_bytes"] = (out["term_table_bytes"] + out["bitmap_bytes"] + out["docmat_bytes"]
-                                + out["posdir_bytes"])
+                                + out["posdir_bytes"] + out["lead_mat_bytes"])
         out["tantivy_bytes"] = (out["index_bytes"] + out["positions_bytes"] + out["fieldnorm_bytes"]
                                 + out["alive_bytes"])
         return out
diff --git a/tantivy_amd/csrc/tq_api.cpp b/tantivy_amd/csrc/tq_api.cpp
--- a/tantivy_amd/csrc/tq_api.cpp
+++ b/tantivy_amd/csrc/tq_api.cpp
@@ -541,6 +541,8 @@
   r.n_docmat_columns = s->n_mat_slots;
   r.probe_evictions = (uint32_t)std::min<uint64_t>(s->probe_evictions, 0xFFFFFFFFull);
   r.dense_budget_bytes = s->dense_budget();
+  r.lead_mat_bytes = s->lmat_bytes_total;
+  r.lead_mat_stale = s->lmat_stale_skips;
   *out = r;
   return TQ_OK;
 }
@@ -562,6 +564,10 @@
     s->opt.dense_ratio = (int)value;
   else if (!strcmp(name, "rdir_budget_x") && value >= 0 && value <= 0x7FFFFFFF)
     s->opt.rdir_budget_x = (int)value;
+  else if (!strcmp(name, "lead_mat_budget_x") && value >= 0 && value <= 0x7FFFFFFF)
+    s->opt.lead_mat_budget_x = (int)value;
+  else if (!strcmp(name, "lead_mat_cut") && value >= 1 && value <= 0x7FFFFFFF)
+    s->opt.lead_mat_cut = (int)value;
   else if (!strcmp(name, "probe_budget_x") && value >= 0 && value <= 0x7FFFFFFF)
     s->opt.probe_budget_x = (int)value, s->probe_full = false;
   else if (!strcmp(name, "dense_budget_x") && value >= 0)
@@ -694,6 +700,7 @@
     case TQ_TABLE_RMAX: span(list ? t.rmax_blob : nullptr, tqd_rm_level_off(s->max_doc, TQD_RM_LEVELS)); return true;
     case TQ_TABLE_RDIR: span(list ? t.rdir_blob : nullptr, t.rdir_shift ? rdir_bytes(s, t.doc_freq, t.rdir_shift) : 0); return true;
     case TQ_TABLE_LNORM: span(list ? t.lnorm_blob : nullptr, (size_t)t.n_blocks * 128u); return true;
+    case TQ_TABLE_LMAT: span(list && lmat_valid(s, t) ? t.lmat_blob : nullptr, (size_t)t.n_blocks * 1024u); return true;
     case TQ_TABLE_FLAT:
       span(list ? t.flat_blob : nullptr, (((size_t)t.doc_freq * sizeof(uint32_t) + 15) & ~(size_t)15) + t.doc_freq);
       return true;
diff --git a/tantivy_amd/csrc/tq_ashare.hip b/tantivy_amd/csrc/tq_ashare.hip
--- a/tantivy_amd/csrc/tq_ashare.hip
+++ b/tantivy_amd/csrc/tq_ashare.hip
@@ -19,7 +19,7 @@
 namespace {
 
 constexpr uint32_t AS_GROUP = TQD_AS_GROUP;
-constexpr uint32_t AS_COUNTER_BITS = 0x7FE0u | 0xF00000u | 0x40000000u;
+constexpr uint32_t AS_COUNTER_BITS = 0x7FE0u | 0xF00000u | 0x40000000u | 0x20000000u;
 
 template <bool BOOLQ>
 struct AShareLds {
@@ -32,6 +32,7 @@
   uint32_t flen[AS_GROUP];
   float bw[BOOLQ ? AS_GROUP * TQD_AS_MAX_TERMS : 1];
   uint32_t pay[(TQ_AS_PREFETCH && !BOOLQ) ? 260 : 1];
+  alignas((TQ_AS_PREFETCH && !BOOLQ) ? 16 : 4) uint32_t mat[(TQ_AS_PREFETCH && !BOOLQ) ? 256 : 1];
 };
 
 template <int R>
@@ -369,6 +370,11 @@
     auto norm_pair = [&](uint32_t j) __attribute__((always_inline)) -> uint32_t {
       return reinterpret_cast<const uint16_t *>(tbase + ((uint64_t)lnorm << 3))[(size_t)j * 64u + (uint32_t)lane];
     };
+    uint32_t lmat = 0;
+    if constexpr (!BOOLQ) lmat = sload(&p.leads[lead0].any2_hi);
+    auto mat_pair = [&](uint32_t j) __attribute__((always_inline)) -> uint4 {
+      return reinterpret_cast<const uint4 *>(tbase + ((uint64_t)lmat << 3))[(size_t)j * 64u + (uint32_t)lane];
+    };
     if (ci != cache_loaded) {
       const float *cg = p.caches + (size_t)ci * 256u;
       wave_mem_fence();
@@ -535,6 +541,9 @@
         if (!PF || !rest) return;
         const uint32_t nb2 = (uint32_t)__builtin_ctzll(rest);
         if (lnorm) npair_next = norm_pair(i_base + nb2);
+        if (lmat)
+          __builtin_amdgcn_global_load_lds((const __attribute__((address_space(1))) void *)(tbase + ((uint64_t)lmat << 3) + (size_t)(i_base + nb2) * 1024u + 16u * (uint32_t)lane),
+                                           (__attribute__((address_space(3))) void *)L.mat, 16, 0, 0);
         const uint32_t meta = (uint32_t)__builtin_amdgcn_readlane((int)rec_mine.y, (int)nb2);
         const uint32_t off = (uint32_t)__builtin_amdgcn_readlane((int)rec_mine.z, (int)nb2);
         if (meta == META_TAIL) return;
@@ -578,10 +587,13 @@
           n_scored += 16u + (mo_l.x == META_TAIL ? 8u * lead.n_tail : 16u * ((mo_l.x & 31u) + (lead.has_freq ? (mo_l.x >> 8) & 0xFFu : 0u)));
         uint32_t c0, c1, t0, t1;
         uint32_t npair = 0;
+        uint4 mpair = make_uint4(0u, 0u, 0u, 0u);
         if constexpr (PF) {
         npair = npair_next;
         if (mo_l.x == META_TAIL) {
           asm volatile("s_waitcnt vmcnt(0)" ::: "memory");
+          wave_mem_fence();
+          if (lmat) mpair = *reinterpret_cast<const uint4 *>(&L.mat[4u * (uint32_t)lane]);
           decode_docs<USE_DPP>(idx, lead, mo_l, prev_l, lane, c0, c1);
           decode_tfs(idx, lead, mo_l, lane, t0, t1);
         } else {
@@ -590,6 +602,7 @@
           const uint32_t tf_bits = lead.has_freq ? (mo_l.x >> 8) & 0xFFu : 0u;
           asm volatile("s_waitcnt vmcnt(0)" ::: "memory");
           wave_mem_fence();
+          if (lmat) mpair = *reinterpret_cast<const uint4 *>(&L.mat[4u * (uint32_t)lane]);
           if (lead.has_freq) {
             unpack2_lds(L.pay + 4u * doc_bits, tf_bits, lane, t0, t1);
             t0 += strict;
@@ -602,10 +615,12 @@
           unpack2_lds(L.pay, doc_bits, lane, x0, x1);
           finish_docs<USE_DPP>(x0, x1, strict, prev_l, lane, c0, c1);
         }
+        asm volatile("s_waitcnt lgkmcnt(0)" : "+v"(mpair.x), "+v"(mpair.y), "+v"(mpair.z), "+v"(mpair.w) : : "memory");
         wave_mem_fence();
         prefetch(todo);
         } else {
         if (lnorm) npair = norm_pair(i_base + b);
+        if (lmat) mpair = mat_pair(i_base + b);
         decode_docs<USE_DPP>(idx, lead, mo_l, prev_l, lane, c0, c1);
         decode_tfs(idx, lead, mo_l, lane, t0, t1);
         }
@@ -633,11 +648,18 @@
         const float tfn0 = f0 * __builtin_amdgcn_rcpf(f0 + L.cache[nid0]);
         const float tfn1 = f1 * __builtin_amdgcn_rcpf(f1 + L.cache[nid1]);
         const bool g0 = v0 && tfn0 >= block_need, g1 = v1 && tfn1 >= block_need;
-        const uint64_t mw0 = g0 ? seg.docmat[c0] : 0ull;
-        const uint64_t mw1 = g1 ? seg.docmat[c1] : 0ull;
+        uint64_t mw0, mw1;
+        if (lmat) {
+          mw0 = g0 ? (uint64_t)mpair.x | ((uint64_t)mpair.y << 32) : 0ull;
+          mw1 = g1 ? (uint64_t)mpair.z | ((uint64_t)mpair.w << 32) : 0ull;
+        } else {
+          mw0 = g0 ? seg.docmat[c0] : 0ull;
+          mw1 = g1 ? seg.docmat[c1] : 0ull;
+        }
         const uint64_t valid0 = __ballot(g0), valid1 = __ballot(g1);
         if (p.debug & 0x200000u) n_scored += (uint32_t)(__popcll(__ballot(v0)) + __popcll(__ballot(v1)));
         if (p.debug & 0x400000u) n_scored += (uint32_t)(__popcll(valid0) + __popcll(valid1));
+        if ((p.debug & 0x20000000u) && !lmat) n_scored += (uint32_t)(__popcll(valid0) + __popcll(valid1));
         if (TQ_AS_TIMERS && tphase == 5u && (uint32_t)mw0 == 0xFFFFFFFEu) ++n_scored;
         te(5u);
         tb(6u);
diff --git a/tantivy_amd/csrc/tq_internal.hpp b/tantivy_amd/csrc/tq_internal.hpp
--- a/tantivy_amd/csrc/tq_internal.hpp
+++ b/tantivy_amd/csrc/tq_internal.hpp
@@ -104,6 +104,8 @@
   uint32_t rmax_list = 255;
   void *flat_blob = nullptr;
   void *lnorm_blob = nullptr;
+  void *lmat_blob = nullptr;
+  uint64_t lmat_epoch = 0;
   uint32_t doc_freq = 0, n_blocks = 0, n_full = 0, n_tail = 0;
   uint32_t last_doc = 0;
   bool wants_col = true;
@@ -161,6 +163,8 @@
   int bound_slack_ppm = 0;
   int xunion_ratio = 64;
   int xunion_min_queries = 64;
+  int lead_mat_budget_x = 4;
+  int lead_mat_cut = 16;
   int rdir_budget_x = 4;
   int probe_budget_x = 16;
   int count_bitmap_ratio = 128;
@@ -301,6 +305,10 @@
   uint64_t share_table_lo = 0;
   bool share_span_ok = true;
   bool lnorm_off = false;
+  uint64_t docmat_epoch = 1, docmat_epoch_planned = 0;
+  size_t lmat_bytes_total = 0;
+  bool lmat_off = false;
+  uint32_t lmat_stale_skips = 0;
   uint32_t last_batch_queries = 0;
   DevBuf d_slop_over;
   bool last_batch_slop = false;
@@ -776,6 +784,20 @@
 int build_dense_device(tq_segment *s, uint32_t handle);
 int build_flat(tq_segment *s, uint32_t handle, hipStream_t st, bool *ok);
 void build_lnorm(tq_segment *s, uint32_t handle, hipStream_t st);
+inline void docmat_written(tq_segment *s) { ++s->docmat_epoch; }
+inline int lead_mat_budget_x(const tq_segment *s) {
+  static const uint32_t kEnv = tune_u32("TQ_LEAD_MAT_BUDGET_X", 0xFFFFFFFFu);
+  return kEnv != 0xFFFFFFFFu ? (int)std::min<uint32_t>(kEnv, 0x7FFFFFFFu) : s->opt.lead_mat_budget_x;
+}
+inline uint32_t lead_mat_cut(const tq_segment *s) {
+  static const uint32_t kEnv = tune_u32("TQ_LEAD_MAT_CUT", 0);
+  return kEnv ? kEnv : (uint32_t)std::max(1, s->opt.lead_mat_cut);
+}
+inline bool lmat_valid(const tq_segment *s, const TermHost &t) {
+  return t.lmat_blob && t.lmat_epoch == s->docmat_epoch && lead_mat_budget_x(s) > 0;
+}
+bool plan_lmat(tq_segment *s, uint32_t handle, bool *fill);
+hipError_t fill_lmat(tq_segment *s, uint32_t handle, hipStream_t st);
 void prep_apply_lmax(tq_segment *s, bool wait);
 int build_probe_tables(tq_segment *s, uint32_t handle, bool *ok, bool must = false);
 int build_probe_posdir(tq_segment *s, uint32_t handle, bool *ok);
diff --git a/tantivy_amd/csrc/tq_launch.h b/tantivy_amd/csrc/tq_launch.h
--- a/tantivy_amd/csrc/tq_launch.h
+++ b/tantivy_amd/csrc/tq_launch.h
@@ -541,6 +541,8 @@
                                 uint32_t n_blocks, uint32_t *docs, uint8_t *tf8, hipStream_t st);
 hipError_t tqk_launch_lead_norms(const TqdSegment &seg, const TqdTerm *terms, uint32_t handle, uint32_t n_blocks,
                                  uint8_t *out, hipStream_t st);
+hipError_t tqk_launch_lead_mat(const TqdSegment &seg, const TqdTerm *terms, uint32_t handle, uint32_t n_blocks,
+                               uint64_t *out, hipStream_t st);
 hipError_t tqk_launch_decode_list(const TqdSegment &seg, const TqdTerm *terms, uint32_t handle,
                                   uint32_t n_blocks, uint32_t *docs, uint32_t *tfs, bool use_dpp,
                                   hipStream_t st);
diff --git a/tantivy_amd/csrc/tq_misc.hip b/tantivy_amd/csrc/tq_misc.hip
--- a/tantivy_amd/csrc/tq_misc.hip
+++ b/tantivy_amd/csrc/tq_misc.hip
@@ -256,6 +256,18 @@
   reinterpret_cast<uint16_t *>(out)[j * 64u + (uint32_t)lane] = (uint16_t)(n0 | (n1 << 8));
 }
 
+__global__ __launch_bounds__(256) void lead_mat_kernel(TqdSegment seg, const TqdTerm *terms, uint32_t handle, uint64_t *out) {
+  const int lane = (int)__lane_id();
+  const uint32_t wave = uni(threadIdx.x >> 6);
+  const TermRef t = load_term(terms, handle);
+  const uint32_t j = blockIdx.x * 4u + wave;
+  if (j >= t.n_blocks) return;
+  uint32_t d0, d1;
+  decode_docs<true>(uni_ptr(seg.idx), t, uni_mo(t, j), block_prev_last(t, j), lane, d0, d1);
+  const uint64_t w0 = d0 < seg.max_doc ? seg.docmat[d0] : 0ull, w1 = d1 < seg.max_doc ? seg.docmat[d1] : 0ull;
+  reinterpret_cast<ulonglong2 *>(out)[(size_t)j * 64u + (uint32_t)lane] = make_ulonglong2(w0, w1);
+}
+
 }
 
 hipError_t tqk_launch_tf8_pack(const uint32_t *tfs, uint32_t n, uint8_t *out, hipStream_t st) {
@@ -267,6 +279,12 @@
                                  uint8_t *out, hipStream_t st) {
   if (n_blocks == 0 || !seg.fieldnorm) return hipSuccess;
   hipLaunchKernelGGL(lead_norms_kernel, dim3((n_blocks + 3) / 4), dim3(256), 0, st, seg, terms, handle, out);
+  return hipGetLastError();
+}
+hipError_t tqk_launch_lead_mat(const TqdSegment &seg, const TqdTerm *terms, uint32_t handle, uint32_t n_blocks,
+                               uint64_t *out, hipStream_t st) {
+  if (n_blocks == 0 || !seg.docmat) return hipSuccess;
+  hipLaunchKernelGGL(lead_mat_kernel, dim3((n_blocks + 3) / 4), dim3(256), 0, st, seg, terms, handle, out);
   return hipGetLastError();
 }
 hipError_t tqk_launch_docmat_init(uint64_t *mat, const uint8_t *fieldnorm, uint32_t const_id,
diff --git a/tantivy_amd/csrc/tq_plan_share.cpp b/tantivy_amd/csrc/tq_plan_share.cpp
--- a/tantivy_amd/csrc/tq_plan_share.cpp
+++ b/tantivy_amd/csrc/tq_plan_share.cpp
@@ -373,6 +373,7 @@
           ld.any1_hi = (ld.excl_lo || (kUseRanges && rdir)) ? t1.rmax_list : 255u;
         }
         ld.any2_lo = off_of(s->terms[dq.term[0]].lnorm_blob);
+        ld.any2_hi = lmat_valid(s, s->terms[dq.term[0]]) ? off_of(s->terms[dq.term[0]].lmat_blob) : 0u;
         ld.k = dq.k;
         ld.thr_row = dq.thr_index;
         unsorted[lead0[q]] = ld;
diff --git a/tantivy_amd/csrc/tq_search.cpp b/tantivy_amd/csrc/tq_search.cpp
--- a/tantivy_amd/csrc/tq_search.cpp
+++ b/tantivy_amd/csrc/tq_search.cpp
@@ -53,6 +53,7 @@
   DeviceScratch *sc = nullptr;
   int slot = 0;
   uint32_t grid[kNGroups] = {};
+  std::vector<uint32_t> lmat_fill;
 };
 
 }
@@ -61,7 +62,7 @@
   if (s->share_span_terms == s->terms.size()) return;
   uint64_t lo = ~0ull, hi = 0;
   for (const TermHost &th : s->terms)
-    for (const void *ptr : {th.dense_blob, th.tf8_blob, th.probe_dense_blob, th.probe_tf8_blob, th.rmax_blob, th.posdir_blob, th.probe_posdir_blob, th.lnorm_blob})
+    for (const void *ptr : {th.dense_blob, th.tf8_blob, th.probe_dense_blob, th.probe_tf8_blob, th.rmax_blob, th.posdir_blob, th.probe_posdir_blob, th.lnorm_blob, th.lmat_blob})
       if (ptr) {
         lo = std::min<uint64_t>(lo, (uint64_t)ptr);
         hi = std::max<uint64_t>(hi, (uint64_t)ptr);
@@ -316,11 +317,20 @@
 }
 
 void build_leader_norms(Batch &b) {
-  if (!b.ashare_and || !b.s->dseg.fieldnorm) return;
-  const PlanScratch &ps = *b.ps;
-  for (size_t h = 0; h < ps.and_lead_count.size(); ++h)
-    if (ps.and_lead_count[h] >= knobs().ashare_min && !b.s->terms[h].lnorm_blob) build_lnorm(b.s, (uint32_t)h, b.st);
-  update_table_span(b.s);
+  tq_segment *s = b.s;
+  s->lmat_stale_skips = 0;
+  if (b.ashare_and) {
+    const PlanScratch &ps = *b.ps;
+    const bool norms = s->dseg.fieldnorm != nullptr;
+    for (size_t h = 0; h < ps.and_lead_count.size(); ++h) {
+      if (ps.and_lead_count[h] < knobs().ashare_min) continue;
+      if (norms && !s->terms[h].lnorm_blob) build_lnorm(s, (uint32_t)h, b.st);
+      bool fill = false;
+      if (plan_lmat(s, (uint32_t)h, &fill) && fill) b.lmat_fill.push_back((uint32_t)h);
+    }
+    update_table_span(s);
+  }
+  s->docmat_epoch_planned = s->docmat_epoch;
 }
 
 struct Route {
@@ -996,6 +1006,22 @@
   return TQ_OK;
 }
 
+void drop_leader_mats(Batch &b) {
+  for (uint32_t h : b.lmat_fill) b.s->terms[h].lmat_epoch = 0;
+  b.lmat_fill.clear();
+}
+int fill_leader_mats(Batch &b) {
+  for (uint32_t h : b.lmat_fill) {
+    const hipError_t e = fill_lmat(b.s, h, b.st);
+    if (e != hipSuccess) {
+      drop_leader_mats(b);
+      return fail(TQ_ERR_HIP, "leader doc-matrix words: %s", hipGetErrorString(e));
+    }
+  }
+  b.lmat_fill.clear();
+  return TQ_OK;
+}
+
 int enqueue_copy(Batch &b) {
   if (b.s->buf_used[b.bx]) HIP_TRY(hipStreamWaitEvent(b.s->copy_stream, b.s->ev_buf_free[b.bx], 0));
   HIP_TRY(hipMemcpyAsync((void *)b.ds, b.s->h_stage.p, b.stage, hipMemcpyHostToDevice, b.s->copy_stream));
@@ -1511,16 +1537,21 @@
   b.slop_q = strip.slop_q.empty() ? nullptr : strip.slop_q.data();
   rc = plan_batch(b);
   while (rc != TQ_OK && b.replan) {
+    drop_leader_mats(b);
     b = Batch{s, queries, n_queries, out_stride, d_out_scores, d_out_docs, d_out_counts, hip_stream, b.co, d_out_segment_ords, segment_ord};
     b.n_all_queries = strip.n_all_based;
     b.set_q = strip.n_set ? strip.set_q.data() : nullptr;
     b.slop_q = strip.slop_q.empty() ? nullptr : strip.slop_q.data();
     rc = plan_batch(b);
   }
+  struct DropMats {
+    Batch &b;
+    ~DropMats() { drop_leader_mats(b); }
+  } drop_mats{b};
   if (rc != TQ_OK) return rc;
   b.sc = s->dscratch;
   std::unique_lock<std::mutex> scratch_lock(b.sc->m);
-  if ((rc = lay_out_stage(b)) != TQ_OK || (rc = fill_stage(b)) != TQ_OK || (rc = order_batch(b)) != TQ_OK) return rc;
+  if ((rc = lay_out_stage(b)) != TQ_OK || (rc = fill_stage(b)) != TQ_OK || (rc = order_batch(b)) != TQ_OK || (rc = fill_leader_mats(b)) != TQ_OK) return rc;
   DrainOnError drain_on_error{s, b.st};
   if ((rc = enqueue_copy(b)) != TQ_OK || (rc = zero_batch_buffers(b)) != TQ_OK || (rc = launch_groups(b)) != TQ_OK ||
       (rc = launch_merges(b)) != TQ_OK || (rc = finish_batch(b)) != TQ_OK)
diff --git a/tantivy_amd/csrc/tq_term_tables.cpp b/tantivy_amd/csrc/tq_term_tables.cpp
--- a/tantivy_amd/csrc/tq_term_tables.cpp
+++ b/tantivy_amd/csrc/tq_term_tables.cpp
@@ -179,12 +179,59 @@
   s->share_span_terms = ~(size_t)0;
 }
 
+bool plan_lmat(tq_segment *s, uint32_t handle, bool *fill) {
+  TermHost &t = s->terms[handle];
+  *fill = false;
+  if (lead_mat_budget_x(s) <= 0 || !s->d_docmat) return false;
+  if (t.lmat_blob) {
+    if (t.lmat_epoch == s->docmat_epoch) return true;
+    if (s->docmat_epoch != s->docmat_epoch_planned) {
+      ++s->lmat_stale_skips;
+      return false;
+    }
+    t.lmat_epoch = s->docmat_epoch;
+    *fill = true;
+    return true;
+  }
+  if (s->lmat_off || !t.n_blocks || !t.d_self || t.field || t.set_kind != TermHost::kNoSet) return false;
+  if ((uint64_t)t.doc_freq * lead_mat_cut(s) > s->max_doc) return false;
+  const size_t bytes = (size_t)t.n_blocks * 1024u;
+  if (s->lmat_bytes_total + bytes > (size_t)lead_mat_budget_x(s) * (s->idx_len + s->pos_len + s->max_doc)) return false;
+  void *blob = nullptr;
+  if (dense_alloc(s, bytes + PAD, &blob) != TQ_OK) {
+    (void)hipGetLastError();
+    return false;
+  }
+  if ((uint64_t)blob & 15u) {
+    dense_release(s, blob);
+    return false;
+  }
+  if ((uint64_t)blob < s->share_table_lo + 8u || (uint64_t)blob + bytes - s->share_table_lo >= (8ull << 32)) {
+    dense_release(s, blob);
+    s->lmat_off = true;
+    return false;
+  }
+  t.lmat_blob = blob;
+  t.lmat_epoch = s->docmat_epoch;
+  s->lmat_bytes_total += bytes;
+  s->share_span_terms = ~(size_t)0;
+  *fill = true;
+  return true;
+}
+hipError_t fill_lmat(tq_segment *s, uint32_t handle, hipStream_t st) {
+  TermHost &t = s->terms[handle];
+  const hipError_t e = tqk_launch_lead_mat(s->dseg, t.d_self, 0u, t.n_blocks, (uint64_t *)t.lmat_blob, st);
+  if (e != hipSuccess) t.lmat_epoch = 0;
+  return e;
+}
+
 int ensure_docmat(tq_segment *s) {
   if (s->d_docmat) return TQ_OK;
   const size_t mat_bytes = (size_t)s->max_doc * sizeof(uint64_t);
   if (s->dense_bytes_total + mat_bytes > s->dense_budget()) return TQ_OK;
   HIP_TRY(hipMalloc((void **)&s->d_docmat, mat_bytes + PAD));
   HIP_TRY(hipMemsetAsync((uint8_t *)s->d_docmat + mat_bytes, 0, PAD, s->stream));
+  docmat_written(s);
   const hipError_t e = tqk_launch_docmat_init(s->d_docmat, s->d_fn, s->dseg.const_fieldnorm_id, s->max_doc, s->stream);
   if (e != hipSuccess) return fail(TQ_ERR_HIP, "docmat init: %s", hipGetErrorString(e));
   s->dense_bytes_total += mat_bytes;
@@ -211,6 +258,7 @@
   hipError_t e = hipSuccess;
   if (want_sig) {
     const uint32_t bit = sig_bit(handle);
+    docmat_written(s);
     e = tqk_launch_docmat_set(s->d_docmat, dl.dd, t.doc_freq, (TQD_SIG_SHIFT - 8u) + bit, s->max_doc, s->stream);
     if (e != hipSuccess) return fail(TQ_ERR_HIP, "docmat signature: %s", hipGetErrorString(e));
     s->h_dterms[handle].has_freq |= (bit + 1u) << 16;
@@ -276,6 +324,7 @@
     }
     if (s->d_docmat) {
       const uint32_t slot = s->n_mat_slots++;
+      docmat_written(s);
       e = tqk_launch_docmat_set(s->d_docmat, dd, t.doc_freq, slot, s->max_doc, s->stream);
       if (e != hipSuccess) return fail(TQ_ERR_HIP, "docmat set: %s", hipGetErrorString(e));
       static const bool kDocCls = tune_u32("TQ_DOCCLS", 1) != 0;
diff --git a/tantivy_amd/csrc/tq_terms.cpp b/tantivy_amd/csrc/tq_terms.cpp
--- a/tantivy_amd/csrc/tq_terms.cpp
+++ b/tantivy_amd/csrc/tq_terms.cpp
@@ -431,6 +431,7 @@
     uint32_t *const *d_tabs = (uint32_t *const *)(d_selfs + n_sig);
     const uint32_t *d_bits = (const uint32_t *)(d_tabs + n_sig);
     uint32_t *d_lmax = (uint32_t *)(d_bits + 3 * n_sig);
+    if (s->d_docmat) docmat_written(s);
     e = tqk_launch_docsig_batch(s->dseg, d_selfs, d_bits, n_sig, s->d_docmat, b.any_tab ? d_tabs : nullptr, d_bits + n_sig,
                                 d_bits + 2 * n_sig, s->d_local_cache, d_lmax, s->opt.use_dpp != 0, cs);
     if (e == hipSuccess && b.any_tab && s->d_local_cache) {
diff --git a/tantivy_amd/host/searcher.cpp b/tantivy_amd/host/searcher.cpp
--- a/tantivy_amd/host/searcher.cpp
+++ b/tantivy_amd/host/searcher.cpp
@@ -563,6 +563,26 @@
     for (auto &w : weights) total_terms += w.terms.size();
     handles.clear();
     handles.reserve(total_terms);
+    if (const std::atomic<tq_term_handle> *fast = seg.fast_handle_table()) {
+      size_t i = 0;
+      for (; i < n; ++i) {
+        const Weight &w = weights[i];
+        const size_t at = handles.size();
+        bool known = true;
+        for (uint32_t t : w.terms) {
+          const tq_term_handle h = t < SegmentReader::kFastHandles ? fast[t].load(std::memory_order_acquire) : SegmentReader::kHandleUnknown;
+          if (h == SegmentReader::kHandleUnknown) {
+            known = false;
+            break;
+          }
+          handles.push_back(h);
+        }
+        if (!known) break;
+        fill_record(qs[i], w, handles.data() + at, k);
+      }
+      if (i == n) return;
+      handles.clear();
+    }
     if (n > 1) {
       std::vector<uint32_t> fresh;
       for (auto &w : weights)
@@ -574,22 +594,24 @@
       const Weight &w = weights[i];
       const size_t at = handles.size();
       for (uint32_t t : w.terms) handles.push_back(resolve_handle(seg_p, w, t));
-      tq_query &q = qs[i];
-      q.n_terms = (uint32_t)w.terms.size();
-      q.terms = handles.data() + at;
-      q.weights = w.weights.data();
-      q.tf_cache = w.bm25->tf_cache();
-      q.mode = w.mode;
-      q.phrase_offsets = w.phrase_offsets.empty() ? nullptr : w.phrase_offsets.data();
-      q.k = k;
-      q.occurs = w.occurs.empty() ? nullptr : w.occurs.data();
-      q.clause_of = w.clause_of.empty() ? nullptr : w.clause_of.data();
-      q.min_should_match = w.min_should_match;
-      q.slop = w.slop;
-      q.nested_occurs = w.nested_occurs.empty() ? nullptr : w.nested_occurs.data();
-      q.clause_min_should = w.clause_min_should.empty() ? nullptr : w.clause_min_should.data();
-      q.atom_of = w.atom_of.empty() ? nullptr : w.atom_of.data();
-    }
+      fill_record(qs[i], w, handles.data() + at, k);
+    }
+  }
+  static void fill_record(tq_query &q, const Weight &w, const tq_term_handle *terms, uint32_t k) {
+    q.n_terms = (uint32_t)w.terms.size();
+    q.terms = terms;
+    q.weights = w.weights.data();
+    q.tf_cache = w.bm25->tf_cache();
+    q.mode = w.mode;
+    q.phrase_offsets = w.phrase_offsets.empty() ? nullptr : w.phrase_offsets.data();
+    q.k = k;
+    q.occurs = w.occurs.empty() ? nullptr : w.occurs.data();
+    q.clause_of = w.clause_of.empty() ? nullptr : w.clause_of.data();
+    q.min_should_match = w.min_should_match;
+    q.slop = w.slop;
+    q.nested_occurs = w.nested_occurs.empty() ? nullptr : w.nested_occurs.data();
+    q.clause_min_should = w.clause_min_should.empty() ? nullptr : w.clause_min_should.data();
+    q.atom_of = w.atom_of.empty() ? nullptr : w.atom_of.data();
   }
 };
 }
diff --git a/tantivy_amd/host/searcher.hpp b/tantivy_amd/host/searcher.hpp
--- a/tantivy_amd/host/searcher.hpp
+++ b/tantivy_amd/host/searcher.hpp
@@ -55,6 +55,9 @@
   tq_term_handle term_handle(uint32_t term_id);
   void prepare_terms(const uint32_t *term_ids, size_t n);
   bool handle_known(uint32_t term_id) const;
+  static constexpr uint32_t kFastHandles = 1u << 20;
+  static constexpr tq_term_handle kHandleUnknown = 0xFFFFFFFEu;
+  const std::atomic<tq_term_handle> *fast_handle_table() const { return fast_handles_.load(std::memory_order_acquire); }
   uint32_t max_doc() const { return max_doc_; }
   uint32_t segment_ord() const { return segment_ord_; }
   uint64_t total_num_tokens(uint32_t field = 0) const { return field < n_fields_ ? total_num_tokens_[field] : 0; }
@@ -71,8 +74,6 @@
   mutable std::mutex m_;
   mutable std::unordered_map<uint32_t, TermInfo> terms_;
   std::unordered_map<uint32_t, tq_term_handle> handles_;
-  static constexpr uint32_t kFastHandles = 1u << 20;
-  static constexpr tq_term_handle kHandleUnknown = 0xFFFFFFFEu;
   std::atomic<std::atomic<tq_term_handle> *> fast_handles_{nullptr};
   std::shared_ptr<const class TermInfoStore> store_;
 };
```

After: 12.36 million queries/s (median of 6 runs). 1.04x the previous value.
